# CICE-Consortium/CICE

Measured on AMD Instinct MI355X. Metric: EVP subcycle cell-updates/sec (gx1 fp64), higher is better.
Workload: dtype f64

## Files before the change

### __graft_entry__.py

```python
from __future__ import annotations

import os
import subprocess
import sys
from pathlib import Path

ROOT = Path(__file__).resolve().parent
CSRC = ROOT / "cice_amd" / "csrc"
LIB = ROOT / "cice_amd" / "libcice_evp_hip.so"
HIPCC = os.environ.get("HIPCC", "/opt/rocm/bin/hipcc")


def _stale(target: Path, sources) -> bool:
    if not target.exists():
        return True
    t = target.stat().st_mtime
    return any(Path(s).stat().st_mtime > t for s in sources)


HIP_SRCS = ["evp_kernels.hip", "evp_resident2.hip", "evp_halo_direct.hip", "evp_prep.hip",
            "evp_copy.hip", "evp_cgrid.hip", "evp_cgrid_res.hip", "evp_cgrid_prep.hip", "evp_march.hip", "evp_api.cpp", "evp_host_common.cpp", "evp_host_loop.cpp",
            "evp_host_resident.cpp", "evp_host_mailbox.cpp", "evp_host_prep.cpp", "evp_host_cgrid.cpp", "evp_host_march.cpp", "march_plan.cpp", "halo_plan.cpp", "cgrid_plan.cpp", "rim_plan.cpp"]
HIP_HDRS = ["evp_cell.inc", "evp_device.h", "evp_forcing.h", "evp_math.h", "halo_plan.h", "cgrid_plan.h", "evp_host.h", "evp_halo_direct.h", "march_plan.h", "rim_plan.h"]


LIB_TESTING = ROOT / "cice_amd" / "libcice_evp_hip_testing.so"
TESTING_KERNELS = {"evp_resident2.hip", "evp_cgrid_res.hip"}


def build_hip(force: bool = False) -> Path:
    from concurrent.futures import ThreadPoolExecutor
    srcs = [CSRC / n for n in HIP_SRCS if (CSRC / n).exists()]
    hdrs = [CSRC / n for n in HIP_HDRS if (CSRC / n).exists()] + [ROOT / "include" / "cice_evp_hip.h",
                                                                  ROOT / "include" / "cice_evp_hip_testing.h"]
    objdir = CSRC / "build"
    objdir.mkdir(exist_ok=True)
    flags = ["--offload-arch=gfx950", "-O3", "-std=c++17", "-fPIC"]
    jobs = [(src, objdir / (src.name + ".o"), []) for src in srcs]
    jobs += [(src, objdir / (src.name + ".testing.o"), ["-DCICE_EVP_HIP_TESTING"]) for src in srcs
             if src.suffix == ".cpp" or src.name in TESTING_KERNELS]

    def compile_one(job):
        src, obj, extra = job
        if force or _stale(obj, [src] + hdrs):
            subprocess.run([HIPCC, *flags, *extra, "-c", str(src), "-o", str(obj)], check=True)
        return obj

    with ThreadPoolExecutor(max_workers=min(8, os.cpu_count() or 1)) as ex:
        objs = list(ex.map(compile_one, jobs))
    kernels = [o for (src, o, extra) in jobs if src.suffix != ".cpp" and src.name not in TESTING_KERNELS]
    host = {False: [o for (src, o, extra) in jobs if (src.suffix == ".cpp" or src.name in TESTING_KERNELS) and not extra],
            True: [o for (src, o, extra) in jobs if extra]}
    for testing, lib in ((False, LIB), (True, LIB_TESTING)):
        mine = kernels + host[testing]
        if force or _stale(lib, mine + [CSRC / "exports.map"]):
            subprocess.run([HIPCC, "--offload-arch=gfx950", "-shared", "-fPIC", "-Wl,-Bsymbolic", f"-Wl,--version-script={CSRC / 'exports.map'}", *map(str, mine), "-o", str(lib),
                            "-L/opt/rocm/lib", "-lrccl"], check=True)
    return LIB


def build() -> None:
    build_hip()
    sys.path.insert(0, str(ROOT))
    sys.path.insert(0, str(ROOT / "oracle"))
    import oracle
    oracle.build()
    shim = ROOT / "cice_amd" / "fortran" / "build_shim.sh"
    if shim.exists():
        subprocess.run(["bash", str(shim)], check=True)
    ref = ROOT / "oracle" / "ref" / "build_ref.sh"
    try:
        have_reference = Path("/root/reference/cicecore").is_dir()
    except OSError:
        have_reference = False
    if have_reference:
        refdir = ROOT / "oracle" / "ref"
        srcs = [q for q in refdir.iterdir() if q.suffix in (".F90", ".c", ".sh")]
        shims = list((ROOT / "cice_amd" / "fortran").glob("*.F90"))
        out = ROOT / "oracle" / "_ref"
        for variant, binaries, extra in (("strict", ["evp_ref_harness_strict", "evp_hip_dropin_harness"], shims),
                                         ("fast", ["evp_ref_harness_fast", "evp_ref_harness_fast1d"], []),
                                         ("mpi", ["evp_ref_harness_mpistrict", "evp_ref_harness_mpifast", "evp_hip_dropin_harness_mpi"], shims)):
            if variant == "mpi" and not (Path("/opt/conda/include/mpif.h").exists() and Path("/opt/conda/lib/libmpifort.so.12").exists()):
                continue
            if any(_stale(out / b, srcs + extra) for b in binaries):
                subprocess.run(["bash", str(ref), variant], check=True)
    import cice_amd
    from cice_amd import evp
    evp.load_library()


def smoke() -> None:
    sys.path.insert(0, str(ROOT))
    sys.path.insert(0, str(ROOT / "oracle"))
    sys.path.insert(0, str(ROOT / "tests"))
    import numpy as np
    build_hip()
    from test_gpu_parity import run_hip, run_oracle, synth_case
    from cice_amd import synth
    scal = synth.evp_scalars(120)
    dc, geo, fields, tm, um = synth_case("gx3", "full", seed=1, warm=True, bs=(50, 58))
    want = run_oracle(dc, geo, fields, tm, um, scal, 8)
    got = run_hip(dc, geo, fields, tm, um, scal, strict=True, ndte=8)
    for k, w in want.items():
        assert np.array_equal(got[k].view(np.uint64), w.view(np.uint64)), f"smoke: {k} differs from the oracle (strict)"
    fused = run_hip(dc, geo, fields, tm, um, scal, strict=False, ndte=8)
# ... 11 lines not shown
```

### cice_amd/csrc/evp_api.cpp

```cpp
#include "evp_host.h"
#include "rim_plan.h"

using namespace evp_host;

namespace {
int32_t *at(int32_t *out, size_t k) { return out ? out + k : nullptr; }
template <class T> size_t copy_out(int32_t *out, const std::vector<T> &v, int stride = 1)
{
    for (size_t k = 0; out && k < v.size(); ++k) out[k * stride] = (int32_t)v[k];
    return v.size();
}
template <class T> size_t copy_out(int32_t *out, const std::vector<HaloPeer> &peers, std::vector<T> HaloPeer::*member, int stride = 1)
{
    size_t n = 0;
    for (const HaloPeer &p : peers) n += copy_out(at(out, n * stride), p.*member, stride);
    return n;
}
}

#ifdef CICE_EVP_HIP_TESTING
namespace {
struct PlanDump {
    int32_t *out;
    int32_t n = 0;
// ... 933 lines not shown
    PlanDump count{nullptr};
    count.put(S.plan);
    if (!out) return count.n;
    if (n < count.n) return fail(-1, "plan_dump: room for %d values, %d needed", (int)n, (int)count.n);
    PlanDump dump{out};
    dump.put(S.plan);
    return dump.n;
}

int cice_evp_hip_halo_plan(int32_t *counts4, int32_t *local_dst, int32_t *local_src,
                           int32_t *local_sign, int32_t *peer_rank, int32_t *peer_nsend,
                           int32_t *peer_nrecv, int32_t *send_src, int32_t *recv_dst)
{
    const HaloPlan &P = S.plan;
    copy_out(local_dst, P.local_dst);
    copy_out(local_src, P.local_src);
    copy_out(local_sign, P.local_sign);
    const size_t ns = copy_out(send_src, P.peers, &HaloPeer::send_src), nr = copy_out(recv_dst, P.peers, &HaloPeer::recv_dst);
    for (size_t q = 0; q < P.peers.size(); ++q) {
        if (peer_rank) peer_rank[q] = P.peers[q].rank;
        if (peer_nsend) peer_nsend[q] = (int32_t)P.peers[q].send_src.size();
        if (peer_nrecv) peer_nrecv[q] = (int32_t)P.peers[q].recv_dst.size();
    }
    if (counts4) {
        counts4[0] = (int32_t)P.local_dst.size();
        counts4[1] = (int32_t)P.peers.size();
        counts4[2] = (int32_t)ns;
        counts4[3] = (int32_t)nr;
    }
    return 0;
}

int cice_evp_hip_peer_plan(int32_t *send_dst, int32_t *recv_gid)
{
    copy_out(send_dst, S.plan.peers, &HaloPeer::send_dst);
    copy_out(recv_gid, S.plan.peers, &HaloPeer::recv_gid);
    return 0;
}

int cice_evp_hip_fold_images_plan(int32_t *counts4, int32_t *send_sign, int32_t *out3, int32_t *in3)
{
    const std::vector<HaloPeer> &peers = S.plan.peers;
    for (size_t q = 0; counts4 && q < peers.size(); ++q) {
        const HaloPeer &p = peers[q];
        counts4[4 * q] = p.n_ghost_send; counts4[4 * q + 1] = p.n_ghost_recv;
        counts4[4 * q + 2] = (int32_t)p.fimg_src.size(); counts4[4 * q + 3] = (int32_t)p.fimg_recv_dst.size();
    }
    copy_out(send_sign, peers, &HaloPeer::send_sign);
    copy_out(out3, peers, &HaloPeer::fimg_src, 3);
    copy_out(at(out3, 1), peers, &HaloPeer::fimg_dst, 3);
    copy_out(at(out3, 2), peers, &HaloPeer::fimg_sign, 3);
    copy_out(in3, peers, &HaloPeer::fimg_recv_dst, 3);
    copy_out(at(in3, 1), peers, &HaloPeer::fimg_recv_col, 3);
    copy_out(at(in3, 2), peers, &HaloPeer::fimg_recv_sign, 3);
    return 0;
}

int cice_evp_hip_peer_signs(int32_t *recv_sign)
{
    copy_out(recv_sign, S.plan.peers, &HaloPeer::recv_sign);
    return 0;
}

int cice_evp_hip_center_plan(int32_t *count, int32_t *dst, int32_t *src, int32_t *vsign)
{
    const HaloPlan &P = S.plan;
    const size_t n = copy_out(dst, P.center_dst);
    copy_out(src, P.center_src);
    copy_out(vsign, P.center_vsign);
    if (count) *count = (int32_t)n;
    return P.center_remote ? 1 : 0;
}

int cice_evp_hip_fold_split_plan(int32_t which, int32_t *count, int32_t *cells)
{
    const HaloPlan &P = S.plan;
    const std::vector<int32_t> *lists[9] = {&P.fold_shift_cells, &P.center_foldr_dst, &P.stress_foldr_dst, &P.center_seam_dst, &P.center_seam_slot,
                                            &P.stress_own_dst, &P.stress_own_src, &P.stress_corner_dst, &P.stress_corner_src};
    const size_t n = copy_out(cells, *lists[which >= 0 && which < 8 ? which : 8]);
    if (count) *count = (int32_t)n;
    return P.fold_split ? 1 : 0;
}

int cice_evp_hip_stress_plan(int32_t *count, int32_t *dst, int32_t *src)
{
    const size_t n = copy_out(dst, S.plan.stress_dst);
    copy_out(src, S.plan.stress_src);
    if (count) *count = (int32_t)n;
    return 0;
}
#endif

int cice_evp_hip_seam_fin_plan(int32_t *counts2, int32_t *dst, int32_t *a, int32_t *b, int32_t *coef)
{
    const HaloPlan &P = S.plan;
    if (counts2) { counts2[0] = (int32_t)P.fin_dst.size(); counts2[1] = (int32_t)P.tail; }
    copy_out(dst, P.fin_dst);
    copy_out(a, P.fin_a);
    copy_out(b, P.fin_b);
    copy_out(coef, P.fin_coef);
    return P.stress_remote ? 1 : 0;
}

int cice_evp_hip_march_info(int32_t *out, int32_t n)
{
    const State::March &M = S.march;
    const int32_t v[12] = {M.mode, (int32_t)std::min<long>(M.passes, 0x7fffffffL), M.declined, M.nstrips, M.nseg, M.seglen,
                           M.last_call ? 1 : 0, M.direct, M.kpass, (int32_t)std::min<long>(M.subcycles, 0x7fffffffL),
                           M.mode == 1 ? M.fold_h : 0, M.last_call ? M.call_band_subcycles : 0};
    for (int k = 0; out && k < n && k < 12; ++k) out[k] = v[k];
    return 0;
}

int cice_evp_hip_describe_path(char *buf, int32_t n)
{
    if (!buf || n < 2) return fail(-1, "describe_path: no buffer");
    const State::March &M = S.march;
    const char *kernel = S.res_mode == 1 ? (S.res_remote ? "on-chip resident (tagged records, neighbours on other ranks)"
                                                       : S.res2_rimu ? "on-chip resident (tagged records; edge U-cells in the rim wave)"
                                                                     : "on-chip resident (tagged records)")
                         : (M.last_call ? (M.kpass == 4 ? "four subcycles per pass (marching)" : M.kpass == 3 ? "three subcycles per pass (marching)" : "two subcycles per pass (marching)")
                                      : "one subcycle per launch (streaming)");
    const char *transport = S.plan.peers.empty() ? "none (one rank)" : (S.direct.on ? "mailbox over HIP IPC" : (S.have_comm ? "RCCL send/recv" : "not set up"));
    const char *ring = (M.mode == 1 && !S.plan.peers.empty())
                           ? (M.direct == 1 ? " (ring between ranks: stores into HIP-IPC-mapped inboxes)"
                                            : (M.direct == 2 ? " (ring between ranks: RCCL send/recv, direct stores on trial)" : " (ring between ranks: RCCL send/recv)"))
                           : "";
    char band[96] = "";
    if (M.mode == 1 && M.fold_h > 0)
        std::snprintf(band, sizeof band, " (tripole: rows 1 .. %d marched, fold band of %d rows one subcycle per launch)", M.fold_zone, M.fold_h);
    std::snprintf(buf, (size_t)n, "rank %d of %d: kernel = %s; halo transport = %s%s%s; marching path: %s%s%s%s%s; blocks %d, cells per exchange %d",
                  (int)S.d.rank, (int)std::max(1, (int)S.d.nranks), kernel, transport,
                  (!S.plan.peers.empty() && !S.direct.on && !S.direct.why.empty()) ? " (mailbox off: " : "",
                  (!S.plan.peers.empty() && !S.direct.on && !S.direct.why.empty()) ? (S.direct.why + ")").c_str() : "",
                  M.mode == 1 ? "on" : (M.mode == 0 ? "off" : "undecided"), (M.mode == 0 && !M.why.empty()) ? " -- " : "",
                  (M.mode == 0 && !M.why.empty()) ? M.why.c_str() : "", ring, band, (int)S.d.nblocks, (int)(S.msk.on ? S.msk.n_send : S.n_send));
    const std::string cg = cgrid_schedule();
    if (!cg.empty()) {
        const size_t used = std::strlen(buf);
        std::snprintf(buf + used, (size_t)n - used, "; %s", cg.c_str());
    }
    return 0;
}

#ifdef CICE_EVP_HIP_TESTING
int cice_evp_hip_plan_flags(int32_t *flags, int32_t n)
{
    const HaloPlan &P = S.plan;
    const int32_t v[5] = {P.any_fold_exchange, P.fold_rows, P.stress_remote, P.center_remote, P.center_fold_remote};
    int32_t k = 0;
    for (; flags && k < n && k < 5; ++k) flags[k] = v[k];
    return k;
}

int cice_evp_hip_cgrid_fold_xplan(int32_t loc, int32_t *info4, int32_t *count, int32_t *dst, int32_t *a, int32_t *b, int32_t *flip)
{
    if (loc < 0 || loc > 3) return fail(-1, "bad location %d", (int)loc);
    const HaloPlan &P = S.plan;
    if (info4) {
        info4[0] = P.cg_split ? 1 : 0;
        info4[1] = P.cg_tail;
        info4[2] = (int32_t)P.cg_peers.size();
        info4[3] = 0;
        for (const HaloPeer &p : P.cg_peers) info4[3] += (int32_t)p.send_src.size();
    }
    const FoldList &L = P.cg_fold[loc];
// ... 44 lines not shown
```

### cice_amd/csrc/evp_cell.inc

```

struct StressIn {
    double u_ij, u_im, u_jm, u_mm;
    double v_ij, v_im, v_jm, v_mm;
    double dxT, dyT, dxhy, dyhx, cxp, cyp, cxm, cym, DminTarea, strength;
};

__device__ __forceinline__ void metrics_cell(double hte, double hte_im, double htn, double htn_jm,
                                             double deltaminEVP, StressIn &a)
{
    a.cyp = (c1p5 * hte - p5 * hte_im);
    a.cxp = (c1p5 * htn - p5 * htn_jm);
    a.cym = -(c1p5 * hte_im - p5 * hte);
    a.cxm = -(c1p5 * htn_jm - p5 * htn);
    a.dxhy = p5 * (hte - hte_im);
    a.dyhx = p5 * (htn - htn_jm);
    const double tarea = a.dxT * a.dyT;
    a.DminTarea = deltaminEVP * tarea;
}

template <int CAP, bool SIMPLE = false>
__device__ __forceinline__ void visc_replpress(const EvpScalars &p, double strength, double DminArea,
                                               double Delta, double &zetax2, double &etax2,
                                               double &rep_prs)
{
    double tmpcalc;
    if (CAP == 1) {
        tmpcalc = strength / fmax(Delta, DminArea);
    } else if (CAP == 0) {
        tmpcalc = strength / (Delta + DminArea);
    } else {
        tmpcalc = p.capping * (strength / fmax(Delta, DminArea)) +
                  (1.0 - p.capping) * (strength / (Delta + DminArea));
    }
    if (SIMPLE) {
        zetax2 = tmpcalc;
        rep_prs = tmpcalc * Delta;
    } else {
        zetax2 = (1.0 + p.Ktens) * tmpcalc;
        rep_prs = (1.0 - p.Ktens) * tmpcalc * Delta;
    }
    etax2 = p.epp2i * zetax2;
}

template <int CAP, bool SIMPLE = false>
__device__ __forceinline__ void stress_cell(const EvpScalars &p, const StressIn &a, double (&s)[12],
                                            double (&str)[8])
{
    const double divune = a.cyp * a.u_ij - a.dyT * a.u_im + a.cxp * a.v_ij - a.dxT * a.v_jm;
    const double divunw = a.cym * a.u_im + a.dyT * a.u_ij + a.cxp * a.v_im - a.dxT * a.v_mm;
    const double divusw = a.cym * a.u_mm + a.dyT * a.u_jm + a.cxm * a.v_mm + a.dxT * a.v_im;
    const double divuse = a.cyp * a.u_jm - a.dyT * a.u_mm + a.cxm * a.v_jm + a.dxT * a.v_ij;
    const double tensionne = -a.cym * a.u_ij - a.dyT * a.u_im + a.cxm * a.v_ij + a.dxT * a.v_jm;
    const double tensionnw = -a.cyp * a.u_im + a.dyT * a.u_ij + a.cxm * a.v_im + a.dxT * a.v_mm;
    const double tensionsw = -a.cyp * a.u_mm + a.dyT * a.u_jm + a.cxp * a.v_mm - a.dxT * a.v_im;
    const double tensionse = -a.cym * a.u_jm - a.dyT * a.u_mm + a.cxp * a.v_jm - a.dxT * a.v_ij;
    const double shearne = -a.cym * a.v_ij - a.dyT * a.v_im - a.cxm * a.u_ij - a.dxT * a.u_jm;
    const double shearnw = -a.cyp * a.v_im + a.dyT * a.v_ij - a.cxm * a.u_im - a.dxT * a.u_mm;
    const double shearsw = -a.cyp * a.v_mm + a.dyT * a.v_jm - a.cxp * a.u_mm + a.dxT * a.u_im;
    const double shearse = -a.cym * a.v_jm - a.dyT * a.v_mm - a.cxp * a.u_jm + a.dxT * a.u_ij;
    const double Deltane = sqrt(divune * divune + p.e_factor * (tensionne * tensionne + shearne * shearne));
    const double Deltanw = sqrt(divunw * divunw + p.e_factor * (tensionnw * tensionnw + shearnw * shearnw));
    const double Deltasw = sqrt(divusw * divusw + p.e_factor * (tensionsw * tensionsw + shearsw * shearsw));
    const double Deltase = sqrt(divuse * divuse + p.e_factor * (tensionse * tensionse + shearse * shearse));

    double zetax2ne, etax2ne, rep_prsne, zetax2nw, etax2nw, rep_prsnw;
    double zetax2sw, etax2sw, rep_prssw, zetax2se, etax2se, rep_prsse;
    visc_replpress<CAP, SIMPLE>(p, a.strength, a.DminTarea, Deltane, zetax2ne, etax2ne, rep_prsne);
    visc_replpress<CAP, SIMPLE>(p, a.strength, a.DminTarea, Deltanw, zetax2nw, etax2nw, rep_prsnw);
    visc_replpress<CAP, SIMPLE>(p, a.strength, a.DminTarea, Deltasw, zetax2sw, etax2sw, rep_prssw);
    visc_replpress<CAP, SIMPLE>(p, a.strength, a.DminTarea, Deltase, zetax2se, etax2se, rep_prsse);

    const double arlx1i = p.arlx1i, revp = p.revp, denom1 = p.denom1;
    if (SIMPLE) {
        s[0] = (s[0] + arlx1i * (zetax2ne * divune - rep_prsne)) * denom1;
        s[1] = (s[1] + arlx1i * (zetax2nw * divunw - rep_prsnw)) * denom1;
        s[2] = (s[2] + arlx1i * (zetax2sw * divusw - rep_prssw)) * denom1;
        s[3] = (s[3] + arlx1i * (zetax2se * divuse - rep_prsse)) * denom1;

        s[4] = (s[4] + arlx1i * etax2ne * tensionne) * denom1;
        s[5] = (s[5] + arlx1i * etax2nw * tensionnw) * denom1;
        s[6] = (s[6] + arlx1i * etax2sw * tensionsw) * denom1;
        s[7] = (s[7] + arlx1i * etax2se * tensionse) * denom1;

        s[8] = (s[8] + arlx1i * p5 * etax2ne * shearne) * denom1;
        s[9] = (s[9] + arlx1i * p5 * etax2nw * shearnw) * denom1;
        s[10] = (s[10] + arlx1i * p5 * etax2sw * shearsw) * denom1;
        s[11] = (s[11] + arlx1i * p5 * etax2se * shearse) * denom1;
    } else {
    s[0] = (s[0] * (1.0 - arlx1i * revp) + arlx1i * (zetax2ne * divune - rep_prsne)) * denom1;
    s[1] = (s[1] * (1.0 - arlx1i * revp) + arlx1i * (zetax2nw * divunw - rep_prsnw)) * denom1;
    s[2] = (s[2] * (1.0 - arlx1i * revp) + arlx1i * (zetax2sw * divusw - rep_prssw)) * denom1;
    s[3] = (s[3] * (1.0 - arlx1i * revp) + arlx1i * (zetax2se * divuse - rep_prsse)) * denom1;

    s[4] = (s[4] * (1.0 - arlx1i * revp) + arlx1i * etax2ne * tensionne) * denom1;
    s[5] = (s[5] * (1.0 - arlx1i * revp) + arlx1i * etax2nw * tensionnw) * denom1;
    s[6] = (s[6] * (1.0 - arlx1i * revp) + arlx1i * etax2sw * tensionsw) * denom1;
    s[7] = (s[7] * (1.0 - arlx1i * revp) + arlx1i * etax2se * tensionse) * denom1;

    s[8] = (s[8] * (1.0 - arlx1i * revp) + arlx1i * p5 * etax2ne * shearne) * denom1;
    s[9] = (s[9] * (1.0 - arlx1i * revp) + arlx1i * p5 * etax2nw * shearnw) * denom1;
    s[10] = (s[10] * (1.0 - arlx1i * revp) + arlx1i * p5 * etax2sw * shearsw) * denom1;
    s[11] = (s[11] * (1.0 - arlx1i * revp) + arlx1i * p5 * etax2se * shearse) * denom1;
    }

    const double ssigpn = s[0] + s[1];
    const double ssigps = s[2] + s[3];
    const double ssigpe = s[0] + s[3];
    const double ssigpw = s[1] + s[2];
    const double ssigp1 = (s[0] + s[2]) * p055;
    const double ssigp2 = (s[1] + s[3]) * p055;

    const double ssigmn = s[4] + s[5];
    const double ssigms = s[6] + s[7];
    const double ssigme = s[4] + s[7];
    const double ssigmw = s[5] + s[6];
    const double ssigm1 = (s[4] + s[6]) * p055;
    const double ssigm2 = (s[5] + s[7]) * p055;

    const double ssig12n = s[8] + s[9];
    const double ssig12s = s[10] + s[11];
    const double ssig12e = s[8] + s[11];
    const double ssig12w = s[9] + s[10];
    const double ssig121 = (s[8] + s[10]) * p111;
    const double ssig122 = (s[9] + s[11]) * p111;

    const double csigpne = p111 * s[0] + ssigp2 + p027 * s[2];
    const double csigpnw = p111 * s[1] + ssigp1 + p027 * s[3];
    const double csigpsw = p111 * s[2] + ssigp2 + p027 * s[0];
    const double csigpse = p111 * s[3] + ssigp1 + p027 * s[1];

    const double csigmne = p111 * s[4] + ssigm2 + p027 * s[6];
    const double csigmnw = p111 * s[5] + ssigm1 + p027 * s[7];
    const double csigmsw = p111 * s[6] + ssigm2 + p027 * s[4];
    const double csigmse = p111 * s[7] + ssigm1 + p027 * s[5];

    const double csig12ne = p222 * s[8] + ssig122 + p055 * s[10];
    const double csig12nw = p222 * s[9] + ssig121 + p055 * s[11];
    const double csig12sw = p222 * s[10] + ssig122 + p055 * s[8];
    const double csig12se = p222 * s[11] + ssig121 + p055 * s[9];

    const double str12ew = p5 * a.dxT * (p333 * ssig12e + p166 * ssig12w);
    const double str12we = p5 * a.dxT * (p333 * ssig12w + p166 * ssig12e);
    const double str12ns = p5 * a.dyT * (p333 * ssig12n + p166 * ssig12s);
    const double str12sn = p5 * a.dyT * (p333 * ssig12s + p166 * ssig12n);

    double strp_tmp = p25 * a.dyT * (p333 * ssigpn + p166 * ssigps);
    double strm_tmp = p25 * a.dyT * (p333 * ssigmn + p166 * ssigms);
    str[0] = -strp_tmp - strm_tmp - str12ew + a.dxhy * (-csigpne + csigmne) + a.dyhx * csig12ne;
    str[1] = strp_tmp + strm_tmp - str12we + a.dxhy * (-csigpnw + csigmnw) + a.dyhx * csig12nw;
    strp_tmp = p25 * a.dyT * (p333 * ssigps + p166 * ssigpn);
    strm_tmp = p25 * a.dyT * (p333 * ssigms + p166 * ssigmn);
    str[2] = -strp_tmp - strm_tmp + str12ew + a.dxhy * (-csigpse + csigmse) + a.dyhx * csig12se;
    str[3] = strp_tmp + strm_tmp + str12we + a.dxhy * (-csigpsw + csigmsw) + a.dyhx * csig12sw;

    strp_tmp = p25 * a.dxT * (p333 * ssigpe + p166 * ssigpw);
    strm_tmp = p25 * a.dxT * (p333 * ssigme + p166 * ssigmw);
    str[4] = -strp_tmp + strm_tmp - str12ns - a.dyhx * (csigpne + csigmne) + a.dxhy * csig12ne;
    str[5] = strp_tmp - strm_tmp - str12sn - a.dyhx * (csigpse + csigmse) + a.dxhy * csig12se;
    strp_tmp = p25 * a.dxT * (p333 * ssigpw + p166 * ssigpe);
    strm_tmp = p25 * a.dxT * (p333 * ssigmw + p166 * ssigme);
    str[6] = -strp_tmp + strm_tmp + str12ns - a.dyhx * (csigpnw + csigmnw) + a.dxhy * csig12nw;
    str[7] = strp_tmp - strm_tmp + str12sn - a.dyhx * (csigpsw + csigmsw) + a.dxhy * csig12sw;
}

struct CornerIn {
    double ua, va, ub, vb, ud, vd;
    double cyA, cyB, cxA, cxB, DY, DX;
    double strength, DminTarea;
};
template <int CAP, bool SIMPLE = false>
__device__ __forceinline__ void stress_corner(const EvpScalars &p, const CornerIn &c, double &sp, double &sm, double &s12)
{
    const double divu = c.cyA * c.ua + c.DY * c.ub + c.cxA * c.va + c.DX * c.vd;
    const double tension = -c.cyB * c.ua + c.DY * c.ub + c.cxB * c.va - c.DX * c.vd;
    const double shear = -c.cyB * c.va + c.DY * c.vb - c.cxB * c.ua + c.DX * c.ud;
    const double Delta = sqrt(divu * divu + p.e_factor * (tension * tension + shear * shear));
    double zetax2, etax2, rep_prs;
    visc_replpress<CAP, SIMPLE>(p, c.strength, c.DminTarea, Delta, zetax2, etax2, rep_prs);
    const double arlx1i = p.arlx1i, revp = p.revp, denom1 = p.denom1;
    if (SIMPLE) {
        sp = (sp + arlx1i * (zetax2 * divu - rep_prs)) * denom1;
        sm = (sm + arlx1i * etax2 * tension) * denom1;
        s12 = (s12 + arlx1i * p5 * etax2 * shear) * denom1;
    } else {
        sp = (sp * (1.0 - arlx1i * revp) + arlx1i * (zetax2 * divu - rep_prs)) * denom1;
        sm = (sm * (1.0 - arlx1i * revp) + arlx1i * etax2 * tension) * denom1;
        s12 = (s12 * (1.0 - arlx1i * revp) + arlx1i * p5 * etax2 * shear) * denom1;
    }
}
__device__ __forceinline__ void corner_operands(int q, double dxT, double dyT, double cxp, double cyp, double cxm, double cym,
                                                CornerIn &c, double &KX, double &K12X, double &KYP, double &K12Y)
{
    const bool east = q == 0 || q == 3, north = q < 2;
    c.cyA = east ? cyp : cym; c.cyB = east ? cym : cyp;
    c.cxA = north ? cxp : cxm; c.cxB = north ? cxm : cxp;
    c.DY = east ? -dyT : dyT;
    c.DX = north ? -dxT : dxT;
    KX = (east ? -p25 : p25) * dyT;
    K12X = (north ? -p5 : p5) * dxT;
    KYP = (north ? -p25 : p25) * dxT;
    K12Y = (east ? -p5 : p5) * dyT;
}
__device__ __forceinline__ void stress_corner_partials(double P0, double P1, double P2, double P3, double M0, double M1, double M2,
                                                       double M3, double T0, double T1, double T2, double T3, double KX, double K12X,
                                                       double KYP, double K12Y, double dxhy, double dyhx, double &X, double &Y)
{
    const double csigp = p111 * P0 + (P1 + P3) * p055 + p027 * P2;
    const double csigm = p111 * M0 + (M1 + M3) * p055 + p027 * M2;
    const double csig12 = p222 * T0 + (T1 + T3) * p111 + p055 * T2;
    const double str12x = K12X * (p333 * (T0 + T3) + p166 * (T1 + T2));
    const double str12y = K12Y * (p333 * (T0 + T1) + p166 * (T2 + T3));
    const double strp_x = KX * (p333 * (P0 + P1) + p166 * (P2 + P3));
    const double strm_x = KX * (p333 * (M0 + M1) + p166 * (M2 + M3));
    X = strp_x + strm_x + str12x + dxhy * (-csigp + csigm) + dyhx * csig12;
    const double strp_y = KYP * (p333 * (P0 + P3) + p166 * (P1 + P2));
    const double strm_y = -KYP * (p333 * (M0 + M3) + p166 * (M1 + M2));
    Y = strp_y + strm_y + str12y - dyhx * (csigp + csigm) + dxhy * csig12;
}

struct StepuIn {
    double uold, vold;
    double vrelfac;
    double uocn, vocn, waterx, watery, forcex, forcey, Umassdti, fm, uarear, TbU;
    double uvel_init, vvel_init;
    double sx0, sx1, sx2, sx3;
    double sy0, sy1, sy2, sy3;
};

struct StepuOut {
    double u, v, strintx, strinty, taubx, tauby;
};

struct StepuPre {
    double taux, tauy, Cb, cca, ccb, ab2;
    double bu, bv;
};

template <bool SIMPLE = false, bool TBU = true, bool WITH_B = true>
__device__ __forceinline__ void stepu_pre_cell(const EvpScalars &p, const StepuIn &a, StepuPre &w)
{
    const double uold = a.uold, vold = a.vold;
    const double du = a.uocn - uold, dv = a.vocn - vold;
    const double vrel = a.vrelfac * sqrt(du * du + dv * dv);
    w.taux = vrel * a.waterx;
    w.tauy = vrel * a.watery;
    double Cb = 0.0;
    if (TBU) Cb = a.TbU / (sqrt(uold * uold + vold * vold) + p.u0);
    w.Cb = Cb;
    double cca, ccb;
    if (SIMPLE) {
        cca = p.brlx * a.Umassdti + vrel + Cb;
        ccb = a.fm;
    } else {
        cca = (p.brlx + p.revp) * a.Umassdti + vrel * p.cosw + Cb;
        ccb = a.fm + copysign(1.0, a.fm) * vrel * p.sinw;
    }
    w.cca = cca; w.ccb = ccb;
    w.ab2 = cca * cca + ccb * ccb;
    if (!WITH_B) return;
    if (SIMPLE) {
        w.bu = p.brlx * uold + 0.0;
        w.bv = p.brlx * vold + 0.0;
    } else {
        w.bu = p.brlx * uold + p.revp * a.uvel_init;
        w.bv = p.brlx * vold + p.revp * a.vvel_init;
    }
}

template <bool SIMPLE = false, bool WITH_B = true>
__device__ __forceinline__ void stepu_post_cell(const EvpScalars &p, const StepuIn &a, const StepuPre &w, StepuOut &o)
{
    o.strintx = a.uarear * (a.sx0 + a.sx1 + a.sx2 + a.sx3);
    o.strinty = a.uarear * (a.sy0 + a.sy1 + a.sy2 + a.sy3);
    double cc1, cc2;
    if (WITH_B) {
        cc1 = o.strintx + a.forcex + w.taux + a.Umassdti * w.bu;
        cc2 = o.strinty + a.forcey + w.tauy + a.Umassdti * w.bv;
    } else if (SIMPLE) {
        cc1 = o.strintx + a.forcex + w.taux + a.Umassdti * (p.brlx * a.uold + 0.0);
        cc2 = o.strinty + a.forcey + w.tauy + a.Umassdti * (p.brlx * a.vold + 0.0);
    } else {
        cc1 = o.strintx + a.forcex + w.taux + a.Umassdti * (p.brlx * a.uold + p.revp * a.uvel_init);
        cc2 = o.strinty + a.forcey + w.tauy + a.Umassdti * (p.brlx * a.vold + p.revp * a.vvel_init);
    }
    o.u = (w.cca * cc1 + w.ccb * cc2) / w.ab2;
    o.v = (w.cca * cc2 - w.ccb * cc1) / w.ab2;
    o.taubx = -o.u * w.Cb;
    o.tauby = -o.v * w.Cb;
}

template <bool SIMPLE = false, bool TBU = true>
__device__ __forceinline__ void stepu_cell(const EvpScalars &p, const StepuIn &a, StepuOut &o)
{
    StepuPre w;
    stepu_pre_cell<SIMPLE, TBU, false>(p, a, w);
    stepu_post_cell<SIMPLE, false>(p, a, w, o);
}

struct DeformOut {
    double divu, shear, vort, rdg_conv, rdg_shear;
};

__device__ __forceinline__ void deform_cell(const EvpScalars &p, const StressIn &a, double tarear,
                                            double dyU_ij, double dyU_im, double dyU_jm, double dyU_mm,
                                            double dxU_ij, double dxU_im, double dxU_jm, double dxU_mm,
                                            DeformOut &o)
{
    const double divune = a.cyp * a.u_ij - a.dyT * a.u_im + a.cxp * a.v_ij - a.dxT * a.v_jm;
    const double divunw = a.cym * a.u_im + a.dyT * a.u_ij + a.cxp * a.v_im - a.dxT * a.v_mm;
    const double divusw = a.cym * a.u_mm + a.dyT * a.u_jm + a.cxm * a.v_mm + a.dxT * a.v_im;
    const double divuse = a.cyp * a.u_jm - a.dyT * a.u_mm + a.cxm * a.v_jm + a.dxT * a.v_ij;
    const double tensionne = -a.cym * a.u_ij - a.dyT * a.u_im + a.cxm * a.v_ij + a.dxT * a.v_jm;
    const double tensionnw = -a.cyp * a.u_im + a.dyT * a.u_ij + a.cxm * a.v_im + a.dxT * a.v_mm;
    const double tensionsw = -a.cyp * a.u_mm + a.dyT * a.u_jm + a.cxp * a.v_mm - a.dxT * a.v_im;
    const double tensionse = -a.cym * a.u_jm - a.dyT * a.u_mm + a.cxp * a.v_jm - a.dxT * a.v_ij;
    const double shearne = -a.cym * a.v_ij - a.dyT * a.v_im - a.cxm * a.u_ij - a.dxT * a.u_jm;
    const double shearnw = -a.cyp * a.v_im + a.dyT * a.v_ij - a.cxm * a.u_im - a.dxT * a.u_mm;
    const double shearsw = -a.cyp * a.v_mm + a.dyT * a.v_jm - a.cxp * a.u_mm + a.dxT * a.u_im;
    const double shearse = -a.cym * a.v_jm - a.dyT * a.v_mm - a.cxp * a.u_jm + a.dxT * a.u_ij;
    const double Deltane = sqrt(divune * divune + p.e_factor * (tensionne * tensionne + shearne * shearne));
    const double Deltanw = sqrt(divunw * divunw + p.e_factor * (tensionnw * tensionnw + shearnw * shearnw));
    const double Deltasw = sqrt(divusw * divusw + p.e_factor * (tensionsw * tensionsw + shearsw * shearsw));
    const double Deltase = sqrt(divuse * divuse + p.e_factor * (tensionse * tensionse + shearse * shearse));

    o.divu = p25 * (divune + divunw + divuse + divusw) * tarear;
    const double tmp = p25 * (Deltane + Deltanw + Deltase + Deltasw) * tarear;
    o.rdg_conv = -fmin(o.divu, 0.0);
    o.rdg_shear = p5 * (tmp - fabs(o.divu));
    const double tsum = tensionne + tensionnw + tensionse + tensionsw;
    const double ssum = shearne + shearnw + shearse + shearsw;
    o.shear = p25 * tarear * sqrt(tsum * tsum + ssum * ssum);
    const double dvdxn = dyU_ij * a.v_ij - dyU_im * a.v_im;
    const double dvdxs = dyU_jm * a.v_jm - dyU_mm * a.v_mm;
    const double dudye = dxU_ij * a.u_ij - dxU_jm * a.u_jm;
    const double dudyw = dxU_im * a.u_im - dxU_mm * a.u_mm;
    o.vort = p5 * tarear * (dvdxn + dvdxs - dudye - dudyw);
}

__device__ __forceinline__ void finish_cell(const EvpScalars &p, double Cw, double aiX, double uocn,
                                            double vocn, double u, double v, double fm,
                                            double &strocnx, double &strocny)
{
    const double du = uocn - u, dv = vocn - v;
    double vrel = p.rhow * Cw * sqrt(du * du + dv * dv);
    vrel = vrel * aiX;
    strocnx = vrel * ((uocn - u) * p.cosw - (vocn - v) * p.sinw * copysign(1.0, fm));
    strocny = vrel * ((vocn - v) * p.cosw + (uocn - u) * p.sinw * copysign(1.0, fm));
}
```

### cice_amd/csrc/evp_device.h

```cpp
#pragma once
const char *evp_env_test(const char *key);
#include <hip/hip_runtime.h>
#include <stdint.h>
#include <algorithm>

struct EvpScalars {
    double arlx1i, denom1, brlx, revp;
    double e_factor, epp2i;
    double capping, Ktens;
    double u0, cosw, sinw;
    double rhow;
};

struct EvpArgs {
    EvpScalars p;
    int nx, ny;
    size_t plane;
    int gx, gy, ntiles;
    int xcdmap;
    const int *tile_list;
    int tile_count;
    int last;
    const int4 *blk;
    const uint8_t *mask;
    const double *u_in, *v_in;
    double *u_out, *v_out;
    const double *sig_in[12];
    double *sig_out[12];
    const double *dxT, *dyT, *dxhy, *dyhx, *cxp, *cyp, *cxm, *cym, *DminTarea, *uarear;
    const double *HTE, *HTN;
    double deltaminEVP;
    const double *strength, *Cw, *aiX, *uocn, *vocn, *waterx, *watery, *forcex, *forcey;
    const double *umassdti, *fm, *TbU, *uvel_init, *vvel_init;
    const double *vrelfac;
    unsigned flags;
    const int *push;
    int push_ni, push_nj;
    double *strintx, *strinty, *taubx, *tauby;
    const struct EvpDirect *dx;
    unsigned *dx_count;
    unsigned *dx_fseq;
    int dx_nb;
};

void evp_resident_geometry(int max_ni, int max_nj, int logw, int *gx, int *gy);
#define EVP_RES2_RING 256
struct EvpResident2 {
    int ndte;
    int cur0;
    int dry;
    unsigned tag_base;
    unsigned spin_limit;
    int *err;
    const uint8_t *pubmap;
    const int4 *ring;
    const int *ring_cnt;
    void *rec[2];
    double *u[2], *v[2];
    double *const *tab;
    int nblocks;
    const int *order;
    int nlaunch;
    const uint8_t *live;
    const int *celltile;
    const uint8_t *perm;
    const uint8_t *uperm;
    const uint8_t *late_waves;
    const uint8_t *nact;
    const uint8_t *nlate;
    int *cuload;
    unsigned long long *prof;
    int dbg;
    int par0;
    const int2 *rimg;
    void *const *peer_rec;
    const size_t *peer_rstride;
    unsigned long long timeout_ticks;
    const int *seam;
    int tfold;
    const int *img3;
    void *rec_raw[2];
    const int2 *rraw;
    void *const *peer_raw;
    const size_t *peer_raw_stride;
};
int evp_resident2_max_blocks_per_cu(bool strict, int cap, unsigned flags, int logw, bool remote, bool coop = false);
bool evp_resident2_coop_built(bool strict, int cap, int logw, bool remote);
bool evp_resident2_lean_built(bool strict, int cap, int logw, bool remote);
void evp_launch_resident2(const EvpArgs &A, const EvpResident2 &R, int max_ni, int max_nj, int logw,
                          bool strict, int cap, int lean, hipStream_t st);

#ifndef EVP_MARCH_PAD
#define EVP_MARCH_PAD 4
#endif
#define EVP_MARCH_KMAX EVP_MARCH_PAD
#define EVP_MARCH_OWN (64 - 2 * EVP_MARCH_PAD)
#define EVP_MARCH_S_NF 14
#define EVP_MARCH_C_NF 13
#define EVP_MARCH_O_NF 5
#define EVP_MARCH_D_NF 4
#define EVP_MARCH_NODUP 0xffffffffu
struct EvpMarch {
    EvpScalars p;
    double deltaminEVP;
    int nxr, nyr;
    int ldx;
    int own;
    int nstrips, nseg, seglen, nitems;
    int wrapx;
    int last;
    int kpass;
    int order;
    unsigned flags;
    const uint8_t *mask;
    const double *st_in;
    double *st_out;
    const double *cst;
    const double *opt;
    double *diag;
    const unsigned *dup;
    const int4 *items;
};
struct EvpMarchGeo {
    int nxr, nyr, ldx, rows;
    int own, nstrips;
    int nxb, nyb, plane;
    int nblocks;
    int bsx, bsy, nbx, nby;
    int ilo;
    int wrapx;
    int gx0, gy0, nxg, nyg, ew_cyclic;
    int ext_w, ext_s, nxo, nyo;
    int nyblk;
    const int *blkid;
    const int2 *blk_org;
    const int4 *blk;
};
#define EVP_MARCH_TAB 40
struct EvpMarchTab {
    double *blk[EVP_MARCH_TAB];
    double *pk[EVP_MARCH_TAB];
    double *pk2[EVP_MARCH_TAB];
    int nf[EVP_MARCH_TAB];
    int slot[EVP_MARCH_TAB];
    int n;
};
void evp_launch_march(const EvpMarch &A, bool strict, int mode, hipStream_t st);
struct EvpMarchRows { int y0, y1, j0, nj; };
constexpr EvpMarchRows EvpMarchAllRows{-(1 << 28), 1 << 28, 1, 1 << 28};
void evp_launch_march_gather(const EvpMarchGeo &G, const EvpMarchTab &T, const uint8_t *mask_blk, uint8_t *mask_rect,
                             EvpMarchRows W, hipStream_t st);
void evp_launch_march_check(const EvpMarchGeo &G, const EvpMarchTab &T, const uint8_t *mask_blk, const uint8_t *mask_rect,
                            int nuv, int nfringe, unsigned *bad, EvpMarchRows W, hipStream_t st);
void evp_launch_march_scatter(const EvpMarchGeo &G, const EvpMarchTab &T, const uint8_t *mask_blk, int nuv, int nsig,
                              EvpMarchRows W, hipStream_t st);
#define EVP_MARCH_DIRECT_MAXPEER 16
struct EvpRingCuts {
    int n;
    int start[EVP_MARCH_DIRECT_MAXPEER + 1];
};
void evp_launch_march_pack(const double *buf, int nf, const int *pos, int n, const EvpRingCuts &C, double *out, hipStream_t st);
struct EvpMarchDirect {
    int npeers;
    double *dst[EVP_MARCH_DIRECT_MAXPEER];
    size_t dst_pstride[EVP_MARCH_DIRECT_MAXPEER];
    unsigned *peer_flag[EVP_MARCH_DIRECT_MAXPEER];
    unsigned *flags_in;
    unsigned *count;
// ... 285 lines not shown
```

### cice_amd/csrc/evp_host_resident.cpp

```cpp
#include "evp_host.h"
#include "rim_plan.h"

namespace evp_host {

bool tripole_seam() { return (S.n_seam + S.n_pole + S.n_late) > 0 || S.plan.tail > 0 || !S.plan.fin_dst.empty(); }

static bool tfold_image(size_t k)
{
    if (!S.plan.tfold) return false;
    const int dst = S.plan.local_dst[k];
    const int b = dst / (int)S.plane, r = dst % (int)S.plane, j = r / S.d.nx_block + 1, i = r % S.d.nx_block + 1;
    return i >= S.ilo[b] && i <= S.ihi[b] && j >= S.jlo[b] && j <= S.jhi[b];
}

bool resident_possible(bool with_peers)
{
    if (!with_peers && !S.plan.peers.empty()) return false;
    if (S.plan.tfold) {
        for (const HaloPeer &p : S.plan.peers)
            for (int k = 0; k < p.n_ghost_recv; ++k) {
                const int dst = p.recv_dst[k];
                const int b = dst / (int)S.plane, r = dst % (int)S.plane, j = r / S.d.nx_block + 1, i = r % S.d.nx_block + 1;
                if (i >= S.ilo[b] && i <= S.ihi[b] && j >= S.jlo[b] && j <= S.jhi[b]) return false;
            }
// ... 297 lines not shown
    }
    S.res2_rimu_ok = rimu_ok;
    S.res2_coop_ok = coop_ok;
    const bool off = env_test("CICE_EVP_HIP_RES_ORDER") && !std::atoi(env_test("CICE_EVP_HIP_RES_ORDER"));
    std::vector<int> order((size_t)ntiles, 0);
    for (int w = 0; w < nrun; ++w) order[w] = run[w];
    if (!off) {
        hipDeviceProp_t prop;
        int ncu = 256;
        if (hipGetDeviceProperties(&prop, S.device) == hipSuccess && prop.multiProcessorCount > 0) ncu = prop.multiProcessorCount;
        std::vector<int> by_cost = run;
        std::stable_sort(by_cost.begin(), by_cost.end(), [&](int a, int c) { return cost[a] > cost[c]; });
        std::vector<int> slots((size_t)ncu), load((size_t)ncu, 0);
        std::vector<std::vector<int>> mine((size_t)ncu);
        for (int c = 0; c < ncu; ++c) slots[c] = nrun / ncu + (c < nrun % ncu ? 1 : 0);
        for (int tile : by_cost) {
            int best = -1;
            for (int c = 0; c < ncu; ++c) {
                if ((int)mine[c].size() >= slots[c]) continue;
                if (best < 0 || load[c] < load[best] || (load[c] == load[best] && slots[c] < slots[best])) best = c;
            }
            mine[best].push_back(tile);
            load[best] += cost[tile] >> 10;
        }
        for (int c = 0; c < ncu; ++c)
            for (size_t k = 0; k < mine[c].size(); ++k) order[c + (int)k * ncu] = mine[c][k];
    }
    if (S.res2_order_for != S.res2_logw) S.mem.free_one(S.res2_order);
    if (!S.res2_order && S.mem.alloc(S.res2_order, order.size())) return -1;
    HIPC(hipMemcpyAsync(S.res2_order, order.data(), order.size() * sizeof(int), hipMemcpyHostToDevice, S.stream));
    HIPC(hipMemcpyAsync(S.res2_live, live.data(), live.size(), hipMemcpyHostToDevice, S.stream));
    HIPC(hipStreamSynchronize(S.stream));
    S.res2_nlive = nrun;
    S.res2_order_for = S.res2_logw;
    S.res2_order_stale = false;
    return 0;
}

int launch_resident2(int ndte, int cur0, bool dry)
{
    if (ndte >= 4096) return fail(-6, "resident2: ndte must be < 4096");
    if (int rc = resident_tables()) return rc;
    if (int rc = resident2_order()) return rc;
    EvpArgs A;
    fill_args(A, cur0, 1);
    EvpResident2 R;
    R.ndte = ndte;
    R.cur0 = dry ? 0 : cur0;
    R.dry = dry ? 1 : 0;
    S.res2_epoch = (S.res2_epoch + 1u) & 0xFFFFFu;
    if (S.res2_epoch == 0) S.res2_epoch = 1;
    R.tag_base = S.res2_epoch << 12;
    R.par0 = S.res2_par;
    S.res2_par = (S.res2_par + ndte + 1) & 1;
    R.nblocks = S.d.nblocks;
    R.order = S.res2_order;
    R.nlaunch = S.res2_nlive;
    R.live = S.plan.peers.empty() ? S.res2_live : nullptr;
    R.celltile = S.res2_celltile;
    R.perm = S.res2_perm;
    R.late_waves = S.res2_late;
    R.nact = S.res2_nact;
    {
        const int want = env_test("CICE_EVP_HIP_RES_COOP") ? std::atoi(env_test("CICE_EVP_HIP_RES_COOP")) : EVP_RES2_COOP_DEFAULT;
        bool can = want != 0 && S.res2_coop_ok && S.res2_logw == 4 && !S.res_remote &&
                   evp_resident2_coop_built(S.prm.strict != 0, cap_mode(), S.res2_logw, false);
        if (can) {
            hipDeviceProp_t prop;
            const int per_cu = std::min(evp_resident2_max_blocks_per_cu(S.prm.strict != 0, cap_mode(), A.flags, 4, false, true), 8);
            can = hipGetDeviceProperties(&prop, S.device) == hipSuccess &&
                  (long)std::max(S.res2_nlive, 1) * 10 <= (long)per_cu * prop.multiProcessorCount * 9;
        }
        S.res2_coop = can ? 1 : 0;
        R.nlate = can ? S.res2_nlate : nullptr;
    }
    R.cuload = S.res2_cuload;
    R.prof = nullptr;
    if (S.res2_logw == 4 && env_test("CICE_EVP_HIP_RES_PROF") && std::atoi(env_test("CICE_EVP_HIP_RES_PROF"))) {
        if (!S.res2_prof && S.mem.alloc(S.res2_prof, (size_t)S.res2_ntiles * 32)) return -1;
        HIPC(hipMemsetAsync(S.res2_prof, 0, (size_t)S.res2_ntiles * 32 * sizeof(unsigned long long), S.stream));
        R.prof = S.res2_prof;
    }
    const int dbg2 = env_test("CICE_EVP_HIP_RES_DEBUG") ? std::atoi(env_test("CICE_EVP_HIP_RES_DEBUG")) : 0;
    R.dbg = dbg2;
    R.seam = S.res2_seam;
    R.tfold = S.plan.tfold ? 1 : 0;
    R.img3 = S.res2_img3;
    R.rec_raw[0] = S.res2_rec_raw[0];
    R.rec_raw[1] = S.res2_rec_raw[1];
    R.rimg = S.res_remote ? S.res2_rimg : nullptr;
    R.peer_rec = S.res2_peer_rec;
    R.peer_rstride = S.res2_peer_rstride;
    R.rraw = S.res_remote ? S.res2_rraw : nullptr;
    R.peer_raw = S.res2_peer_raw;
    R.peer_raw_stride = S.res2_peer_raw_stride;
    const double tmo_ms = env("CICE_EVP_HIP_HALO_TIMEOUT_MS") ? std::atof(env("CICE_EVP_HIP_HALO_TIMEOUT_MS")) : 30000.0;
    R.timeout_ticks = (unsigned long long)((S.res_timeout_ms > 0 ? S.res_timeout_ms : tmo_ms) * 1.0e5);
    R.spin_limit = 4000000u;
    R.err = S.res_err;
    R.pubmap = S.res2_pub;
    R.ring = S.res2_ring;
    R.ring_cnt = S.res2_cnt;
    R.rec[0] = S.res2_rec[0];
    R.rec[1] = S.res2_rec[1];
    if (dry) {
        R.u[0] = S.u[cur0]; R.v[0] = S.v[cur0]; R.u[1] = S.u[cur0]; R.v[1] = S.v[cur0];
    } else {
        R.u[0] = S.u[0]; R.v[0] = S.v[0]; R.u[1] = S.u[1]; R.v[1] = S.v[1];
    }
    R.tab = S.res_tab + (dry ? 28 * (1 + cur0) : 0);
    const bool lean = evp_resident2_lean_built(S.prm.strict != 0, cap_mode(), S.res2_logw, R.rimg != nullptr) &&
                      R.nblocks == 1 && !R.seam && !R.tfold && !R.img3 && !R.rimg && !R.rraw && !R.nlate &&
                      A.p.revp == 0.0 && (A.flags & EVP_F_WATER_IS_OCN) && (A.flags & EVP_F_TBU_ZERO) &&
                      !(env_test("CICE_EVP_HIP_RES_LEAN") && !std::atoi(env_test("CICE_EVP_HIP_RES_LEAN")));
    const int want_rimu = env_test("CICE_EVP_HIP_RES_RIMU") ? std::atoi(env_test("CICE_EVP_HIP_RES_RIMU")) : EVP_RES2_RIMU_DEFAULT;
    const bool rimu = lean && want_rimu != 0 && S.res2_rimu_ok && !(dbg2 & (32 | 256 | 512));
    R.uperm = nullptr;
    if (rimu) { R.perm = S.res2_perm_rim; R.uperm = S.res2_uperm; R.nact = S.res2_nact_rim; }
    S.res2_rimu = rimu ? 1 : 0;
    evp_launch_resident2(A, R, S.max_ni, S.max_nj, S.res2_logw, S.prm.strict != 0, cap_mode(), rimu ? 2 : lean ? 1 : 0, S.stream);
    HIPC(hipGetLastError());
    return 0;
}

int resident_tables()
{
    if (!S.res_tab) {
        double *tab[3][28];
        for (int v = 0; v < 3; ++v) {
            for (int k = 0; k < 12; ++k) {
                tab[v][k] = S.sig[v == 0 ? 0 : v - 1][k];
                tab[v][12 + k] = S.sig[v == 0 ? 1 : v - 1][k];
            }
            tab[v][24] = S.in[F_STRINTX]; tab[v][25] = S.in[F_STRINTY];
            tab[v][26] = S.in[F_TAUBX]; tab[v][27] = S.in[F_TAUBY];
        }
        if (S.mem.alloc(S.res_tab, sizeof tab / sizeof(double *))) return -1;
        HIPC(hipMemcpy(S.res_tab, tab, sizeof tab, hipMemcpyHostToDevice));
    }
    return 0;
}

int resident_check_error()
{
    if (!S.res_launched) return 0;
    S.res_launched = false;
    int ev[8] = {0};
    HIPC(hipMemcpy(ev, S.res_err, sizeof ev, hipMemcpyDeviceToHost));
    const int e = ev[0];
    if (e) {
        HIPC(hipMemset(S.res_err, 0, sizeof ev));
        S.res_mode = 0;
        return fail(-7, "resident EVP kernel: a wait gave up (%s; tile %d, subcycle %d, cell %d, tag seen %#x, wanted %#x)%s",
                    e == 1 ? "record of this GPU" : e == 2 ? "record of another rank" : e == 3 ? "fold-row partner"
                           : e == 5 ? "interior waves of the tile" : "?",
                    ev[1], ev[2], ev[3], (unsigned)ev[4], (unsigned)ev[5],
                    e == 2 ? " -- CICE_EVP_HIP_HALO_TIMEOUT_MS bounds the wait for other ranks"
                           : " -- workgroups not co-resident?");
    }
    return 0;
}


int tune_after_upload()
{
    float ms = 0;
    if (!S.tyb_forced && !S.tuned) {
// ... 74 lines not shown
```

### cice_amd/csrc/evp_math.h

```cpp
#pragma once
#include <hip/hip_runtime.h>
#include "evp_device.h"

namespace {

__device__ constexpr double p027 = 1.0 / 36.0;
__device__ constexpr double p055 = 1.0 / 18.0;
__device__ constexpr double p111 = 1.0 / 9.0;
__device__ constexpr double p166 = 1.0 / 6.0;
__device__ constexpr double p222 = 2.0 / 9.0;
__device__ constexpr double p25 = 0.25;
__device__ constexpr double p333 = 1.0 / 3.0;
__device__ constexpr double p5 = 0.5;
__device__ constexpr double c1p5 = 1.5;

}

#pragma clang fp contract(off)
namespace evp_strict {
#include "evp_cell.inc"
}
#pragma clang fp contract(on)
namespace evp_fused {
#include "evp_cell.inc"
}

namespace {

template <bool STRICT> struct Math;
template <> struct Math<true> {
    using SI = evp_strict::StressIn;
    using UI = evp_strict::StepuIn;
    using UO = evp_strict::StepuOut;
    template <int MODE>
    static __device__ __forceinline__ void stress(const EvpScalars &p, const SI &a, double (&s)[12], double (&str)[8])
    {
        evp_strict::stress_cell<(MODE == 3 ? 1 : MODE), MODE == 3>(p, a, s, str);
    }
    template <int MODE = -1, bool TBU = true>
    static __device__ __forceinline__ void stepu(const EvpScalars &p, const UI &a, UO &o) { evp_strict::stepu_cell<MODE == 3, TBU>(p, a, o); }
    using UP = evp_strict::StepuPre;
    template <int MODE = -1, bool TBU = true>
    static __device__ __forceinline__ void stepu_pre(const EvpScalars &p, const UI &a, UP &w) { evp_strict::stepu_pre_cell<MODE == 3, TBU>(p, a, w); }
    template <int MODE = -1>
    static __device__ __forceinline__ void stepu_post(const EvpScalars &p, const UI &a, const UP &w, UO &o) { evp_strict::stepu_post_cell<MODE == 3, true>(p, a, w, o); }
    static __device__ __forceinline__ void metrics(double hte, double hte_im, double htn, double htn_jm, double dmin, SI &a)
    {
        evp_strict::metrics_cell(hte, hte_im, htn, htn_jm, dmin, a);
    }
    using CI = evp_strict::CornerIn;
    template <int MODE>
    static __device__ __forceinline__ void corner(const EvpScalars &p, const CI &c, double &sp, double &sm, double &s12)
    {
        evp_strict::stress_corner<(MODE == 3 ? 1 : MODE), MODE == 3>(p, c, sp, sm, s12);
    }
    static __device__ __forceinline__ void corner_operands(int q, double dxT, double dyT, double cxp, double cyp, double cxm, double cym,
                                                           CI &c, double &KX, double &K12X, double &KYP, double &K12Y)
    {
        evp_strict::corner_operands(q, dxT, dyT, cxp, cyp, cxm, cym, c, KX, K12X, KYP, K12Y);
    }
    static __device__ __forceinline__ void partials(double P0, double P1, double P2, double P3, double M0, double M1, double M2, double M3,
                                                    double T0, double T1, double T2, double T3, double KX, double K12X, double KYP,
                                                    double K12Y, double dxhy, double dyhx, double &X, double &Y)
    {
        evp_strict::stress_corner_partials(P0, P1, P2, P3, M0, M1, M2, M3, T0, T1, T2, T3, KX, K12X, KYP, K12Y, dxhy, dyhx, X, Y);
    }
};
template <> struct Math<false> {
    using SI = evp_fused::StressIn;
    using UI = evp_fused::StepuIn;
    using UO = evp_fused::StepuOut;
    template <int MODE>
    static __device__ __forceinline__ void stress(const EvpScalars &p, const SI &a, double (&s)[12], double (&str)[8])
    {
        evp_fused::stress_cell<(MODE == 3 ? 1 : MODE), MODE == 3>(p, a, s, str);
    }
    template <int MODE = -1, bool TBU = true>
    static __device__ __forceinline__ void stepu(const EvpScalars &p, const UI &a, UO &o) { evp_fused::stepu_cell<MODE == 3, TBU>(p, a, o); }
    using UP = evp_fused::StepuPre;
    template <int MODE = -1, bool TBU = true>
    static __device__ __forceinline__ void stepu_pre(const EvpScalars &p, const UI &a, UP &w) { evp_fused::stepu_pre_cell<MODE == 3, TBU>(p, a, w); }
    template <int MODE = -1>
    static __device__ __forceinline__ void stepu_post(const EvpScalars &p, const UI &a, const UP &w, UO &o) { evp_fused::stepu_post_cell<MODE == 3, true>(p, a, w, o); }
    static __device__ __forceinline__ void metrics(double hte, double hte_im, double htn, double htn_jm, double dmin, SI &a)
    {
        evp_fused::metrics_cell(hte, hte_im, htn, htn_jm, dmin, a);
    }
    using CI = evp_fused::CornerIn;
    template <int MODE>
    static __device__ __forceinline__ void corner(const EvpScalars &p, const CI &c, double &sp, double &sm, double &s12)
    {
        evp_fused::stress_corner<(MODE == 3 ? 1 : MODE), MODE == 3>(p, c, sp, sm, s12);
    }
    static __device__ __forceinline__ void corner_operands(int q, double dxT, double dyT, double cxp, double cyp, double cxm, double cym,
                                                           CI &c, double &KX, double &K12X, double &KYP, double &K12Y)
    {
        evp_fused::corner_operands(q, dxT, dyT, cxp, cyp, cxm, cym, c, KX, K12X, KYP, K12Y);
    }
    static __device__ __forceinline__ void partials(double P0, double P1, double P2, double P3, double M0, double M1, double M2, double M3,
                                                    double T0, double T1, double T2, double T3, double KX, double K12X, double KYP,
                                                    double K12Y, double dxhy, double dyhx, double &X, double &Y)
    {
        evp_fused::stress_corner_partials(P0, P1, P2, P3, M0, M1, M2, M3, T0, T1, T2, T3, KX, K12X, KYP, K12Y, dxhy, dyhx, X, Y);
    }
};

}
```

### cice_amd/csrc/evp_resident2.hip

```cpp
#include <hip/hip_runtime.h>
#include <stdint.h>
#include <algorithm>

#ifdef CICE_EVP_HIP_TESTING
#define RES_DBG(R) ((R).dbg)
#define RES_PROF(R) ((R).prof != nullptr)
#else
#define RES_DBG(R) 0
#define RES_PROF(R) false
#endif

#include "evp_math.h"

namespace {

constexpr int RTY = 4;

typedef unsigned v4u __attribute__((ext_vector_type(4)));

__device__ __forceinline__ void st_rec2(void *p, v4u a, v4u b)
{
    asm volatile("global_store_dwordx4 %0, %1, off sc1\n\tglobal_store_dwordx4 %0, %2, off offset:16 sc1"
                 :
                 : "v"(p), "v"(a), "v"(b)
                 : "memory");
}
__device__ __forceinline__ void ld_rec2(const void *p, v4u &a, v4u &b)
{
    asm volatile("global_load_dwordx4 %0, %2, off sc1\n\tglobal_load_dwordx4 %1, %2, off offset:16 sc1\n\ts_waitcnt vmcnt(0)"
                 : "=&v"(a), "=&v"(b)
                 : "v"(p)
                 : "memory");
}
__device__ __forceinline__ void st_rec2_s(const void *base, unsigned off, v4u a, v4u b)
{
    asm volatile("global_store_dwordx4 %0, %1, %3 sc1\n\tglobal_store_dwordx4 %0, %2, %3 offset:16 sc1"
                 :
                 : "v"(off), "v"(a), "v"(b), "s"(base)
                 : "memory");
}
__device__ __forceinline__ void ld_rec2_s(const void *base, unsigned off, v4u &a, v4u &b)
{
    asm volatile("global_load_dwordx4 %0, %2, %3 sc1\n\tglobal_load_dwordx4 %1, %2, %3 offset:16 sc1\n\ts_waitcnt vmcnt(0)"
                 : "=&v"(a), "=&v"(b)
                 : "v"(off), "s"(base)
                 : "memory");
}
__device__ __forceinline__ void st_rec2_sys(void *p, v4u a, v4u b)
{
    asm volatile("global_store_dwordx4 %0, %1, off sc0 sc1\n\tglobal_store_dwordx4 %0, %2, off offset:16 sc0 sc1"
                 :
                 : "v"(p), "v"(a), "v"(b)
                 : "memory");
}
__device__ __forceinline__ void ld_rec2_sys(const void *p, v4u &a, v4u &b)
{
    asm volatile("global_load_dwordx4 %0, %2, off sc0 sc1\n\tglobal_load_dwordx4 %1, %2, off offset:16 sc0 sc1\n\ts_waitcnt vmcnt(0)"
                 : "=&v"(a), "=&v"(b)
                 : "v"(p)
                 : "memory");
}
__device__ __forceinline__ v4u pack_rec(double x, unsigned tag)
{
    const unsigned long long bits = (unsigned long long)__double_as_longlong(x);
    v4u r;
    r.x = tag; r.y = (unsigned)bits; r.z = (unsigned)(bits >> 32); r.w = tag;
    return r;
}
__device__ __forceinline__ double unpack_rec(v4u r)
{
    return __longlong_as_double((long long)(((unsigned long long)r.z << 32) | r.y));
}

template <int CTRL>
__device__ __forceinline__ double quad_perm(double v)
{
    const long long b = __double_as_longlong(v);
    const int lo = __builtin_amdgcn_update_dpp(0, (int)(b & 0xffffffffll), CTRL, 0xf, 0xf, false);
    const int hi = __builtin_amdgcn_update_dpp(0, (int)(b >> 32), CTRL, 0xf, 0xf, false);
    return __longlong_as_double(((long long)hi << 32) | (unsigned)lo);
}
constexpr int QP_X1 = 0xB1, QP_X2 = 0x4E, QP_X3 = 0x1B;

template <bool STRICT, int CAP, int LOGW, bool REMOTE, bool COOP = false, bool LEAN = false, bool RIMU = false>
__global__ __launch_bounds__(64 * RTY, REMOTE ? 2 : 3) void evp_resident2_tile(EvpArgs A, EvpResident2 R)
{
    static_assert(!COOP || (STRICT && CAP == 3 && LOGW == 4), "COOP: 16 x 16 tiles, strict build, default scalars");
    static_assert(!LEAN || (!REMOTE && !COOP && LOGW == 4), "LEAN: one rank, 16 x 16 tiles, one thread per rim cell");
    static_assert(!RIMU || LEAN, "RIMU: a schedule of the lean loop");
    using MM = Math<STRICT>;
    constexpr int W = 1 << LOGW;
    constexpr int H = 256 / W;
    constexpr int LW = W + 1;
    constexpr int NUV = ((H + 1) * LW + 7) & ~7;
    constexpr bool PERM = (LOGW == 4);
    constexpr int NSTR = RIMU ? 8 : PERM ? 6 : 4;
    constexpr int SW = PERM ? W + 1 : W;
    constexpr int SP = SW * H;
    extern __shared__ __attribute__((aligned(16))) double smem[];
    double *s_str = smem;
    double *s_tc = smem + NSTR * SP;
    double *s_u = s_tc + 4 * 256;
    double *s_v = s_u + NUV;
    double *s_uc = s_v + NUV;
    double *s_rc = nullptr, *s_r04 = nullptr;
    __shared__ int s_bad;

    __shared__ int s_chunk[4], s_simd[4], s_cu;
    __shared__ int s_slot[4];

    const int tx = threadIdx.x, ty = threadIdx.y;
    const int t = ty * 64 + tx;
    const int tile = R.order ? R.order[blockIdx.x] : (int)blockIdx.x;
    bool no_ucell;
    {
        const int pb = A.gx * A.gy;
        const int4 rb = A.blk[tile / pb];
        no_ucell = rb.x + ((tile % pb) % A.gx) * (W - 1) > rb.y || rb.z + ((tile % pb) / A.gx) * (H - 1) > rb.w;
        if (no_ucell && !(RES_DBG(R) & 512)) return;
    }
    int tq = t;
    int cu_rank = 0;
    if (PERM && R.cuload && !(RES_DBG(R) & 64)) {
        const int wave = t >> 6;
        if ((t & 63) == 0) {
            unsigned hw, xcc;
            asm volatile("s_getreg_b32 %0, hwreg(HW_REG_HW_ID)" : "=s"(hw));
            asm volatile("s_getreg_b32 %0, hwreg(HW_REG_XCC_ID)" : "=s"(xcc));
            s_simd[wave] = (int)((hw >> 4) & 3u);
            if (wave == 0) s_cu = (int)(((xcc & 7u) << 8) | ((hw >> 8) & 0xffu));
        }
        __syncthreads();
        if (t == 0) {
            int *L = R.cuload + 8 * s_cu;
            const int nact = R.nact[tile];
            int chunk_of[4] = {0, 1, 2, 3};
            unsigned spins = 0;
            bool locked = false;
            while (spins++ < 200000u) {
                if (atomicCAS(&L[0], 0, 1) == 0) { locked = true; break; }
                __builtin_amdgcn_s_sleep(2);
            }
            if (locked) {
                int ld[4];
                const int stamp = __hip_atomic_load(&L[1], __ATOMIC_RELAXED, __HIP_MEMORY_SCOPE_AGENT);
                const bool fresh = stamp != (int)R.tag_base;
#pragma unroll
                for (int q = 0; q < 4; ++q)
                    ld[q] = fresh ? 0 : __hip_atomic_load(&L[2 + q], __ATOMIC_RELAXED, __HIP_MEMORY_SCOPE_AGENT);
                const int rank = fresh ? 0 : __hip_atomic_load(&L[6], __ATOMIC_RELAXED, __HIP_MEMORY_SCOPE_AGENT);
                s_simd[0] |= rank << 8;
                bool used[4] = {false, false, false, false};
                for (int ck = 0; ck < 4; ++ck) {
                    int best = -1;
                    for (int w = 0; w < 4; ++w) {
                        if (used[w]) continue;
                        if (best < 0 || ld[s_simd[w] & 3] < ld[s_simd[best] & 3]) best = w;
                    }
                    used[best] = true;
                    chunk_of[best] = ck;
                    if (ck < nact) ld[s_simd[best] & 3] += 1;
                }
#pragma unroll
                for (int q = 0; q < 4; ++q) __hip_atomic_store(&L[2 + q], ld[q], __ATOMIC_RELAXED, __HIP_MEMORY_SCOPE_AGENT);
                __hip_atomic_store(&L[6], rank + 1, __ATOMIC_RELAXED, __HIP_MEMORY_SCOPE_AGENT);
                __hip_atomic_store(&L[1], (int)R.tag_base, __ATOMIC_RELAXED, __HIP_MEMORY_SCOPE_AGENT);
                asm volatile("s_waitcnt vmcnt(0)" ::: "memory");
                __hip_atomic_store(&L[0], 0, __ATOMIC_RELAXED, __HIP_MEMORY_SCOPE_AGENT);
            }
#pragma unroll
            for (int w = 0; w < 4; ++w) s_chunk[w] = chunk_of[w];
        }
        __syncthreads();
// ... 13 lines not shown
    const int by = (tile % per_blk) / A.gx;
    const int4 r = A.blk[bz];
    const int i0 = r.x + bx * (W - 1), j0 = r.z + by * (H - 1);
    const int i = i0 + tcol;
    const int j = j0 + trow;
    const int nx = A.nx, ny = A.ny;
    const int cb = bz * (int)A.plane;
    const int c = cb + (j - 1) * nx + (i - 1);
    const int li = (trow + 1) * LW + (tcol + 1);
    const int upos = RIMU ? (int)R.uperm[tile * 256 + tq] : pos;
    const int ucol = upos & (W - 1), urow = upos >> LOGW;
    const int ui = RIMU ? i0 + ucol : i, uj = RIMU ? j0 + urow : j;
    const int cu = RIMU ? cb + (uj - 1) * nx + (ui - 1) : c;
    const int uli = RIMU ? (urow + 1) * LW + (ucol + 1) : li;
    const int usp = RIMU ? urow * SW + ucol : sp;
    const unsigned flags = A.flags;
    const bool water = !LEAN && !(flags & EVP_F_WATER_IS_OCN);
    const bool tbu = !LEAN && !(flags & EVP_F_TBU_ZERO);
    if (COOP) {
        s_rc = s_uc + (8 + (water ? 2 : 0) + (tbu ? 1 : 0)) * 256;
        s_r04 = s_rc + 10 * 64;
    }

    const bool inT = (i <= r.y + 1) && (j <= r.w + 1);
    unsigned m = 0;
    if (inT) m = A.mask[c];
    const bool actT = inT && (m & 1u);
    const bool ownU = (ucol < W - 1) && (urow < H - 1) && (ui <= r.y) && (uj <= r.w);
    unsigned mU = m;
    if (RIMU) mU = ownU ? A.mask[cu] : 0u;
    const bool isU = ownU && (mU & 2u);
    const bool own = (tcol < W - 1 || i == r.y + 1) && (trow < H - 1 || j == r.w + 1);
    const bool pub = ownU && (R.pubmap[cu] != 0);
    const int par0 = R.par0;
    const int nlate = COOP ? (int)R.nlate[tile] : 0;
    const bool rim_owner = COOP && tq < nlate;
    const bool actN = actT && !rim_owner;
    const int g = t >> 2, qc = t & 3;
    const bool quad = COOP && g < nlate;
    int gc = 0;
    unsigned g_vel = 0, g_out = 0;
    bool gown = false;
    double sr0 = 0.0, sr1 = 0.0, sr2 = 0.0;
    if (quad) {
        const int gpos = (int)R.perm[tile * 256 + g];
        const int gcol = gpos & (W - 1), grow = gpos >> LOGW;
        const int gi = i0 + gcol, gj = j0 + grow;
        gc = cb + (gj - 1) * nx + (gi - 1);
        gown = (gcol < W - 1 || gi == r.y + 1) && (grow < H - 1 || gj == r.w + 1);
        const int gli = (grow + 1) * LW + (gcol + 1);
        const int ij = gli, im = gli - 1, jm = gli - LW, mm = gli - LW - 1;
        const int g_oa = qc == 0 ? ij : qc == 1 ? im : qc == 2 ? mm : jm;
        const int g_ob = qc == 0 ? im : qc == 1 ? ij : qc == 2 ? jm : mm;
        const int g_od = qc == 0 ? jm : qc == 1 ? mm : qc == 2 ? im : ij;
        g_vel = (unsigned)g_oa | ((unsigned)g_ob << 10) | ((unsigned)g_od << 20);
        const int gsp = grow * SW + gcol;
        const int off04 = (int)(s_r04 - s_str);
        const int g_ox = qc == 0 ? off04 + g : (qc == 1 ? 4 : qc == 2 ? 2 : 0) * SP + gsp;
        const int g_oy = qc == 0 ? off04 + 64 + g : (qc == 1 ? 5 : qc == 2 ? 3 : 1) * SP + gsp;
        g_out = (unsigned)g_ox | ((unsigned)g_oy << 16);
        sr0 = R.tab[R.cur0 * 12 + qc][gc];
        sr1 = R.tab[R.cur0 * 12 + 4 + qc][gc];
        sr2 = R.tab[R.cur0 * 12 + 8 + qc][gc];
        if (qc == 0) {
            typename MM::SI b;
            b.dxT = A.dxT[gc]; b.dyT = A.dyT[gc];
            b.strength = A.strength[gc];
            if ((flags & EVP_F_METRICS) && !(flags & EVP_F_DXHY_ARRAY)) {
                MM::metrics(A.HTE[gc], A.HTE[gc - 1], A.HTN[gc], A.HTN[gc - nx], A.deltaminEVP, b);
            } else {
                b.dxhy = A.dxhy[gc]; b.dyhx = A.dyhx[gc];
                b.cxp = A.cxp[gc]; b.cyp = A.cyp[gc]; b.cxm = A.cxm[gc]; b.cym = A.cym[gc];
                b.DminTarea = A.DminTarea[gc];
            }
            s_rc[0 * 64 + g] = b.strength; s_rc[1 * 64 + g] = b.DminTarea;
            s_rc[2 * 64 + g] = b.dxT; s_rc[3 * 64 + g] = b.dyT;
            s_rc[4 * 64 + g] = b.cxp; s_rc[5 * 64 + g] = b.cyp; s_rc[6 * 64 + g] = b.cxm; s_rc[7 * 64 + g] = b.cym;
            s_rc[8 * 64 + g] = b.dxhy; s_rc[9 * 64 + g] = b.dyhx;
        }
    }

    typename MM::SI a;
    double s[12];
    if (actN) {
#pragma unroll
        for (int k = 0; k < 12; ++k) s[k] = R.tab[R.cur0 * 12 + k][c];
        a.dxT = A.dxT[c]; a.dyT = A.dyT[c];
        a.strength = A.strength[c];
        if ((flags & EVP_F_METRICS) && !(flags & EVP_F_DXHY_ARRAY)) {
            MM::metrics(A.HTE[c], A.HTE[c - 1], A.HTN[c], A.HTN[c - nx], A.deltaminEVP, a);
        } else {
            a.dxhy = A.dxhy[c]; a.dyhx = A.dyhx[c];
            a.cxp = A.cxp[c]; a.cyp = A.cyp[c]; a.cxm = A.cxm[c]; a.cym = A.cym[c];
            a.DminTarea = A.DminTarea[c];
        }
        s_tc[0 * 256 + t] = a.strength;
        s_tc[1 * 256 + t] = a.DminTarea;
        s_tc[2 * 256 + t] = a.dxhy;
        s_tc[3 * 256 + t] = a.dyhx;
    }
    if (isU) {
        s_uc[0 * 256 + t] = A.vrelfac[cu];
        s_uc[1 * 256 + t] = A.uocn[cu];
        s_uc[2 * 256 + t] = A.vocn[cu];
        s_uc[3 * 256 + t] = A.forcex[cu];
        s_uc[4 * 256 + t] = A.forcey[cu];
        s_uc[5 * 256 + t] = A.umassdti[cu];
        s_uc[6 * 256 + t] = A.fm[cu];
        s_uc[7 * 256 + t] = A.uarear[cu];
        int row = 8;
        if (water) { s_uc[row * 256 + t] = A.waterx[cu]; s_uc[(row + 1) * 256 + t] = A.watery[cu]; row += 2; }
        if (tbu) s_uc[row * 256 + t] = A.TbU[cu];
    }
    {
        const double *u0 = R.u[R.cur0], *v0 = R.v[R.cur0];
        for (int q = t; q < (H + 1) * LW; q += 256) {
            const int pr = q / LW - 1, pc = q % LW - 1;
            const int gi = i0 + pc, gj = j0 + pr;
            double uu = 0.0, vv = 0.0;
            if (gi >= 1 && gi <= nx && gj >= 1 && gj <= ny) {
                const int cp = cb + (gj - 1) * nx + (gi - 1);
                uu = u0[cp]; vv = v0[cp];
            }
            s_u[q] = uu; s_v[q] = vv;
        }
    }
    int img0 = -1, img1 = -1, img2 = -1;
    int seam_role = 0, seam_partner = -1;
    if (!LEAN && R.seam && ownU && j == r.w) {
        const int sv = R.seam[bz * nx + i - 1];
        seam_role = sv & 3;
        seam_partner = sv >> 2;
    }
    const bool isSeam = seam_role != 0;
    if (!LEAN && R.img3) {
        if (ownU) { img0 = R.img3[3 * c]; img1 = R.img3[3 * c + 1]; img2 = R.img3[3 * c + 2]; }
    } else
    if (ownU && (flags & EVP_F_PUSH) && (ui == r.x || ui == r.y || uj == r.z || uj == r.w)) {
        const int slots[4] = {(ui == r.x) ? (uj - r.z) : -1, (ui == r.y) ? A.push_nj + (uj - r.z) : -1,
                              (uj == r.z) ? 2 * A.push_nj + (ui - r.x) : -1,
                              (uj == r.w) ? 2 * A.push_nj + A.push_ni + (ui - r.x) : -1};
#pragma unroll
        for (int e = 0; e < 4; ++e) {
            if (slots[e] < 0) continue;
#pragma unroll
            for (int w = 0; w < 2; ++w) {
                const int v = A.push[slots[e] * 2 + w];
                if (v < 0) continue;
                if (img0 < 0) img0 = v;
                else if (img1 < 0) img1 = v;
                else img2 = v;
            }
        }
    }
    char *rp0 = nullptr, *rp1 = nullptr, *rp2 = nullptr;
    size_t rs0 = 0, rs1 = 0, rs2 = 0;
    double rg0 = 1.0, rg1 = 1.0, rg2 = 1.0;
    char *rq0 = nullptr, *rq1 = nullptr, *rq2 = nullptr;
    size_t rqs0 = 0, rqs1 = 0, rqs2 = 0;
    if (REMOTE) {
        if (ownU) {
#pragma unroll
            for (int e = 0; e < 3; ++e) {
                const int2 v = R.rimg[3 * (size_t)c + e];
                if (v.x < 0) continue;
                const int pe = v.x & 255;
                char *ptr = (char *)R.peer_rec[pe] + 32 * (size_t)v.y;
                const size_t st = R.peer_rstride[pe];
                const double sg = (v.x & 256) ? -1.0 : 1.0;
                if (!rp0) { rp0 = ptr; rs0 = st; rg0 = sg; }
                else if (!rp1) { rp1 = ptr; rs1 = st; rg1 = sg; }
                else { rp2 = ptr; rs2 = st; rg2 = sg; }
            }
            if (R.rraw && isSeam) {
#pragma unroll
                for (int e = 0; e < 3; ++e) {
                    const int2 v = R.rraw[3 * (size_t)c + e];
                    if (v.x < 0) continue;
                    char *ptr = (char *)R.peer_raw[v.x] + 32 * (size_t)v.y;
                    const size_t st = R.peer_raw_stride[v.x];
                    if (!rq0) { rq0 = ptr; rqs0 = st; }
                    else if (!rq1) { rq1 = ptr; rqs1 = st; }
                    else { rq2 = ptr; rqs2 = st; }
// ... 49 lines not shown
            return wall_clock64() - t0 > R.timeout_ticks ||
                   __hip_atomic_load(R.err, __ATOMIC_RELAXED, __HIP_MEMORY_SCOPE_AGENT) != 0;
        }
        return spins > R.spin_limit ||
               ((spins & 255u) == 0 && __hip_atomic_load(R.err, __ATOMIC_RELAXED, __HIP_MEMORY_SCOPE_AGENT) != 0);
    };
    double u_own = 0.0, v_own = 0.0;
    if (ownU) { u_own = s_u[uli]; v_own = s_v[uli]; }
    {
        const unsigned tag = R.tag_base;
        v4u *r0 = (v4u *)R.rec[par0 & 1];
        if (rpub) publish_remote(par0 & 1, u_own, v_own, tag);
        if (pub) st_rec2(r0 + 2 * (size_t)cu, pack_rec(u_own, tag), pack_rec(v_own, tag));
        if (ownU) {
            if (img0 >= 0) { const double sg = (img0 & 1) ? -1.0 : 1.0; st_rec2(r0 + 2 * (size_t)(img0 >> 1), pack_rec(sg * u_own, tag), pack_rec(sg * v_own, tag)); }
            if (img1 >= 0) { const double sg = (img1 & 1) ? -1.0 : 1.0; st_rec2(r0 + 2 * (size_t)(img1 >> 1), pack_rec(sg * u_own, tag), pack_rec(sg * v_own, tag)); }
            if (img2 >= 0) { const double sg = (img2 & 1) ? -1.0 : 1.0; st_rec2(r0 + 2 * (size_t)(img2 >> 1), pack_rec(sg * u_own, tag), pack_rec(sg * v_own, tag)); }
        }
    }

    const bool prof = RES_PROF(R);
    unsigned long long pc0 = 0, pacc0 = 0, pacc1 = 0, pacc2 = 0, pacc3 = 0, pacc4 = 0;
    if (prof) pc0 = __builtin_readcyclecounter();
#define EVP_STAMP(acc)                                                  \
    if (prof) {                                                         \
        const unsigned long long now_ = __builtin_readcyclecounter();   \
        acc += now_ - pc0;                                              \
        pc0 = now_;                                                     \
    }
    const unsigned ring_off = 32u * (unsigned)(ring_cp >= 0 ? ring_cp : 0);
    const unsigned own_off = 32u * (unsigned)cu;
    const unsigned img_off0 = 32u * (unsigned)(img0 >> 1), img_off1 = 32u * (unsigned)(img1 >> 1), img_off2 = 32u * (unsigned)(img2 >> 1);
    const double img_sg0 = (img0 & 1) ? -1.0 : 1.0, img_sg1 = (img1 & 1) ? -1.0 : 1.0, img_sg2 = (img2 & 1) ? -1.0 : 1.0;
    auto subcycle = [&](const int k, const v4u *rd, v4u *wr) -> bool {
        const unsigned want = R.tag_base + (unsigned)k;

        if (((RES_DBG(R) & 8) && (tile & 3) == 1) || ((RES_DBG(R) & 256) && no_ucell)) {
            const unsigned long long t0 = wall_clock64();
            while (wall_clock64() - t0 < 1000ull) __builtin_amdgcn_s_sleep(8);
        }
        if (REMOTE && ring_remote) {
            v4u ra, rb;
            if (!poll_remote(rd + 2 * (size_t)ring_cp, want, ra, rb)) s_bad = 1;
            s_u[ring_li] = unpack_rec(ra);
            s_v[ring_li] = unpack_rec(rb);
        } else if (ring_cp >= 0 && !(RES_DBG(R) & 2)) {
            v4u ra, rb;
            unsigned spins = 0;
            if (REMOTE) t_wait0 = wall_clock64();
            for (;;) {
                if (LEAN) ld_rec2_s(rd, ring_off, ra, rb);
                else ld_rec2(rd + 2 * (size_t)ring_cp, ra, rb);
                if ((ra.x == want && ra.w == want && rb.x == want && rb.w == want) || (RES_DBG(R) & 1)) break;
                if (gave_up(++spins, t_wait0)) {
                    give_up_note(1, k, ring_cp, ra.x, want);
                    s_bad = 1;
                    break;
                }
                if (RES_DBG(R) & 4) __builtin_amdgcn_s_sleep(8); else __builtin_amdgcn_s_sleep(1);
            }
            s_u[ring_li] = unpack_rec(ra);
            s_v[ring_li] = unpack_rec(rb);
        }
        if (!split) {
            __syncthreads();
            if (s_bad) return false;
        } else {
            __builtin_amdgcn_fence(__ATOMIC_RELEASE, "wavefront");
            __builtin_amdgcn_wave_barrier();
            __builtin_amdgcn_fence(__ATOMIC_ACQUIRE, "wavefront");
        }
        EVP_STAMP(pacc0)

        double str[8];
#pragma unroll
        for (int e = 0; e < 8; ++e) str[e] = 0.0;
        if (actN) {
            a.u_ij = s_u[li]; a.v_ij = s_v[li];
            a.u_im = s_u[li - 1]; a.v_im = s_v[li - 1];
            a.u_jm = s_u[li - LW]; a.v_jm = s_v[li - LW];
            a.u_mm = s_u[li - LW - 1]; a.v_mm = s_v[li - LW - 1];
            a.strength = s_tc[0 * 256 + t]; a.DminTarea = s_tc[1 * 256 + t];
            a.dxhy = s_tc[2 * 256 + t]; a.dyhx = s_tc[3 * 256 + t];
            MM::template stress<CAP>(A.p, a, s, str);
        }
        EVP_STAMP(pacc1)
        double sx1, sy2;
        if (PERM) {
            if (!rim_owner) {
                s_str[0 * SP + sp] = str[2];
                s_str[1 * SP + sp] = str[5];
                s_str[2 * SP + sp] = str[3];
                s_str[3 * SP + sp] = str[7];
                s_str[4 * SP + sp] = str[1];
                s_str[5 * SP + sp] = str[6];
            }
            __syncthreads();
            if (split && s_bad) return false;
            if (COOP) {
                EVP_STAMP(pacc2)
                if (quad) {
                    typename MM::CI cn;
                    double KX, K12X, KYP, K12Y;
                    MM::corner_operands(qc, s_rc[2 * 64 + g], s_rc[3 * 64 + g], s_rc[4 * 64 + g], s_rc[5 * 64 + g], s_rc[6 * 64 + g],
                                        s_rc[7 * 64 + g], cn, KX, K12X, KYP, K12Y);
                    unsigned pv = g_vel, po = g_out;
                    asm volatile("" : "+v"(pv), "+v"(po));
                    const int g_oa = (int)(pv & 1023u), g_ob = (int)((pv >> 10) & 1023u), g_od = (int)(pv >> 20);
                    cn.ua = s_u[g_oa]; cn.va = s_v[g_oa];
                    cn.ub = s_u[g_ob]; cn.vb = s_v[g_ob];
                    cn.ud = s_u[g_od]; cn.vd = s_v[g_od];
                    cn.strength = s_rc[0 * 64 + g]; cn.DminTarea = s_rc[1 * 64 + g];
                    MM::template corner<CAP>(A.p, cn, sr0, sr1, sr2);
                    double X, Y;
                    MM::partials(sr0, quad_perm<QP_X1>(sr0), quad_perm<QP_X2>(sr0), quad_perm<QP_X3>(sr0),
                                 sr1, quad_perm<QP_X1>(sr1), quad_perm<QP_X2>(sr1), quad_perm<QP_X3>(sr1),
                                 sr2, quad_perm<QP_X1>(sr2), quad_perm<QP_X2>(sr2), quad_perm<QP_X3>(sr2),
                                 KX, K12X, KYP, K12Y, s_rc[8 * 64 + g], s_rc[9 * 64 + g], X, Y);
                    s_str[po & 0xffffu] = X;
                    s_str[po >> 16] = Y;
                }
                EVP_STAMP(pacc1)
                __syncthreads();
                if (rim_owner) { str[0] = s_r04[tq]; str[4] = s_r04[64 + tq]; }
            }
            sx1 = s_str[4 * SP + sp + 1];
            sy2 = s_str[5 * SP + sp + 1];
        } else {
            s_str[0 * SP + sp] = str[2];
            s_str[1 * SP + sp] = str[5];
            s_str[2 * SP + sp] = str[3];
            s_str[3 * SP + sp] = str[7];
            sx1 = __shfl_down(str[1], 1);
            sy2 = __shfl_down(str[6], 1);
            __syncthreads();
        }
        EVP_STAMP(pacc2)

        if (isU) {
            typename MM::UI q;
            typename MM::UO o;
            q.uold = u_own; q.vold = v_own;
            q.vrelfac = s_uc[0 * 256 + t]; q.uocn = s_uc[1 * 256 + t]; q.vocn = s_uc[2 * 256 + t];
            q.forcex = s_uc[3 * 256 + t]; q.forcey = s_uc[4 * 256 + t]; q.Umassdti = s_uc[5 * 256 + t];
            q.fm = s_uc[6 * 256 + t]; q.uarear = s_uc[7 * 256 + t];
            int row = 8;
            if (water) { q.waterx = s_uc[row * 256 + t]; q.watery = s_uc[(row + 1) * 256 + t]; row += 2; }
            else { q.waterx = q.uocn; q.watery = q.vocn; }
            q.TbU = tbu ? s_uc[row * 256 + t] : 0.0;
            q.uvel_init = !LEAN && A.p.revp != 0.0 ? A.uvel_init[c] : 0.0;
            q.vvel_init = !LEAN && A.p.revp != 0.0 ? A.vvel_init[c] : 0.0;
            q.sx0 = str[0]; q.sx1 = sx1;
            q.sx2 = s_str[0 * SP + sp + SW]; q.sx3 = s_str[2 * SP + sp + SW + 1];
            q.sy0 = str[4]; q.sy1 = s_str[1 * SP + sp + SW];
            q.sy2 = sy2; q.sy3 = s_str[3 * SP + sp + SW + 1];
            if (tbu) MM::template stepu<CAP, true>(A.p, q, o);
            else MM::template stepu<CAP, false>(A.p, q, o);
            u_own = o.u; v_own = o.v;
            if (k == R.ndte - 1 && !R.dry) {
                R.tab[24][c] = o.strintx; R.tab[25][c] = o.strinty;
                R.tab[26][c] = o.taubx; R.tab[27][c] = o.tauby;
            }
        }
        bool published = false;
        if (!LEAN && R.tfold && !isSeam) {
            if (ownU) {
                const unsigned tag = want + 1u;
                if (pub) st_rec2(wr + 2 * (size_t)c, pack_rec(u_own, tag), pack_rec(v_own, tag));
                if (img0 >= 0) { const double sg = (img0 & 1) ? -1.0 : 1.0; st_rec2(wr + 2 * (size_t)(img0 >> 1), pack_rec(sg * u_own, tag), pack_rec(sg * v_own, tag)); }
                if (img1 >= 0) { const double sg = (img1 & 1) ? -1.0 : 1.0; st_rec2(wr + 2 * (size_t)(img1 >> 1), pack_rec(sg * u_own, tag), pack_rec(sg * v_own, tag)); }
                if (img2 >= 0) { const double sg = (img2 & 1) ? -1.0 : 1.0; st_rec2(wr + 2 * (size_t)(img2 >> 1), pack_rec(sg * u_own, tag), pack_rec(sg * v_own, tag)); }
            }
            if (rpub) publish_remote(((k + par0) & 1) ^ 1, u_own, v_own, want + 1u);
            published = true;
        }
        if (isSeam) {
            const double isign = -1.0;
            const unsigned tag = want + 1u;
            if (R.tfold) {
                v4u ra, rb;
                unsigned spins = 0;
                if (REMOTE) t_wait0 = wall_clock64();
                for (;;) {
                    ld_rec2(wr + 2 * (size_t)seam_partner, ra, rb);
                    if (ra.x == tag && ra.w == tag && rb.x == tag && rb.w == tag) {
                        u_own = isign * unpack_rec(ra); v_own = isign * unpack_rec(rb);
                        break;
                    }
                    if (gave_up(++spins, t_wait0)) {
                        give_up_note(3, k, seam_partner, ra.x, tag);
                        s_bad = 1;
                        break;
                    }
                    __builtin_amdgcn_s_sleep(1);
                }
            } else if (seam_role == 3) {
                u_own = isign * u_own; v_own = isign * v_own;
            } else {
                v4u *rw = (v4u *)R.rec_raw[((k + par0) & 1) ^ 1];
                st_rec2(rw + 2 * (size_t)c, pack_rec(u_own, tag), pack_rec(v_own, tag));
                if (REMOTE && rq0) {
                    const int parw = ((k + par0) & 1) ^ 1;
                    const v4u a = pack_rec(u_own, tag), b = pack_rec(v_own, tag);
                    st_rec2_sys(rq0 + (size_t)parw * rqs0, a, b);
                    if (rq1) st_rec2_sys(rq1 + (size_t)parw * rqs1, a, b);
                    if (rq2) st_rec2_sys(rq2 + (size_t)parw * rqs2, a, b);
                }
                v4u ra, rb;
                unsigned spins = 0;
                bool ok = true;
                if (REMOTE) t_wait0 = wall_clock64();
                if (seam_remote) {
                    ok = poll_remote(rw + 2 * (size_t)seam_partner, tag, ra, rb, 3, seam_partner);
                    if (!ok) s_bad = 1;
                } else
                for (;;) {
                    ld_rec2(rw + 2 * (size_t)seam_partner, ra, rb);
                    if (ra.x == tag && ra.w == tag && rb.x == tag && rb.w == tag) break;
                    if (gave_up(++spins, t_wait0)) {
                        give_up_note(3, k, seam_partner, ra.x, tag);
                        ok = false;
                        break;
                    }
                    __builtin_amdgcn_s_sleep(1);
                }
                if (ok) {
                    const double pu = unpack_rec(ra), pv = unpack_rec(rb);
                    if (seam_role == 1) {
                        u_own = 0.5 * (u_own + isign * pu);
                        v_own = 0.5 * (v_own + isign * pv);
                    } else {
                        u_own = isign * (0.5 * (pu + isign * u_own));
                        v_own = isign * (0.5 * (pv + isign * v_own));
                    }
                }
            }
        }
        if (isU || isSeam) { s_u[li] = u_own; s_v[li] = v_own; }
        if (LEAN && ownU) {
            const unsigned tag = want + 1u;
            if (pub) st_rec2_s(wr, own_off, pack_rec(u_own, tag), pack_rec(v_own, tag));
            if (img0 >= 0) st_rec2_s(wr, img_off0, pack_rec(img_sg0 * u_own, tag), pack_rec(img_sg0 * v_own, tag));
            if (img1 >= 0) st_rec2_s(wr, img_off1, pack_rec(img_sg1 * u_own, tag), pack_rec(img_sg1 * v_own, tag));
            if (img2 >= 0) st_rec2_s(wr, img_off2, pack_rec(img_sg2 * u_own, tag), pack_rec(img_sg2 * v_own, tag));
        } else if (ownU && !published) {
            const unsigned tag = want + 1u;
            if (pub) st_rec2(wr + 2 * (size_t)c, pack_rec(u_own, tag), pack_rec(v_own, tag));
            if (img0 >= 0) { const double sg = (img0 & 1) ? -1.0 : 1.0; st_rec2(wr + 2 * (size_t)(img0 >> 1), pack_rec(sg * u_own, tag), pack_rec(sg * v_own, tag)); }
            if (img1 >= 0) { const double sg = (img1 & 1) ? -1.0 : 1.0; st_rec2(wr + 2 * (size_t)(img1 >> 1), pack_rec(sg * u_own, tag), pack_rec(sg * v_own, tag)); }
            if (img2 >= 0) { const double sg = (img2 & 1) ? -1.0 : 1.0; st_rec2(wr + 2 * (size_t)(img2 >> 1), pack_rec(sg * u_own, tag), pack_rec(sg * v_own, tag)); }
        }
        if (rpub && !published) publish_remote(((k + par0) & 1) ^ 1, u_own, v_own, want + 1u);
        EVP_STAMP(pacc3)
        if (split) __syncthreads();
        EVP_STAMP(pacc4)
        return true;
    };
    const bool rimw = RIMU && __builtin_amdgcn_readfirstlane(tq >> 6) == 0;
    typename MM::UP upre;
    auto ucell_operands = [&](typename MM::UI &q) {
        q.uold = u_own; q.vold = v_own;
        q.vrelfac = s_uc[0 * 256 + t]; q.uocn = s_uc[1 * 256 + t]; q.vocn = s_uc[2 * 256 + t];
        q.forcex = s_uc[3 * 256 + t]; q.forcey = s_uc[4 * 256 + t]; q.Umassdti = s_uc[5 * 256 + t];
        q.fm = s_uc[6 * 256 + t]; q.uarear = s_uc[7 * 256 + t];
        q.waterx = q.uocn; q.watery = q.vocn;
        q.TbU = 0.0; q.uvel_init = 0.0; q.vvel_init = 0.0;
    };
    if constexpr (RIMU) if (rimw && isU) {
        typename MM::UI q;
        ucell_operands(q);
        MM::template stepu_pre<CAP, false>(A.p, q, upre);
    }
    auto subcycle_rim = [&](const int k, const v4u *rd, v4u *wr) -> bool {
        const unsigned want = R.tag_base + (unsigned)k;
        const int done = k + 1;
        if ((RES_DBG(R) & 8) && (tile & 3) == 1) {
            const unsigned long long t0 = wall_clock64();
            while (wall_clock64() - t0 < 1000ull) __builtin_amdgcn_s_sleep(8);
        }
        int bad = 0;
        if (rimw) {
            bool gave = false;
            if (ring_cp >= 0 && !(RES_DBG(R) & 2)) {
                v4u ra, rb;
                unsigned spins = 0;
                for (;;) {
                    ld_rec2_s(rd, ring_off, ra, rb);
                    if ((ra.x == want && ra.w == want && rb.x == want && rb.w == want) || (RES_DBG(R) & 1)) break;
                    if (gave_up(++spins, t_wait0)) {
                        give_up_note(1, k, ring_cp, ra.x, want);
                        __hip_atomic_store(&s_bad, 1, __ATOMIC_RELAXED, __HIP_MEMORY_SCOPE_WORKGROUP);
                        gave = true;
                        break;
                    }
                    if (RES_DBG(R) & 4) __builtin_amdgcn_s_sleep(8); else __builtin_amdgcn_s_sleep(1);
                }
                s_u[ring_li] = unpack_rec(ra);
                s_v[ring_li] = unpack_rec(rb);
            }
            __builtin_amdgcn_fence(__ATOMIC_RELEASE, "wavefront");
            __builtin_amdgcn_wave_barrier();
            __builtin_amdgcn_fence(__ATOMIC_ACQUIRE, "wavefront");
            bad = __builtin_amdgcn_ballot_w64(gave) != 0;
        }
        int slots_seen = 0;
        if (rimw && !bad) {
            const int a0 = __hip_atomic_load(&s_slot[0], __ATOMIC_RELAXED, __HIP_MEMORY_SCOPE_WORKGROUP);
            const int a1 = __hip_atomic_load(&s_slot[1], __ATOMIC_RELAXED, __HIP_MEMORY_SCOPE_WORKGROUP);
            const int a2 = __hip_atomic_load(&s_slot[2], __ATOMIC_RELAXED, __HIP_MEMORY_SCOPE_WORKGROUP);
            slots_seen = __builtin_amdgcn_readfirstlane(min(a0, min(a1, a2))) >= done;
            __builtin_amdgcn_fence(__ATOMIC_ACQUIRE, "workgroup");
        }
        EVP_STAMP(pacc0)
        if (!bad) {
            if (actT) {
                double str[8];
                a.u_ij = s_u[li]; a.v_ij = s_v[li];
                a.u_im = s_u[li - 1]; a.v_im = s_v[li - 1];
                a.u_jm = s_u[li - LW]; a.v_jm = s_v[li - LW];
                a.u_mm = s_u[li - LW - 1]; a.v_mm = s_v[li - LW - 1];
                a.strength = s_tc[0 * 256 + t]; a.DminTarea = s_tc[1 * 256 + t];
                a.dxhy = s_tc[2 * 256 + t]; a.dyhx = s_tc[3 * 256 + t];
                MM::template stress<CAP>(A.p, a, s, str);
                s_str[0 * SP + sp] = str[2];
                s_str[1 * SP + sp] = str[5];
                s_str[2 * SP + sp] = str[3];
                s_str[3 * SP + sp] = str[7];
                s_str[4 * SP + sp] = str[1];
                s_str[5 * SP + sp] = str[6];
                s_str[6 * SP + sp] = str[0];
                s_str[7 * SP + sp] = str[4];
            }
            EVP_STAMP(pacc1)
            __builtin_amdgcn_fence(__ATOMIC_RELEASE, "workgroup");
            if (!rimw && (t & 63) == 0) __hip_atomic_store(&s_slot[(tq >> 6) - 1], done, __ATOMIC_RELAXED, __HIP_MEMORY_SCOPE_WORKGROUP);
            if (!slots_seen) {
                unsigned spins = 0;
                for (;;) {
                    const int a0 = __hip_atomic_load(&s_slot[0], __ATOMIC_RELAXED, __HIP_MEMORY_SCOPE_WORKGROUP);
                    const int a1 = __hip_atomic_load(&s_slot[1], __ATOMIC_RELAXED, __HIP_MEMORY_SCOPE_WORKGROUP);
                    const int a2 = __hip_atomic_load(&s_slot[2], __ATOMIC_RELAXED, __HIP_MEMORY_SCOPE_WORKGROUP);
                    const int lo = __builtin_amdgcn_readfirstlane(min(a0, min(a1, a2)));
                    if (lo >= done) break;
                    if (++spins > R.spin_limit) {
                        give_up_note(5, k, -1, (unsigned)lo, (unsigned)done);
                        __hip_atomic_store(&s_bad, 1, __ATOMIC_RELAXED, __HIP_MEMORY_SCOPE_WORKGROUP);
                    }
                    if ((spins & 255u) == 0 || spins > R.spin_limit)
                        bad = __builtin_amdgcn_readfirstlane(__hip_atomic_load(&s_bad, __ATOMIC_RELAXED, __HIP_MEMORY_SCOPE_WORKGROUP));
                    if (bad) break;
                    __builtin_amdgcn_s_sleep(1);
                }
            }
            __builtin_amdgcn_fence(__ATOMIC_ACQUIRE, "workgroup");
            EVP_STAMP(pacc2)
        }
        if (!bad) {
            double fin0 = 0.0, fin1 = 0.0, fin2 = 0.0, fin3 = 0.0;
            if (isU) {
                typename MM::UI q;
                typename MM::UO o;
                ucell_operands(q);
                q.sx0 = s_str[6 * SP + usp]; q.sx1 = s_str[4 * SP + usp + 1];
                q.sx2 = s_str[0 * SP + usp + SW]; q.sx3 = s_str[2 * SP + usp + SW + 1];
                q.sy0 = s_str[7 * SP + usp]; q.sy1 = s_str[1 * SP + usp + SW];
                q.sy2 = s_str[5 * SP + usp + 1]; q.sy3 = s_str[3 * SP + usp + SW + 1];
                if (!rimw) MM::template stepu_pre<CAP, false>(A.p, q, upre);
                MM::template stepu_post<CAP>(A.p, q, upre, o);
                u_own = o.u; v_own = o.v;
                fin0 = o.strintx; fin1 = o.strinty; fin2 = o.taubx; fin3 = o.tauby;
            }
            if (ownU) {
                const unsigned tag = want + 1u;
                if (pub) st_rec2_s(wr, own_off, pack_rec(u_own, tag), pack_rec(v_own, tag));
                if (img0 >= 0) st_rec2_s(wr, img_off0, pack_rec(img_sg0 * u_own, tag), pack_rec(img_sg0 * v_own, tag));
                if (img1 >= 0) st_rec2_s(wr, img_off1, pack_rec(img_sg1 * u_own, tag), pack_rec(img_sg1 * v_own, tag));
                if (img2 >= 0) st_rec2_s(wr, img_off2, pack_rec(img_sg2 * u_own, tag), pack_rec(img_sg2 * v_own, tag));
            }
            if (isU) {
                s_u[uli] = u_own; s_v[uli] = v_own;
                if (k == R.ndte - 1 && !R.dry) {
                    R.tab[24][cu] = fin0; R.tab[25][cu] = fin1;
                    R.tab[26][cu] = fin2; R.tab[27][cu] = fin3;
                }
            }
            EVP_STAMP(pacc3)
        }
        __syncthreads();
        EVP_STAMP(pacc4)
        if (s_bad) return false;
        if (rimw && isU) {
            typename MM::UI q;
            ucell_operands(q);
            MM::template stepu_pre<CAP, false>(A.p, q, upre);
        }
        return true;
    };
    if constexpr (RIMU) {
        const v4u *const rec_a = (const v4u *)R.rec[par0 & 1];
        v4u *const rec_b = (v4u *)R.rec[(par0 & 1) ^ 1];
        for (int k = 0; k < R.ndte; k += 2) {
            if (!subcycle_rim(k, rec_a, rec_b)) return;
            if (k + 1 == R.ndte) break;
            if (!subcycle_rim(k + 1, rec_b, (v4u *)rec_a)) return;
        }
    } else
    if (LEAN) {
        const v4u *const rec_a = (const v4u *)R.rec[par0 & 1];
        v4u *const rec_b = (v4u *)R.rec[(par0 & 1) ^ 1];
        for (int k = 0; k < R.ndte; k += 2) {
            if (!subcycle(k, rec_a, rec_b)) return;
            if (k + 1 == R.ndte) break;
            if (!subcycle(k + 1, rec_b, (v4u *)rec_a)) return;
        }
    } else {
        for (int k = 0; k < R.ndte; ++k)
            if (!subcycle(k, (const v4u *)R.rec[(k + par0) & 1], (v4u *)R.rec[((k + par0) & 1) ^ 1])) return;
    }
#undef EVP_STAMP
    if (prof && (t & 63) == 0) {
        unsigned long long *o = R.prof + ((size_t)tile * 4 + (tq >> 6)) * 8;
        o[0] = pacc0; o[1] = pacc1; o[2] = pacc2; o[3] = pacc3; o[4] = pacc4;
        o[5] = (unsigned long long)cu_rank | ((unsigned long long)(PERM && R.cuload ? s_cu : 0) << 8) | ((unsigned long long)(s_simd[t >> 6] & 3) << 24);
        o[6] = (unsigned long long)(t >> 6); o[7] = (unsigned long long)R.nact[tile];
    }
    if (REMOTE && ring_remote) {
        v4u ra, rb;
        const v4u *rd = (const v4u *)R.rec[(R.ndte + par0) & 1];
        const bool ok = poll_remote(rd + 2 * (size_t)ring_cp, R.tag_base + (unsigned)R.ndte, ra, rb);
        if (ok && !R.dry) {
#pragma unroll
            for (int b = 0; b < 2; ++b) { R.u[b][ring_cp] = unpack_rec(ra); R.v[b][ring_cp] = unpack_rec(rb); }
        }
    }

    if (!R.dry) {
        if (actN && own) {
#pragma unroll
            for (int k = 0; k < 12; ++k) {
                R.tab[k][c] = s[k];
                R.tab[12 + k][c] = s[k];
            }
        }
        if (quad && gown) {
            R.tab[qc][gc] = sr0; R.tab[12 + qc][gc] = sr0;
            R.tab[4 + qc][gc] = sr1; R.tab[16 + qc][gc] = sr1;
            R.tab[8 + qc][gc] = sr2; R.tab[20 + qc][gc] = sr2;
        }
        if (isU || isSeam) {
#pragma unroll
            for (int b = 0; b < 2; ++b) {
                double *uu = R.u[b], *vv = R.v[b];
                uu[cu] = u_own; vv[cu] = v_own;
                if (img0 >= 0) { const double sg = (img0 & 1) ? -1.0 : 1.0; uu[img0 >> 1] = sg * u_own; vv[img0 >> 1] = sg * v_own; }
                if (img1 >= 0) { const double sg = (img1 & 1) ? -1.0 : 1.0; uu[img1 >> 1] = sg * u_own; vv[img1 >> 1] = sg * v_own; }
                if (img2 >= 0) { const double sg = (img2 & 1) ? -1.0 : 1.0; uu[img2 >> 1] = sg * u_own; vv[img2 >> 1] = sg * v_own; }
            }
        }
    }
}

size_t lds_bytes(unsigned flags, int logw, bool coop = false, bool rimu = false)
{
    const int W = 1 << logw, H = 256 / W;
    const int nuv = ((H + 1) * (W + 1) + 7) & ~7;
    const int nu = 8 + ((flags & EVP_F_WATER_IS_OCN) ? 0 : 2) + ((flags & EVP_F_TBU_ZERO) ? 0 : 1);
    const size_t nstr = logw == 4 ? (rimu ? 8 : 6) * (size_t)(W + 1) * H : 4 * (size_t)256;
    return sizeof(double) * (nstr + (size_t)256 * (4 + nu) + 2 * (size_t)nuv + (coop ? 12 * (size_t)64 : 0));
}

template <int LOGW, bool REMOTE>
int occ(bool strict, int cap, size_t lds)
{
    int nb = 0;
#define EVP_OCC(S, C) hipOccupancyMaxActiveBlocksPerMultiprocessor(&nb, evp_resident2_tile<S, C, LOGW, REMOTE>, 64 * RTY, lds)
    hipError_t e;
    if (strict) e = cap == 3 ? EVP_OCC(true, 3) : cap == 1 ? EVP_OCC(true, 1) : cap == 0 ? EVP_OCC(true, 0) : EVP_OCC(true, -1);
    else e = cap == 3 ? EVP_OCC(false, 3) : cap == 1 ? EVP_OCC(false, 1) : cap == 0 ? EVP_OCC(false, 0) : EVP_OCC(false, -1);
#undef EVP_OCC
    return e == hipSuccess ? nb : 0;
}

template <int LOGW, bool REMOTE>
void launch(const EvpArgs &A, const EvpResident2 &R, bool strict, int cap, hipStream_t st)
{
    dim3 grid(R.nlaunch > 0 ? R.nlaunch : A.ntiles), block(64, RTY);
    const size_t lds = lds_bytes(A.flags, LOGW);
#define EVP_LAUNCH(S, C) hipLaunchKernelGGL((evp_resident2_tile<S, C, LOGW, REMOTE>), grid, block, lds, st, A, R)
    if (strict) {
        if (cap == 3) EVP_LAUNCH(true, 3);
        else if (cap == 1) EVP_LAUNCH(true, 1);
        else if (cap == 0) EVP_LAUNCH(true, 0);
        else EVP_LAUNCH(true, -1);
    } else {
        if (cap == 3) EVP_LAUNCH(false, 3);
        else if (cap == 1) EVP_LAUNCH(false, 1);
        else if (cap == 0) EVP_LAUNCH(false, 0);
        else EVP_LAUNCH(false, -1);
    }
#undef EVP_LAUNCH
}

}

void evp_resident_geometry(int max_ni, int max_nj, int logw, int *gx, int *gy)
{
    const int W = 1 << logw, H = 256 / W;
    *gx = (max_ni + W - 2) / (W - 1);
    *gy = (max_nj + H - 2) / (H - 1);
}

bool evp_resident2_lean_built(bool, int cap, int logw, bool remote) { return cap == 3 && logw == 4 && !remote; }

#ifdef CICE_EVP_HIP_TESTING
bool evp_resident2_coop_built(bool strict, int cap, int logw, bool remote) { return strict && cap == 3 && logw == 4 && !remote; }
#else
bool evp_resident2_coop_built(bool, int, int, bool) { return false; }
#endif

int evp_resident2_max_blocks_per_cu(bool strict, int cap, unsigned flags, int logw, bool remote, bool coop)
{
    if (coop) {
#ifdef CICE_EVP_HIP_TESTING
        if (!evp_resident2_coop_built(strict, cap, logw, remote)) return 0;
        int nb = 0;
        return hipOccupancyMaxActiveBlocksPerMultiprocessor(&nb, evp_resident2_tile<true, 3, 4, false, true>, 64 * RTY, lds_bytes(flags, 4, true)) == hipSuccess ? nb : 0;
#else
        return 0;
#endif
    }
    const size_t lds = lds_bytes(flags, logw);
    if (evp_resident2_lean_built(strict, cap, logw, remote)) {
        int nb = 0;
        const hipError_t e = strict ? hipOccupancyMaxActiveBlocksPerMultiprocessor(&nb, evp_resident2_tile<true, 3, 4, false, false, true>, 64 * RTY, lds)
                                    : hipOccupancyMaxActiveBlocksPerMultiprocessor(&nb, evp_resident2_tile<false, 3, 4, false, false, true>, 64 * RTY, lds);
        int nr = 0;
        const size_t lds_r = lds_bytes(flags | EVP_F_WATER_IS_OCN | EVP_F_TBU_ZERO, 4, false, true);
        const hipError_t er = strict ? hipOccupancyMaxActiveBlocksPerMultiprocessor(&nr, evp_resident2_tile<true, 3, 4, false, false, true, true>, 64 * RTY, lds_r)
                                     : hipOccupancyMaxActiveBlocksPerMultiprocessor(&nr, evp_resident2_tile<false, 3, 4, false, false, true, true>, 64 * RTY, lds_r);
        return e == hipSuccess && er == hipSuccess ? std::min(std::min(nb, nr), occ<4, false>(strict, cap, lds)) : 0;
    }
    if (remote) return logw == 4 ? occ<4, true>(strict, cap, lds) : logw == 5 ? occ<5, true>(strict, cap, lds) : occ<6, true>(strict, cap, lds);
    return logw == 4 ? occ<4, false>(strict, cap, lds) : logw == 5 ? occ<5, false>(strict, cap, lds) : occ<6, false>(strict, cap, lds);
}

void evp_launch_resident2(const EvpArgs &A0, const EvpResident2 &R, int max_ni, int max_nj, int logw,
                          bool strict, int cap, int lean, hipStream_t st)
{
    EvpArgs A = A0;
    evp_resident_geometry(max_ni, max_nj, logw, &A.gx, &A.gy);
    A.ntiles = A.gx * A.gy * (R.nblocks > 0 ? R.nblocks : 1);
    const bool remote = R.rimg != nullptr;
#ifdef CICE_EVP_HIP_TESTING
    if (R.nlate && evp_resident2_coop_built(strict, cap, logw, remote)) {
        dim3 grid(R.nlaunch > 0 ? R.nlaunch : A.ntiles), block(64, RTY);
        hipLaunchKernelGGL((evp_resident2_tile<true, 3, 4, false, true>), grid, block, lds_bytes(A.flags, 4, true), st, A, R);
        return;
    }
#endif
    if (lean == 2 && evp_resident2_lean_built(strict, cap, logw, remote)) {
        dim3 grid(R.nlaunch > 0 ? R.nlaunch : A.ntiles), block(64, RTY);
        const size_t lds = lds_bytes(A.flags, 4, false, true);
        if (strict) hipLaunchKernelGGL((evp_resident2_tile<true, 3, 4, false, false, true, true>), grid, block, lds, st, A, R);
        else hipLaunchKernelGGL((evp_resident2_tile<false, 3, 4, false, false, true, true>), grid, block, lds, st, A, R);
        return;
    }
    if (lean && evp_resident2_lean_built(strict, cap, logw, remote)) {
        dim3 grid(R.nlaunch > 0 ? R.nlaunch : A.ntiles), block(64, RTY);
        if (strict) hipLaunchKernelGGL((evp_resident2_tile<true, 3, 4, false, false, true>), grid, block, lds_bytes(A.flags, 4), st, A, R);
        else hipLaunchKernelGGL((evp_resident2_tile<false, 3, 4, false, false, true>), grid, block, lds_bytes(A.flags, 4), st, A, R);
        return;
    }
    if (remote) {
        if (logw == 4) launch<4, true>(A, R, strict, cap, st);
        else if (logw == 5) launch<5, true>(A, R, strict, cap, st);
        else launch<6, true>(A, R, strict, cap, st);
    } else {
        if (logw == 4) launch<4, false>(A, R, strict, cap, st);
        else if (logw == 5) launch<5, false>(A, R, strict, cap, st);
        else launch<6, false>(A, R, strict, cap, st);
    }
}
```

### cice_amd/evp.py

```python
from __future__ import annotations

import ctypes as C
import os
from pathlib import Path

import numpy as np

HERE = Path(__file__).resolve().parent
LIB_PATH = Path(os.environ["CICE_EVP_HIP_LIBRARY"]) if os.environ.get("CICE_EVP_HIP_LIBRARY") else HERE / "libcice_evp_hip.so"
LIB_TESTING_PATH = HERE / "libcice_evp_hip_testing.so"

BND = {"closed": 0, "open": 1, "cyclic": 2, "tripole": 3, "tripoleT": 4}

FIELDS = [
    "stressp_1", "stressp_2", "stressp_3", "stressp_4",
    "stressm_1", "stressm_2", "stressm_3", "stressm_4",
    "stress12_1", "stress12_2", "stress12_3", "stress12_4",
    "strength", "cdn_ocnU", "aiU", "uocnU", "vocnU", "waterxU", "wateryU",
    "forcexU", "forceyU", "umassdti", "fmU", "strintxU", "strintyU", "TbU",
    "taubxU", "taubyU", "uvel", "vvel", "uvel_init", "vvel_init",
]
OUTPUTS = FIELDS[:12] + ["strintxU", "strintyU", "taubxU", "taubyU", "uvel", "vvel"]
EXPORTS = [
    "cice_evp_hip_abi_version", "cice_evp_hip_last_error", "cice_evp_hip_init",
    "cice_evp_hip_set_metrics", "cice_evp_hip_run", "cice_evp_hip_finalize",
    "cice_evp_hip_upload", "cice_evp_hip_subcycle", "cice_evp_hip_download", "cice_evp_hip_sync",
    "cice_evp_hip_comm_unique_id", "cice_evp_hip_comm_init", "cice_evp_hip_comm_info", "cice_evp_hip_get_timings",
    "cice_evp_hip_time_kernels", "cice_evp_hip_mark", "cice_evp_hip_seam_fin_plan",
    "cice_evp_hip_cgrid_set_prep_geometry", "cice_evp_hip_cgrid_prep", "cice_evp_hip_cgrid_seabed_lkd", "cice_evp_hip_cgrid_seabed_prob",
    "cice_evp_hip_cgrid_prep_finish", "cice_evp_hip_cgrid_fetch", "cice_evp_hip_cgrid_set_tb", "cice_evp_hip_describe_path",
    "cice_evp_hip_pin_host", "cice_evp_hip_set_post_geometry", "cice_evp_hip_deformations", "cice_evp_hip_dyn_finish",
    "cice_evp_hip_halo_export", "cice_evp_hip_halo_import", "cice_evp_hip_stress_halo", "cice_evp_hip_stress_halo_available", 
    "cice_evp_hip_set_prep_geometry", "cice_evp_hip_prep", "cice_evp_hip_set_strength", "cice_evp_hip_set_tbu", "cice_evp_hip_seabed_lkd", "cice_evp_hip_seabed_prob", "cice_evp_hip_halo_mask", "cice_evp_hip_march_info", "cice_evp_hip_prep_fetch",
    "cice_evp_hip_set_forcing_layout",
    "cice_evp_hip_addr", "cice_evp_hip_set_option", "cice_evp_hip_fetch_stresses", "cice_evp_hip_invalidate_stresses",
    "cice_evp_hip_cgrid_set_geometry", "cice_evp_hip_cgrid_run", "cice_evp_hip_cgrid_upload", "cice_evp_hip_cgrid_subcycle",
    "cice_evp_hip_cgrid_download", "cice_evp_hip_cgrid_sync", "cice_evp_hip_cgrid_deformations", "cice_evp_hip_cgrid_dyn_finish", "cice_evp_hip_cgrid_timings", "cice_evp_hip_stream_probe", 
]
TEST_EXPORTS = [
    "cice_evp_hip_cgrid_fold_plan", "cice_evp_hip_cgrid_window_plan", "cice_evp_hip_cgrid_window_plan_ext", "cice_evp_hip_cgrid_window_deps", "cice_evp_hip_cgrid_strip_plan", "cice_evp_hip_cgrid_strip_zones", "cice_evp_hip_cgrid_frame_plan", "cice_evp_hip_cgrid_march_fold_plan", "cice_evp_hip_set_test_transport", "cice_evp_hip_march_plan", "cice_evp_hip_march_fold_plan",
    "cice_evp_hip_debug_device_allocs", "cice_evp_hip_debug_cuload", "cice_evp_hip_debug_prof", "cice_evp_hip_debug_cgrid_prof", "cice_evp_hip_debug_cgres_prof", "cice_evp_hip_plan_build", "cice_evp_hip_halo_plan", "cice_evp_hip_seam_plan",
    "cice_evp_hip_peer_plan", "cice_evp_hip_peer_signs", "cice_evp_hip_center_plan", "cice_evp_hip_stress_plan",
    "cice_evp_hip_fold_split_plan", "cice_evp_hip_plan_flags", "cice_evp_hip_fold_images_plan", "cice_evp_hip_cgrid_fold_xplan",
    "cice_evp_hip_cgrid_fold_xpeers", "cice_evp_hip_plan_dump", "cice_evp_hip_rim_plan",
]
TEST_ENV = [
    "CICE_EVP_HIP_RES_REMOTE", "CICE_EVP_HIP_RES_REMOTE_BREAK", "CICE_EVP_HIP_RES_ORDER", "CICE_EVP_HIP_RES_PROF", "CICE_EVP_HIP_RES_DEBUG",
    "CICE_EVP_HIP_MARCH_OWN", "CICE_EVP_HIP_MARCH_SELFX", "CICE_EVP_HIP_MARCH_SEG", "CICE_EVP_HIP_MARCH_ORDER",
    "CICE_EVP_HIP_MARCH_LEAN", "CICE_EVP_HIP_MARCH_K", "CICE_EVP_HIP_CGRID_SPLIT", "CICE_EVP_HIP_CGRID_XCD", "CICE_EVP_HIP_CGRID_ONE_XCD", "CICE_EVP_HIP_CGRID_ONE_SHAPE",
    "CICE_EVP_HIP_CGRID_ONE_STRIP", "CICE_EVP_HIP_CGRID_FAST", "CICE_EVP_HIP_HALO_DEBUG", "CICE_EVP_HIP_SEAM_FIN", "CICE_EVP_HIP_OVERLAP",
    "CICE_EVP_HIP_HALO_RIDE", "CICE_EVP_HIP_GATHER", "CICE_EVP_HIP_SIMPLE", "CICE_EVP_HIP_SELF_EXCHANGE", "CICE_EVP_HIP_FLAGS", "CICE_EVP_HIP_LEAN",
    "CICE_EVP_HIP_PREFETCH", "CICE_EVP_HIP_FAULT_REPLAY", "CICE_EVP_HIP_MARCH_BANDSEG", "CICE_EVP_HIP_CGRID_PROF",
    "CICE_EVP_HIP_NO_OVERLAP", "CICE_EVP_HIP_TYB", "CICE_EVP_HIP_NOGRAPH", "CICE_EVP_HIP_GRAPH_RCCL", "CICE_EVP_HIP_RES_LOGW", "CICE_EVP_HIP_RES_COOP", "CICE_EVP_HIP_RES_LEAN", "CICE_EVP_HIP_RES_RIMU",
    "CICE_EVP_HIP_MARCH_EXT", "CICE_EVP_HIP_MARCH_DIRECT", "CICE_EVP_HIP_CGRID_FUSED", "CICE_EVP_HIP_CGRID_GEO",
    "CICE_EVP_HIP_CGRID_RES_SLEEP", "CICE_EVP_HIP_CGRID_RES_CULL", "CICE_EVP_HIP_CGRID_RES_DEBUG",
    "CICE_EVP_HIP_CGRID_STRIP", "CICE_EVP_HIP_CGRID_STRIP_SEG", "CICE_EVP_HIP_CGRID_STRIP_EDGE", "CICE_EVP_HIP_CGRID_STRIP_RIDE", "CICE_EVP_HIP_CGRID_STRIP_LEN", "CICE_EVP_HIP_CGRID_STRIP_ITEMS", "CICE_EVP_HIP_CGRID_STRIP_LAST",
    "CICE_EVP_HIP_CGRID_MARCH_RESERVE", "CICE_EVP_HIP_CGRID_MARCH_RANKS", "CICE_EVP_HIP_CGRID_MARCH_FOLD", "CICE_EVP_HIP_CGRID_MARCH_FOLD_SERIAL",
]
CGRID_FIELDS = ["uvelE", "vvelE", "uvelN", "vvelN", "uvel", "vvel", "stresspT", "stressmT", "stress12T", "stress12U",
                "strintxE", "strintyN", "taubxE", "taubyN", "zetax2T", "etax2T", "etax2U", "shearU", "deltaU"]
CGRID_INPUTS = ["strength", "cdn_ocnE", "aiE", "uocnE", "vocnE", "waterxE", "forcexE", "emassdti", "fmE", "uvelE_init",
                "TbE", "rheofactE", "cdn_ocnN", "aiN", "uocnN", "vocnN", "wateryN", "forceyN", "nmassdti", "fmN",
                "vvelN_init", "TbN", "rheofactN"]
CGRID_STATIC = ["dxT", "dyT", "dxU", "dyU", "dxE", "dyE", "dxN", "dyN", "uarea", "tarea", "earea", "narea", "earear",
                "narear", "epm", "npm", "uvm", "hm", "DminTarea", "ratiodxN", "ratiodxNr", "ratiodyE", "ratiodyEr"]
CGRID_MASKS = ["iceTmask", "iceUmask", "iceEmask", "iceNmask"]
VISC_METHOD = {"avg_zeta": 0, "avg_strength": 1}
HALO_BLOB = 1024
OPT_STRESS_RESIDENT = 1
PREP_T = ["aice", "vice", "vsno", "aice_init", "cdn_ocn", "uocn", "vocn", "ss_tltx", "ss_tlty",
          "strairxT", "strairyT"]
PREP_FETCH = ["aiU", "cdn_ocnU", "uocnU", "vocnU", "umassdti", "fmU", "waterxU", "wateryU", "forcexU",
              "forceyU", "uvel_init", "vvel_init", "strtltxU", "strtltyU", "strairxU", "strairyU",
              "tmass", "umass", "uvel", "vvel"]
PREP_FETCH_MORE = {"TbU": 20}
PREP_FETCH_TESTING = {"ss_tltxU": 21, "ss_tltyU": 22}
CGRID_FORCING_PRODUCTS = ["strairxE", "strairyN", "ss_tltxE", "ss_tltyN"]
LOC = {"T": 0, "U": 1, "E": 2, "N": 3, "NE": 4}
GRID_LOC = {"A": ("T", "T"), "B": ("U", "U"), "C": ("E", "N"), "CD": ("NE", "NE")}


class PrepParams(C.Structure):
    _fields_ = [("dt", C.c_double), ("rhoi", C.c_double), ("rhos", C.c_double), ("gravit", C.c_double),
                ("dyn_area_min", C.c_double), ("dyn_mass_min", C.c_double), ("ssh_stress_coupled", C.c_int32)]

_i32p = C.POINTER(C.c_int32)
_f64p = C.POINTER(C.c_double)


class EvpHipError(RuntimeError):
    """Raised where the Fortran wrapper would call abort_ice(...)."""


class Dims(C.Structure):
    _fields_ = [("nx_block", C.c_int32), ("ny_block", C.c_int32), ("nblocks", C.c_int32),
                ("max_blocks", C.c_int32), ("nghost", C.c_int32), ("nx_global", C.c_int32),
                ("ny_global", C.c_int32), ("ew_boundary_type", C.c_int32),
                ("ns_boundary_type", C.c_int32), ("rank", C.c_int32), ("nranks", C.c_int32),
                ("ilo", _i32p), ("ihi", _i32p), ("jlo", _i32p), ("jhi", _i32p),
                ("iglob0", _i32p), ("jglob0", _i32p), ("nblocks_tot", C.c_int32),
                ("gi0", _i32p), ("gj0", _i32p), ("gnx", _i32p), ("gny", _i32p),
                ("gowner", _i32p), ("glocal", _i32p)]


class Params(C.Structure):
    _fields_ = [("ndte", C.c_int32), ("strict", C.c_int32)] + [(n, C.c_double) for n in (
        "arlx1i", "denom1", "brlx", "revp", "e_factor", "epp2i", "capping", "Ktens",
        "deltaminEVP", "u0", "cosw", "sinw", "rhow")]


_lib = None
_lib_testing = None


def testing_wanted() -> bool:
    return any(k in os.environ for k in TEST_ENV)


def load_library(path: os.PathLike | None = None, testing: bool = False) -> C.CDLL:
    global _lib, _lib_testing
    if path is None:
        if testing and _lib_testing is not None:
            return _lib_testing
        if not testing and _lib is not None:
            return _lib
    p = Path(path) if path else (LIB_TESTING_PATH if testing else LIB_PATH)
    if not p.exists():
        raise EvpHipError(f"{p} not found: build it with `python -c 'import __graft_entry__ as g; g.build()'` "
                          "(hipcc --offload-arch=gfx950); there is no CPU fallback")
    lib = C.CDLL(str(p), mode=C.RTLD_LOCAL)
    for name in EXPORTS + (TEST_EXPORTS if testing else []):
        getattr(lib, name).restype = C.c_int
    lib.cice_evp_hip_addr.restype = C.c_void_p
    if path is None:
        if testing:
            _lib_testing = lib
# ... 639 lines not shown
                to_block=(int(v[5]), int(v[6])), to_rect=(int(v[7]), int(v[8])), rect_rows=int(v[9]), tile_rows=tr[:int(dims.nblocks)])


def halo_plan(dims: Dims) -> dict:
    lib = load_library(testing=True)
    _check(lib, lib.cice_evp_hip_plan_build(C.byref(dims)), "(plan_build)")
    cnt = np.zeros(4, dtype=np.int32)
    lib.cice_evp_hip_halo_plan(_ip(cnt), None, None, None, None, None, None, None, None)
    nl, npeer, ns, nr = [int(v) for v in cnt]
    ld, ls, lg = [np.zeros(max(nl, 1), dtype=np.int32) for _ in range(3)]
    pr, pns, pnr = [np.zeros(max(npeer, 1), dtype=np.int32) for _ in range(3)]
    ss = np.zeros(max(ns, 1), dtype=np.int32)
    rd = np.zeros(max(nr, 1), dtype=np.int32)
    lib.cice_evp_hip_halo_plan(_ip(cnt), _ip(ld), _ip(ls), _ip(lg), _ip(pr), _ip(pns), _ip(pnr), _ip(ss), _ip(rd))
    c3 = np.zeros(3, dtype=np.int32)
    lib.cice_evp_hip_seam_plan(_ip(c3), None, None, None, None, None, None)
    npair, npole, nlate = [int(v) for v in c3]
    sa, sb = [np.zeros(max(npair, 1), dtype=np.int32) for _ in range(2)]
    sp = np.zeros(max(npole, 1), dtype=np.int32)
    td, ts, tg = [np.zeros(max(nlate, 1), dtype=np.int32) for _ in range(3)]
    lib.cice_evp_hip_seam_plan(_ip(c3), _ip(sa), _ip(sb), _ip(sp), _ip(td), _ip(ts), _ip(tg))
    c1 = np.zeros(1, dtype=np.int32)
    lib.cice_evp_hip_stress_plan(_ip(c1), None, None)
    nst = int(c1[0])
    std, sts = [np.zeros(max(nst, 1), dtype=np.int32) for _ in range(2)]
    lib.cice_evp_hip_stress_plan(_ip(c1), _ip(std), _ip(sts))
    lib.cice_evp_hip_center_plan(_ip(c1), None, None, None)
    ncen = int(c1[0])
    cd, cs, cv = [np.zeros(max(ncen, 1), dtype=np.int32) for _ in range(3)]
    center_remote = lib.cice_evp_hip_center_plan(_ip(c1), _ip(cd), _ip(cs), _ip(cv)) == 1
    sd = np.zeros(max(ns, 1), dtype=np.int32)
    rg = np.zeros(max(nr, 1), dtype=np.int32)
    lib.cice_evp_hip_peer_plan(_ip(sd), _ip(rg))
    rsg = np.zeros(max(nr, 1), dtype=np.int32)
    lib.cice_evp_hip_peer_signs(_ip(rsg))
    c2 = np.zeros(2, dtype=np.int32)
    stress_remote = lib.cice_evp_hip_seam_fin_plan(_ip(c2), None, None, None, None) == 1
    nfin, tail = int(c2[0]), int(c2[1])
    fd, fa, fb, fc = [np.zeros(max(nfin, 1), dtype=np.int32) for _ in range(4)]
    lib.cice_evp_hip_seam_fin_plan(_ip(c2), _ip(fd), _ip(fa), _ip(fb), _ip(fc))
    c4 = np.zeros((max(npeer, 1), 4), dtype=np.int32)
    lib.cice_evp_hip_fold_images_plan(_ip(c4), None, None, None)
    ssg = np.zeros(max(ns, 1), dtype=np.int32)
    fo = np.zeros((max(int(c4[:, 2].sum()), 1), 3), dtype=np.int32)
    fi = np.zeros((max(int(c4[:, 3].sum()), 1), 3), dtype=np.int32)
    lib.cice_evp_hip_fold_images_plan(_ip(c4), _ip(ssg), _ip(fo), _ip(fi))
    fl = np.zeros(5, dtype=np.int32)
    lib.cice_evp_hip_plan_flags(_ip(fl), 5)
    return dict(peer_counts4=c4[:npeer], send_sign=ssg[:ns], fimg_out=fo[:int(c4[:npeer, 2].sum())], fimg_in=fi[:int(c4[:npeer, 3].sum())],
                any_fold_exchange=bool(fl[0]), fold_rows=int(fl[1]), fin_dst=fd[:nfin], fin_a=fa[:nfin], fin_b=fb[:nfin], fin_coef=fc[:nfin], tail=tail, stress_remote=stress_remote, recv_sign=rsg[:nr],
                stress_dst=std[:nst], stress_src=sts[:nst], send_dst=sd[:ns], recv_gid=rg[:nr],
                center_dst=cd[:ncen], center_src=cs[:ncen], center_vsign=cv[:ncen], center_remote=center_remote,
                local_dst=ld[:nl], local_src=ls[:nl], local_sign=lg[:nl], peer_rank=pr[:npeer],
                peer_nsend=pns[:npeer], peer_nrecv=pnr[:npeer], send_src=ss[:ns], recv_dst=rd[:nr],
                seam_a=sa[:npair], seam_b=sb[:npair], seam_pole=sp[:npole],
                late_dst=td[:nlate], late_src=ts[:nlate], late_sign=tg[:nlate])


def halo_plan_dump(dims: Dims) -> np.ndarray:
    lib = load_library(testing=True)
    _check(lib, lib.cice_evp_hip_plan_build(C.byref(dims)), "(plan_build)")
    out = np.zeros(lib.cice_evp_hip_plan_dump(None, 0), dtype=np.int32)
    n = lib.cice_evp_hip_plan_dump(_ip(out), len(out))
    if n != len(out):
        _check(lib, n if n < 0 else -1, "(plan_dump)")
    return out


def rim_plan(ni: int, nj: int, mask: np.ndarray, cyclic_ew: bool = False, cyclic_ns: bool = False) -> dict:
    lib = load_library(testing=True)
    mask = np.ascontiguousarray(mask, dtype=np.uint8)
    assert mask.shape == (nj + 2, ni + 2), mask.shape
    u8 = lambda a: a.ctypes.data_as(C.POINTER(C.c_uint8))
    nt = lib.cice_evp_hip_rim_plan(ni, nj, int(cyclic_ew), int(cyclic_ns), u8(mask), 0, None, None, None, None)
    if nt < 0:
        _check(lib, nt, "(rim_plan)")
    perm, uperm, cls = (np.zeros((nt, 256), dtype=np.uint8) for _ in range(3))
    info = np.zeros((nt, 8), dtype=np.int32)
    rc = lib.cice_evp_hip_rim_plan(ni, nj, int(cyclic_ew), int(cyclic_ns), u8(mask), nt, u8(perm), u8(uperm), _ip(info), u8(cls))
    if rc != nt:
        _check(lib, rc if rc < 0 else -1, "(rim_plan)")
    return dict(perm=perm, uperm=uperm, cls=cls, n_lt=info[:, 0], n_lu=info[:, 1], nact=info[:, 2], nact_packed=info[:, 3],
                ok=info[:, 4].astype(bool), gx=int(info[0, 5]), gy=int(info[0, 6]))
```

### include/cice_evp_hip_testing.h

```cpp
#ifndef CICE_EVP_HIP_TESTING_H
#define CICE_EVP_HIP_TESTING_H

#include "cice_evp_hip.h"

#ifdef __cplusplus
extern "C" {
#endif

int cice_evp_hip_cgrid_fold_plan(const cice_evp_hip_dims *dims, int32_t loc, int32_t *count, int32_t *dst, int32_t *a,
                                 int32_t *b, int32_t *flip);
int cice_evp_hip_cgrid_window_plan(const cice_evp_hip_dims *dims, int32_t ox, int32_t oy, int32_t *ntiles, int32_t *tiles4, int32_t *tab);
int cice_evp_hip_cgrid_window_plan_ext(const cice_evp_hip_dims *dims, int32_t ox, int32_t oy, int32_t extra, int32_t *ntiles,
                                       int32_t *tiles4, int32_t *tab);
int cice_evp_hip_cgrid_window_deps(const cice_evp_hip_dims *dims, int32_t *n_windows, int32_t *n_edges, int32_t *n_oneway, int32_t *n_unsafe);
int cice_evp_hip_cgrid_strip_plan(const cice_evp_hip_dims *dims, int32_t ex, int32_t ey, int32_t lo0, int32_t slots, int32_t seg_min, int32_t seg,
                                  int32_t *n_items, int32_t *items6, int32_t items_cap, int32_t *n_windows, int32_t *tiles4, uint8_t *in_zone, int32_t windows_cap,
                                  int32_t *seg_rows);
int cice_evp_hip_cgrid_strip_zones(const cice_evp_hip_dims *dims, int32_t ex, int32_t ey, int32_t *n_zones, int32_t *zones10, int32_t zones_cap);
int cice_evp_hip_cgrid_frame_plan(const cice_evp_hip_dims *dims, int32_t ex, int32_t ey, int32_t lo0, int32_t slots, int32_t seg_min, int32_t seg,
                                  int64_t *info6, uint8_t *cells, int32_t *wg, int32_t wg_cap, int32_t *items6, int32_t items_cap);
int cice_evp_hip_cgrid_march_fold_plan(const cice_evp_hip_dims *dims, int32_t ex, int32_t ey, int32_t slots, int32_t seg_min, int32_t seg, int32_t len,
                                       int64_t *info11, uint8_t *cells, int32_t *wg, int32_t wg_cap, int32_t *items6, int32_t items_cap);
typedef int (*cice_evp_hip_test_xchg_fn)(void *user, int32_t npeers, const int32_t *peer_rank, const int64_t *send_count,
                                         const int64_t *recv_count, const double *send, double *recv);
typedef int (*cice_evp_hip_test_reduce_fn)(void *user, int32_t op, void *value);
int cice_evp_hip_set_test_transport(cice_evp_hip_test_xchg_fn xchg, cice_evp_hip_test_reduce_fn reduce, void *user);
int cice_evp_hip_march_plan(const cice_evp_hip_dims *dims, int32_t own_max, int32_t wrap_inside, int32_t ext, int32_t *geo14,
                            int32_t *peer_rank, int32_t *peer_nsend, int32_t *peer_nrecv, int32_t *send_pos,
                            int32_t *recv_pos1, int32_t *recv_pos2);
int cice_evp_hip_march_fold_plan(const cice_evp_hip_dims *dims, int32_t ext, int32_t tyb, int32_t *out10, int32_t *tile_rows);
int cice_evp_hip_debug_cuload(int32_t *out, int32_t n);
int cice_evp_hip_debug_prof(uint64_t *out, int32_t ntiles_max);
int cice_evp_hip_debug_cgrid_prof(uint64_t *out, int32_t ntiles_max);
int cice_evp_hip_debug_cgres_prof(uint64_t *out, int32_t ntiles_max);
int cice_evp_hip_debug_device_allocs(int64_t *count);
int cice_evp_hip_plan_build(const cice_evp_hip_dims *dims);
int cice_evp_hip_plan_dump(int32_t *out, int32_t n);
int cice_evp_hip_rim_plan(int32_t ni, int32_t nj, int32_t cyclic_ew, int32_t cyclic_ns, const uint8_t *mask, int32_t ntiles_max,
                          uint8_t *perm, uint8_t *uperm, int32_t *info8, uint8_t *cls);
int cice_evp_hip_halo_plan(int32_t *counts4, int32_t *local_dst, int32_t *local_src,
                           int32_t *local_sign, int32_t *peer_rank, int32_t *peer_nsend,
                           int32_t *peer_nrecv, int32_t *send_src, int32_t *recv_dst);

int cice_evp_hip_seam_plan(int32_t *counts3, int32_t *seam_a, int32_t *seam_b, int32_t *seam_pole,
                           int32_t *late_dst, int32_t *late_src, int32_t *late_sign);
int cice_evp_hip_peer_plan(int32_t *send_dst, int32_t *recv_gid);
int cice_evp_hip_fold_images_plan(int32_t *counts4, int32_t *send_sign, int32_t *out3, int32_t *in3);
int cice_evp_hip_peer_signs(int32_t *recv_sign);
int cice_evp_hip_center_plan(int32_t *count, int32_t *dst, int32_t *src, int32_t *vsign);
int cice_evp_hip_stress_plan(int32_t *count, int32_t *dst, int32_t *src);
int cice_evp_hip_fold_split_plan(int32_t which, int32_t *count, int32_t *cells);
int cice_evp_hip_plan_flags(int32_t *flags, int32_t n);
int cice_evp_hip_cgrid_fold_xplan(int32_t loc, int32_t *info4, int32_t *count, int32_t *dst, int32_t *a, int32_t *b, int32_t *flip);
int cice_evp_hip_cgrid_fold_xpeers(int32_t *peer5, int32_t *send_src, int32_t *send_dst, int32_t *recv_dst, int32_t *recv_gid);


#ifdef __cplusplus
}
#endif
#endif
```

Baseline: 32.39 billion.

## Use range-checked core sqrt and division paths in EVP stress and stepu

Adds a range-math policy that checks whether Delta² and the division operands fall inside a safe exponent range for the whole wavefront. When they do, it uses cheaper core sqrt and division sequences that skip the library's special-case handling, and otherwise it falls back to the library calls. The aim is to cut the expensive fp64 sqrt/div instruction sequences in the stress and momentum updates. The cost is a wave-uniform vote, duplicated code paths that raise register pressure, and reliance on the range proof for bitwise parity. It appears to be gated by a new CICE_EVP_HIP_RES_RANGE environment variable.

```diff
diff --git a/__graft_entry__.py b/__graft_entry__.py
--- a/__graft_entry__.py
+++ b/__graft_entry__.py
@@ -21,7 +21,7 @@
 HIP_SRCS = ["evp_kernels.hip", "evp_resident2.hip", "evp_halo_direct.hip", "evp_prep.hip",
             "evp_copy.hip", "evp_cgrid.hip", "evp_cgrid_res.hip", "evp_cgrid_prep.hip", "evp_march.hip", "evp_api.cpp", "evp_host_common.cpp", "evp_host_loop.cpp",
             "evp_host_resident.cpp", "evp_host_mailbox.cpp", "evp_host_prep.cpp", "evp_host_cgrid.cpp", "evp_host_march.cpp", "march_plan.cpp", "halo_plan.cpp", "cgrid_plan.cpp", "rim_plan.cpp"]
-HIP_HDRS = ["evp_cell.inc", "evp_device.h", "evp_forcing.h", "evp_math.h", "halo_plan.h", "cgrid_plan.h", "evp_host.h", "evp_halo_direct.h", "march_plan.h", "rim_plan.h"]
+HIP_HDRS = ["evp_cell.inc", "evp_device.h", "evp_forcing.h", "evp_math.h", "evp_range_math.h", "halo_plan.h", "cgrid_plan.h", "evp_host.h", "evp_halo_direct.h", "march_plan.h", "rim_plan.h"]
 
 
 LIB_TESTING = ROOT / "cice_amd" / "libcice_evp_hip_testing.so"
diff --git a/cice_amd/csrc/evp_api.cpp b/cice_amd/csrc/evp_api.cpp
--- a/cice_amd/csrc/evp_api.cpp
+++ b/cice_amd/csrc/evp_api.cpp
@@ -1039,6 +1039,30 @@
     return P.fold_split ? 1 : 0;
 }
 
+int cice_evp_hip_debug_range_math(int64_t n, const double *x, const double *num, const double *den, double *sqrt_lib, double *sqrt_core,
+                                  double *div_lib, double *div_core, uint8_t *verdict)
+{
+    if (n < 1 || n > ((int64_t)1 << 26) || !x || !num || !den || !sqrt_lib || !sqrt_core || !div_lib || !div_core || !verdict)
+        return fail(-1, "debug_range_math: bad argument");
+    const size_t nb = (size_t)n * sizeof(double);
+    double *d = nullptr;
+    unsigned char *dv = nullptr;
+    HIPC(hipMalloc((void **)&d, 7 * nb));
+    hipError_t e = hipMalloc((void **)&dv, (size_t)n);
+    if (e == hipSuccess) e = hipMemcpy(d, x, nb, hipMemcpyHostToDevice);
+    if (e == hipSuccess) e = hipMemcpy(d + n, num, nb, hipMemcpyHostToDevice);
+    if (e == hipSuccess) e = hipMemcpy(d + 2 * n, den, nb, hipMemcpyHostToDevice);
+    if (e == hipSuccess) e = evp_range_math_probe((long long)n, d, d + n, d + 2 * n, d + 3 * n, d + 4 * n, d + 5 * n, d + 6 * n, dv, nullptr);
+    if (e == hipSuccess) e = hipDeviceSynchronize();
+    double *outs[4] = {sqrt_lib, sqrt_core, div_lib, div_core};
+    for (int k = 0; k < 4 && e == hipSuccess; ++k) e = hipMemcpy(outs[k], d + (3 + k) * n, nb, hipMemcpyDeviceToHost);
+    if (e == hipSuccess) e = hipMemcpy(verdict, dv, (size_t)n, hipMemcpyDeviceToHost);
+    (void)hipFree(d);
+    if (dv) (void)hipFree(dv);
+    if (e != hipSuccess) return fail(-2, "debug_range_math: %s", hipGetErrorString(e));
+    return 0;
+}
+
 int cice_evp_hip_stress_plan(int32_t *count, int32_t *dst, int32_t *src)
 {
     const size_t n = copy_out(dst, S.plan.stress_dst);
diff --git a/cice_amd/csrc/evp_cell.inc b/cice_amd/csrc/evp_cell.inc
--- a/cice_amd/csrc/evp_cell.inc
+++ b/cice_amd/csrc/evp_cell.inc
@@ -18,13 +18,16 @@
     a.DminTarea = deltaminEVP * tarea;
 }
 
-template <int CAP, bool SIMPLE = false>
+template <int CAP, bool SIMPLE = false, bool CORE = false>
 __device__ __forceinline__ void visc_replpress(const EvpScalars &p, double strength, double DminArea,
                                                double Delta, double &zetax2, double &etax2,
                                                double &rep_prs)
 {
+    static_assert(!CORE || CAP == 1, "the range-proved division is instantiated for capping == 1 only");
     double tmpcalc;
-    if (CAP == 1) {
+    if (CORE) {
+        tmpcalc = evp_range::div_core(strength, fmax(Delta, DminArea));
+    } else if (CAP == 1) {
         tmpcalc = strength / fmax(Delta, DminArea);
     } else if (CAP == 0) {
         tmpcalc = strength / (Delta + DminArea);
@@ -42,9 +45,302 @@
     etax2 = p.epp2i * zetax2;
 }
 
+template <int CAP, bool SIMPLE = false, class POL = evp_range::LibMath>
+__device__ __forceinline__ void stress_cell(const EvpScalars &p, const StressIn &a, double (&s)[12],
+                                            double (&str)[8], const POL &pol = POL())
+{
+    const double divune = a.cyp * a.u_ij - a.dyT * a.u_im + a.cxp * a.v_ij - a.dxT * a.v_jm;
+    const double divunw = a.cym * a.u_im + a.dyT * a.u_ij + a.cxp * a.v_im - a.dxT * a.v_mm;
+    const double divusw = a.cym * a.u_mm + a.dyT * a.u_jm + a.cxm * a.v_mm + a.dxT * a.v_im;
+    const double divuse = a.cyp * a.u_jm - a.dyT * a.u_mm + a.cxm * a.v_jm + a.dxT * a.v_ij;
+    const double tensionne = -a.cym * a.u_ij - a.dyT * a.u_im + a.cxm * a.v_ij + a.dxT * a.v_jm;
+    const double tensionnw = -a.cyp * a.u_im + a.dyT * a.u_ij + a.cxm * a.v_im + a.dxT * a.v_mm;
+    const double tensionsw = -a.cyp * a.u_mm + a.dyT * a.u_jm + a.cxp * a.v_mm - a.dxT * a.v_im;
+    const double tensionse = -a.cym * a.u_jm - a.dyT * a.u_mm + a.cxp * a.v_jm - a.dxT * a.v_ij;
+    const double shearne = -a.cym * a.v_ij - a.dyT * a.v_im - a.cxm * a.u_ij - a.dxT * a.u_jm;
+    const double shearnw = -a.cyp * a.v_im + a.dyT * a.v_ij - a.cxm * a.u_im - a.dxT * a.u_mm;
+    const double shearsw = -a.cyp * a.v_mm + a.dyT * a.v_jm - a.cxp * a.u_mm + a.dxT * a.u_im;
+    const double shearse = -a.cym * a.v_jm - a.dyT * a.v_mm - a.cxp * a.u_jm + a.dxT * a.u_ij;
+    double zetax2ne, etax2ne, rep_prsne, zetax2nw, etax2nw, rep_prsnw;
+    double zetax2sw, etax2sw, rep_prssw, zetax2se, etax2se, rep_prsse;
+    if constexpr (POL::ranged) {
+        using namespace evp_range;
+        const double Delta2ne = divune * divune + p.e_factor * (tensionne * tensionne + shearne * shearne);
+        const double Delta2nw = divunw * divunw + p.e_factor * (tensionnw * tensionnw + shearnw * shearnw);
+        const double Delta2sw = divusw * divusw + p.e_factor * (tensionsw * tensionsw + shearsw * shearsw);
+        const double Delta2se = divuse * divuse + p.e_factor * (tensionse * tensionse + shearse * shearse);
+        bool cores;
+        const unsigned far = umax(umax(off_pos(Delta2ne), off_pos(Delta2nw)), umax(off_pos(Delta2sw), off_pos(Delta2se)));
+        cores = pol.wave_inside(outside(far), true);
+        if (cores) {
+            const double Deltane = sqrt_core(Delta2ne), Deltanw = sqrt_core(Delta2nw);
+            const double Deltasw = sqrt_core(Delta2sw), Deltase = sqrt_core(Delta2se);
+            visc_replpress<CAP, SIMPLE, true>(p, a.strength, a.DminTarea, Deltane, zetax2ne, etax2ne, rep_prsne);
+            visc_replpress<CAP, SIMPLE, true>(p, a.strength, a.DminTarea, Deltanw, zetax2nw, etax2nw, rep_prsnw);
+            visc_replpress<CAP, SIMPLE, true>(p, a.strength, a.DminTarea, Deltasw, zetax2sw, etax2sw, rep_prssw);
+            visc_replpress<CAP, SIMPLE, true>(p, a.strength, a.DminTarea, Deltase, zetax2se, etax2se, rep_prsse);
+        } else {
+            const double Deltane = sqrt(Delta2ne), Deltanw = sqrt(Delta2nw);
+            const double Deltasw = sqrt(Delta2sw), Deltase = sqrt(Delta2se);
+            visc_replpress<CAP, SIMPLE>(p, a.strength, a.DminTarea, Deltane, zetax2ne, etax2ne, rep_prsne);
+            visc_replpress<CAP, SIMPLE>(p, a.strength, a.DminTarea, Deltanw, zetax2nw, etax2nw, rep_prsnw);
+            visc_replpress<CAP, SIMPLE>(p, a.strength, a.DminTarea, Deltasw, zetax2sw, etax2sw, rep_prssw);
+            visc_replpress<CAP, SIMPLE>(p, a.strength, a.DminTarea, Deltase, zetax2se, etax2se, rep_prsse);
+        }
+    } else {
+    const double Deltane = sqrt(divune * divune + p.e_factor * (tensionne * tensionne + shearne * shearne));
+    const double Deltanw = sqrt(divunw * divunw + p.e_factor * (tensionnw * tensionnw + shearnw * shearnw));
+    const double Deltasw = sqrt(divusw * divusw + p.e_factor * (tensionsw * tensionsw + shearsw * shearsw));
+    const double Deltase = sqrt(divuse * divuse + p.e_factor * (tensionse * tensionse + shearse * shearse));
+    visc_replpress<CAP, SIMPLE>(p, a.strength, a.DminTarea, Deltane, zetax2ne, etax2ne, rep_prsne);
+    visc_replpress<CAP, SIMPLE>(p, a.strength, a.DminTarea, Deltanw, zetax2nw, etax2nw, rep_prsnw);
+    visc_replpress<CAP, SIMPLE>(p, a.strength, a.DminTarea, Deltasw, zetax2sw, etax2sw, rep_prssw);
+    visc_replpress<CAP, SIMPLE>(p, a.strength, a.DminTarea, Deltase, zetax2se, etax2se, rep_prsse);
+    }
+
+    const double arlx1i = p.arlx1i, revp = p.revp, denom1 = p.denom1;
+    if (SIMPLE) {
+        s[0] = (s[0] + arlx1i * (zetax2ne * divune - rep_prsne)) * denom1;
+        s[1] = (s[1] + arlx1i * (zetax2nw * divunw - rep_prsnw)) * denom1;
+        s[2] = (s[2] + arlx1i * (zetax2sw * divusw - rep_prssw)) * denom1;
+        s[3] = (s[3] + arlx1i * (zetax2se * divuse - rep_prsse)) * denom1;
+
+        s[4] = (s[4] + arlx1i * etax2ne * tensionne) * denom1;
+        s[5] = (s[5] + arlx1i * etax2nw * tensionnw) * denom1;
+        s[6] = (s[6] + arlx1i * etax2sw * tensionsw) * denom1;
+        s[7] = (s[7] + arlx1i * etax2se * tensionse) * denom1;
+
+        s[8] = (s[8] + arlx1i * p5 * etax2ne * shearne) * denom1;
+        s[9] = (s[9] + arlx1i * p5 * etax2nw * shearnw) * denom1;
+        s[10] = (s[10] + arlx1i * p5 * etax2sw * shearsw) * denom1;
+        s[11] = (s[11] + arlx1i * p5 * etax2se * shearse) * denom1;
+    } else {
+    s[0] = (s[0] * (1.0 - arlx1i * revp) + arlx1i * (zetax2ne * divune - rep_prsne)) * denom1;
+    s[1] = (s[1] * (1.0 - arlx1i * revp) + arlx1i * (zetax2nw * divunw - rep_prsnw)) * denom1;
+    s[2] = (s[2] * (1.0 - arlx1i * revp) + arlx1i * (zetax2sw * divusw - rep_prssw)) * denom1;
+    s[3] = (s[3] * (1.0 - arlx1i * revp) + arlx1i * (zetax2se * divuse - rep_prsse)) * denom1;
+
+    s[4] = (s[4] * (1.0 - arlx1i * revp) + arlx1i * etax2ne * tensionne) * denom1;
+    s[5] = (s[5] * (1.0 - arlx1i * revp) + arlx1i * etax2nw * tensionnw) * denom1;
+    s[6] = (s[6] * (1.0 - arlx1i * revp) + arlx1i * etax2sw * tensionsw) * denom1;
+    s[7] = (s[7] * (1.0 - arlx1i * revp) + arlx1i * etax2se * tensionse) * denom1;
+
+    s[8] = (s[8] * (1.0 - arlx1i * revp) + arlx1i * p5 * etax2ne * shearne) * denom1;
+    s[9] = (s[9] * (1.0 - arlx1i * revp) + arlx1i * p5 * etax2nw * shearnw) * denom1;
+    s[10] = (s[10] * (1.0 - arlx1i * revp) + arlx1i * p5 * etax2sw * shearsw) * denom1;
+    s[11] = (s[11] * (1.0 - arlx1i * revp) + arlx1i * p5 * etax2se * shearse) * denom1;
+    }
+
+    const double ssigpn = s[0] + s[1];
+    const double ssigps = s[2] + s[3];
+    const double ssigpe = s[0] + s[3];
+    const double ssigpw = s[1] + s[2];
+    const double ssigp1 = (s[0] + s[2]) * p055;
+    const double ssigp2 = (s[1] + s[3]) * p055;
+
+    const double ssigmn = s[4] + s[5];
+    const double ssigms = s[6] + s[7];
+    const double ssigme = s[4] + s[7];
+    const double ssigmw = s[5] + s[6];
+    const double ssigm1 = (s[4] + s[6]) * p055;
+    const double ssigm2 = (s[5] + s[7]) * p055;
+
+    const double ssig12n = s[8] + s[9];
+    const double ssig12s = s[10] + s[11];
+    const double ssig12e = s[8] + s[11];
+    const double ssig12w = s[9] + s[10];
+    const double ssig121 = (s[8] + s[10]) * p111;
+    const double ssig122 = (s[9] + s[11]) * p111;
+
+    const double csigpne = p111 * s[0] + ssigp2 + p027 * s[2];
+    const double csigpnw = p111 * s[1] + ssigp1 + p027 * s[3];
+    const double csigpsw = p111 * s[2] + ssigp2 + p027 * s[0];
+    const double csigpse = p111 * s[3] + ssigp1 + p027 * s[1];
+
+    const double csigmne = p111 * s[4] + ssigm2 + p027 * s[6];
+    const double csigmnw = p111 * s[5] + ssigm1 + p027 * s[7];
+    const double csigmsw = p111 * s[6] + ssigm2 + p027 * s[4];
+    const double csigmse = p111 * s[7] + ssigm1 + p027 * s[5];
+
+    const double csig12ne = p222 * s[8] + ssig122 + p055 * s[10];
+    const double csig12nw = p222 * s[9] + ssig121 + p055 * s[11];
+    const double csig12sw = p222 * s[10] + ssig122 + p055 * s[8];
+    const double csig12se = p222 * s[11] + ssig121 + p055 * s[9];
+
+    const double str12ew = p5 * a.dxT * (p333 * ssig12e + p166 * ssig12w);
+    const double str12we = p5 * a.dxT * (p333 * ssig12w + p166 * ssig12e);
+    const double str12ns = p5 * a.dyT * (p333 * ssig12n + p166 * ssig12s);
+    const double str12sn = p5 * a.dyT * (p333 * ssig12s + p166 * ssig12n);
+
+    double strp_tmp = p25 * a.dyT * (p333 * ssigpn + p166 * ssigps);
+    double strm_tmp = p25 * a.dyT * (p333 * ssigmn + p166 * ssigms);
+    str[0] = -strp_tmp - strm_tmp - str12ew + a.dxhy * (-csigpne + csigmne) + a.dyhx * csig12ne;
+    str[1] = strp_tmp + strm_tmp - str12we + a.dxhy * (-csigpnw + csigmnw) + a.dyhx * csig12nw;
+    strp_tmp = p25 * a.dyT * (p333 * ssigps + p166 * ssigpn);
+    strm_tmp = p25 * a.dyT * (p333 * ssigms + p166 * ssigmn);
+    str[2] = -strp_tmp - strm_tmp + str12ew + a.dxhy * (-csigpse + csigmse) + a.dyhx * csig12se;
+    str[3] = strp_tmp + strm_tmp + str12we + a.dxhy * (-csigpsw + csigmsw) + a.dyhx * csig12sw;
+
+    strp_tmp = p25 * a.dxT * (p333 * ssigpe + p166 * ssigpw);
+    strm_tmp = p25 * a.dxT * (p333 * ssigme + p166 * ssigmw);
+    str[4] = -strp_tmp + strm_tmp - str12ns - a.dyhx * (csigpne + csigmne) + a.dxhy * csig12ne;
+    str[5] = strp_tmp - strm_tmp - str12sn - a.dyhx * (csigpse + csigmse) + a.dxhy * csig12se;
+    strp_tmp = p25 * a.dxT * (p333 * ssigpw + p166 * ssigpe);
+    strm_tmp = p25 * a.dxT * (p333 * ssigmw + p166 * ssigme);
+    str[6] = -strp_tmp + strm_tmp + str12ns - a.dyhx * (csigpnw + csigmnw) + a.dxhy * csig12nw;
+    str[7] = strp_tmp - strm_tmp + str12sn - a.dyhx * (csigpsw + csigmsw) + a.dxhy * csig12sw;
+}
+
+struct CornerIn {
+    double ua, va, ub, vb, ud, vd;
+    double cyA, cyB, cxA, cxB, DY, DX;
+    double strength, DminTarea;
+};
 template <int CAP, bool SIMPLE = false>
-__device__ __forceinline__ void stress_cell(const EvpScalars &p, const StressIn &a, double (&s)[12],
-                                            double (&str)[8])
+__device__ __forceinline__ void stress_corner(const EvpScalars &p, const CornerIn &c, double &sp, double &sm, double &s12)
+{
+    const double divu = c.cyA * c.ua + c.DY * c.ub + c.cxA * c.va + c.DX * c.vd;
+    const double tension = -c.cyB * c.ua + c.DY * c.ub + c.cxB * c.va - c.DX * c.vd;
+    const double shear = -c.cyB * c.va + c.DY * c.vb - c.cxB * c.ua + c.DX * c.ud;
+    const double Delta = sqrt(divu * divu + p.e_factor * (tension * tension + shear * shear));
+    double zetax2, etax2, rep_prs;
+    visc_replpress<CAP, SIMPLE>(p, c.strength, c.DminTarea, Delta, zetax2, etax2, rep_prs);
+    const double arlx1i = p.arlx1i, revp = p.revp, denom1 = p.denom1;
+    if (SIMPLE) {
+        sp = (sp + arlx1i * (zetax2 * divu - rep_prs)) * denom1;
+        sm = (sm + arlx1i * etax2 * tension) * denom1;
+        s12 = (s12 + arlx1i * p5 * etax2 * shear) * denom1;
+    } else {
+        sp = (sp * (1.0 - arlx1i * revp) + arlx1i * (zetax2 * divu - rep_prs)) * denom1;
+        sm = (sm * (1.0 - arlx1i * revp) + arlx1i * etax2 * tension) * denom1;
+        s12 = (s12 * (1.0 - arlx1i * revp) + arlx1i * p5 * etax2 * shear) * denom1;
+    }
+}
+__device__ __forceinline__ void corner_operands(int q, double dxT, double dyT, double cxp, double cyp, double cxm, double cym,
+                                                CornerIn &c, double &KX, double &K12X, double &KYP, double &K12Y)
+{
+    const bool east = q == 0 || q == 3, north = q < 2;
+    c.cyA = east ? cyp : cym; c.cyB = east ? cym : cyp;
+    c.cxA = north ? cxp : cxm; c.cxB = north ? cxm : cxp;
+    c.DY = east ? -dyT : dyT;
+    c.DX = north ? -dxT : dxT;
+    KX = (east ? -p25 : p25) * dyT;
+    K12X = (north ? -p5 : p5) * dxT;
+    KYP = (north ? -p25 : p25) * dxT;
+    K12Y = (east ? -p5 : p5) * dyT;
+}
+__device__ __forceinline__ void stress_corner_partials(double P0, double P1, double P2, double P3, double M0, double M1, double M2,
+                                                       double M3, double T0, double T1, double T2, double T3, double KX, double K12X,
+                                                       double KYP, double K12Y, double dxhy, double dyhx, double &X, double &Y)
+{
+    const double csigp = p111 * P0 + (P1 + P3) * p055 + p027 * P2;
+    const double csigm = p111 * M0 + (M1 + M3) * p055 + p027 * M2;
+    const double csig12 = p222 * T0 + (T1 + T3) * p111 + p055 * T2;
+    const double str12x = K12X * (p333 * (T0 + T3) + p166 * (T1 + T2));
+    const double str12y = K12Y * (p333 * (T0 + T1) + p166 * (T2 + T3));
+    const double strp_x = KX * (p333 * (P0 + P1) + p166 * (P2 + P3));
+    const double strm_x = KX * (p333 * (M0 + M1) + p166 * (M2 + M3));
+    X = strp_x + strm_x + str12x + dxhy * (-csigp + csigm) + dyhx * csig12;
+    const double strp_y = KYP * (p333 * (P0 + P3) + p166 * (P1 + P2));
+    const double strm_y = -KYP * (p333 * (M0 + M3) + p166 * (M1 + M2));
+    Y = strp_y + strm_y + str12y - dyhx * (csigp + csigm) + dxhy * csig12;
+}
+
+struct StepuIn {
+    double uold, vold;
+    double vrelfac;
+    double uocn, vocn, waterx, watery, forcex, forcey, Umassdti, fm, uarear, TbU;
+    double uvel_init, vvel_init;
+    double sx0, sx1, sx2, sx3;
+    double sy0, sy1, sy2, sy3;
+};
+
+struct StepuOut {
+    double u, v, strintx, strinty, taubx, tauby;
+};
+
+struct StepuPre {
+    double taux, tauy, Cb, cca, ccb, ab2;
+    double bu, bv;
+};
+
+template <bool SIMPLE = false, bool TBU = true, bool WITH_B = true, class POL = evp_range::LibMath>
+__device__ __forceinline__ void stepu_pre_cell(const EvpScalars &p, const StepuIn &a, StepuPre &w, const POL &pol = POL())
+{
+    const double uold = a.uold, vold = a.vold;
+    const double du = a.uocn - uold, dv = a.vocn - vold;
+    double vrel;
+    if constexpr (POL::ranged) {
+        const double speed2 = du * du + dv * dv;
+        if (pol.wave_inside(evp_range::outside(evp_range::off_pos(speed2)), false)) vrel = a.vrelfac * evp_range::sqrt_core(speed2);
+        else vrel = a.vrelfac * sqrt(speed2);
+    } else {
+    vrel = a.vrelfac * sqrt(du * du + dv * dv);
+    }
+    w.taux = vrel * a.waterx;
+    w.tauy = vrel * a.watery;
+    double Cb = 0.0;
+    if (TBU) Cb = a.TbU / (sqrt(uold * uold + vold * vold) + p.u0);
+    w.Cb = Cb;
+    double cca, ccb;
+    if (SIMPLE) {
+        cca = p.brlx * a.Umassdti + vrel + Cb;
+        ccb = a.fm;
+    } else {
+        cca = (p.brlx + p.revp) * a.Umassdti + vrel * p.cosw + Cb;
+        ccb = a.fm + copysign(1.0, a.fm) * vrel * p.sinw;
+    }
+    w.cca = cca; w.ccb = ccb;
+    w.ab2 = cca * cca + ccb * ccb;
+    if (!WITH_B) return;
+    if (SIMPLE) {
+        w.bu = p.brlx * uold + 0.0;
+        w.bv = p.brlx * vold + 0.0;
+    } else {
+        w.bu = p.brlx * uold + p.revp * a.uvel_init;
+        w.bv = p.brlx * vold + p.revp * a.vvel_init;
+    }
+}
+
+template <bool SIMPLE = false, bool WITH_B = true, class POL = evp_range::LibMath>
+__device__ __forceinline__ void stepu_post_cell(const EvpScalars &p, const StepuIn &a, const StepuPre &w, StepuOut &o)
+{
+    o.strintx = a.uarear * (a.sx0 + a.sx1 + a.sx2 + a.sx3);
+    o.strinty = a.uarear * (a.sy0 + a.sy1 + a.sy2 + a.sy3);
+    double cc1, cc2;
+    if (WITH_B) {
+        cc1 = o.strintx + a.forcex + w.taux + a.Umassdti * w.bu;
+        cc2 = o.strinty + a.forcey + w.tauy + a.Umassdti * w.bv;
+    } else if (SIMPLE) {
+        cc1 = o.strintx + a.forcex + w.taux + a.Umassdti * (p.brlx * a.uold + 0.0);
+        cc2 = o.strinty + a.forcey + w.tauy + a.Umassdti * (p.brlx * a.vold + 0.0);
+    } else {
+        cc1 = o.strintx + a.forcex + w.taux + a.Umassdti * (p.brlx * a.uold + p.revp * a.uvel_init);
+        cc2 = o.strinty + a.forcey + w.tauy + a.Umassdti * (p.brlx * a.vold + p.revp * a.vvel_init);
+    }
+    o.u = (w.cca * cc1 + w.ccb * cc2) / w.ab2;
+    o.v = (w.cca * cc2 - w.ccb * cc1) / w.ab2;
+    if (POL::lazy_taub) return;
+    o.taubx = -o.u * w.Cb;
+    o.tauby = -o.v * w.Cb;
+}
+
+template <bool SIMPLE = false, bool TBU = true, class POL = evp_range::LibMath>
+__device__ __forceinline__ void stepu_cell(const EvpScalars &p, const StepuIn &a, StepuOut &o, const POL &pol = POL())
+{
+    StepuPre w;
+    stepu_pre_cell<SIMPLE, TBU, false, POL>(p, a, w, pol);
+    stepu_post_cell<SIMPLE, false>(p, a, w, o);
+}
+
+struct DeformOut {
+    double divu, shear, vort, rdg_conv, rdg_shear;
+};
+
+__device__ __forceinline__ void deform_cell(const EvpScalars &p, const StressIn &a, double tarear,
+                                            double dyU_ij, double dyU_im, double dyU_jm, double dyU_mm,
+                                            double dxU_ij, double dxU_im, double dxU_jm, double dxU_mm,
+                                            DeformOut &o)
 {
     const double divune = a.cyp * a.u_ij - a.dyT * a.u_im + a.cxp * a.v_ij - a.dxT * a.v_jm;
     const double divunw = a.cym * a.u_im + a.dyT * a.u_ij + a.cxp * a.v_im - a.dxT * a.v_mm;
@@ -63,266 +359,6 @@
     const double Deltasw = sqrt(divusw * divusw + p.e_factor * (tensionsw * tensionsw + shearsw * shearsw));
     const double Deltase = sqrt(divuse * divuse + p.e_factor * (tensionse * tensionse + shearse * shearse));
 
-    double zetax2ne, etax2ne, rep_prsne, zetax2nw, etax2nw, rep_prsnw;
-    double zetax2sw, etax2sw, rep_prssw, zetax2se, etax2se, rep_prsse;
-    visc_replpress<CAP, SIMPLE>(p, a.strength, a.DminTarea, Deltane, zetax2ne, etax2ne, rep_prsne);
-    visc_replpress<CAP, SIMPLE>(p, a.strength, a.DminTarea, Deltanw, zetax2nw, etax2nw, rep_prsnw);
-    visc_replpress<CAP, SIMPLE>(p, a.strength, a.DminTarea, Deltasw, zetax2sw, etax2sw, rep_prssw);
-    visc_replpress<CAP, SIMPLE>(p, a.strength, a.DminTarea, Deltase, zetax2se, etax2se, rep_prsse);
-
-    const double arlx1i = p.arlx1i, revp = p.revp, denom1 = p.denom1;
-    if (SIMPLE) {
-        s[0] = (s[0] + arlx1i * (zetax2ne * divune - rep_prsne)) * denom1;
-        s[1] = (s[1] + arlx1i * (zetax2nw * divunw - rep_prsnw)) * denom1;
-        s[2] = (s[2] + arlx1i * (zetax2sw * divusw - rep_prssw)) * denom1;
-        s[3] = (s[3] + arlx1i * (zetax2se * divuse - rep_prsse)) * denom1;
-
-        s[4] = (s[4] + arlx1i * etax2ne * tensionne) * denom1;
-        s[5] = (s[5] + arlx1i * etax2nw * tensionnw) * denom1;
-        s[6] = (s[6] + arlx1i * etax2sw * tensionsw) * denom1;
-        s[7] = (s[7] + arlx1i * etax2se * tensionse) * denom1;
-
-        s[8] = (s[8] + arlx1i * p5 * etax2ne * shearne) * denom1;
-        s[9] = (s[9] + arlx1i * p5 * etax2nw * shearnw) * denom1;
-        s[10] = (s[10] + arlx1i * p5 * etax2sw * shearsw) * denom1;
-        s[11] = (s[11] + arlx1i * p5 * etax2se * shearse) * denom1;
-    } else {
-    s[0] = (s[0] * (1.0 - arlx1i * revp) + arlx1i * (zetax2ne * divune - rep_prsne)) * denom1;
-    s[1] = (s[1] * (1.0 - arlx1i * revp) + arlx1i * (zetax2nw * divunw - rep_prsnw)) * denom1;
-    s[2] = (s[2] * (1.0 - arlx1i * revp) + arlx1i * (zetax2sw * divusw - rep_prssw)) * denom1;
-    s[3] = (s[3] * (1.0 - arlx1i * revp) + arlx1i * (zetax2se * divuse - rep_prsse)) * denom1;
-
-    s[4] = (s[4] * (1.0 - arlx1i * revp) + arlx1i * etax2ne * tensionne) * denom1;
-    s[5] = (s[5] * (1.0 - arlx1i * revp) + arlx1i * etax2nw * tensionnw) * denom1;
-    s[6] = (s[6] * (1.0 - arlx1i * revp) + arlx1i * etax2sw * tensionsw) * denom1;
-    s[7] = (s[7] * (1.0 - arlx1i * revp) + arlx1i * etax2se * tensionse) * denom1;
-
-    s[8] = (s[8] * (1.0 - arlx1i * revp) + arlx1i * p5 * etax2ne * shearne) * denom1;
-    s[9] = (s[9] * (1.0 - arlx1i * revp) + arlx1i * p5 * etax2nw * shearnw) * denom1;
-    s[10] = (s[10] * (1.0 - arlx1i * revp) + arlx1i * p5 * etax2sw * shearsw) * denom1;
-    s[11] = (s[11] * (1.0 - arlx1i * revp) + arlx1i * p5 * etax2se * shearse) * denom1;
-    }
-
-    const double ssigpn = s[0] + s[1];
-    const double ssigps = s[2] + s[3];
-    const double ssigpe = s[0] + s[3];
-    const double ssigpw = s[1] + s[2];
-    const double ssigp1 = (s[0] + s[2]) * p055;
-    const double ssigp2 = (s[1] + s[3]) * p055;
-
-    const double ssigmn = s[4] + s[5];
-    const double ssigms = s[6] + s[7];
-    const double ssigme = s[4] + s[7];
-    const double ssigmw = s[5] + s[6];
-    const double ssigm1 = (s[4] + s[6]) * p055;
-    const double ssigm2 = (s[5] + s[7]) * p055;
-
-    const double ssig12n = s[8] + s[9];
-    const double ssig12s = s[10] + s[11];
-    const double ssig12e = s[8] + s[11];
-    const double ssig12w = s[9] + s[10];
-    const double ssig121 = (s[8] + s[10]) * p111;
-    const double ssig122 = (s[9] + s[11]) * p111;
-
-    const double csigpne = p111 * s[0] + ssigp2 + p027 * s[2];
-    const double csigpnw = p111 * s[1] + ssigp1 + p027 * s[3];
-    const double csigpsw = p111 * s[2] + ssigp2 + p027 * s[0];
-    const double csigpse = p111 * s[3] + ssigp1 + p027 * s[1];
-
-    const double csigmne = p111 * s[4] + ssigm2 + p027 * s[6];
-    const double csigmnw = p111 * s[5] + ssigm1 + p027 * s[7];
-    const double csigmsw = p111 * s[6] + ssigm2 + p027 * s[4];
-    const double csigmse = p111 * s[7] + ssigm1 + p027 * s[5];
-
-    const double csig12ne = p222 * s[8] + ssig122 + p055 * s[10];
-    const double csig12nw = p222 * s[9] + ssig121 + p055 * s[11];
-    const double csig12sw = p222 * s[10] + ssig122 + p055 * s[8];
-    const double csig12se = p222 * s[11] + ssig121 + p055 * s[9];
-
-    const double str12ew = p5 * a.dxT * (p333 * ssig12e + p166 * ssig12w);
-    const double str12we = p5 * a.dxT * (p333 * ssig12w + p166 * ssig12e);
-    const double str12ns = p5 * a.dyT * (p333 * ssig12n + p166 * ssig12s);
-    const double str12sn = p5 * a.dyT * (p333 * ssig12s + p166 * ssig12n);
-
-    double strp_tmp = p25 * a.dyT * (p333 * ssigpn + p166 * ssigps);
-    double strm_tmp = p25 * a.dyT * (p333 * ssigmn + p166 * ssigms);
-    str[0] = -strp_tmp - strm_tmp - str12ew + a.dxhy * (-csigpne + csigmne) + a.dyhx * csig12ne;
-    str[1] = strp_tmp + strm_tmp - str12we + a.dxhy * (-csigpnw + csigmnw) + a.dyhx * csig12nw;
-    strp_tmp = p25 * a.dyT * (p333 * ssigps + p166 * ssigpn);
-    strm_tmp = p25 * a.dyT * (p333 * ssigms + p166 * ssigmn);
-    str[2] = -strp_tmp - strm_tmp + str12ew + a.dxhy * (-csigpse + csigmse) + a.dyhx * csig12se;
-    str[3] = strp_tmp + strm_tmp + str12we + a.dxhy * (-csigpsw + csigmsw) + a.dyhx * csig12sw;
-
-    strp_tmp = p25 * a.dxT * (p333 * ssigpe + p166 * ssigpw);
-    strm_tmp = p25 * a.dxT * (p333 * ssigme + p166 * ssigmw);
-    str[4] = -strp_tmp + strm_tmp - str12ns - a.dyhx * (csigpne + csigmne) + a.dxhy * csig12ne;
-    str[5] = strp_tmp - strm_tmp - str12sn - a.dyhx * (csigpse + csigmse) + a.dxhy * csig12se;
-    strp_tmp = p25 * a.dxT * (p333 * ssigpw + p166 * ssigpe);
-    strm_tmp = p25 * a.dxT * (p333 * ssigmw + p166 * ssigme);
-    str[6] = -strp_tmp + strm_tmp + str12ns - a.dyhx * (csigpnw + csigmnw) + a.dxhy * csig12nw;
-    str[7] = strp_tmp - strm_tmp + str12sn - a.dyhx * (csigpsw + csigmsw) + a.dxhy * csig12sw;
-}
-
-struct CornerIn {
-    double ua, va, ub, vb, ud, vd;
-    double cyA, cyB, cxA, cxB, DY, DX;
-    double strength, DminTarea;
-};
-template <int CAP, bool SIMPLE = false>
-__device__ __forceinline__ void stress_corner(const EvpScalars &p, const CornerIn &c, double &sp, double &sm, double &s12)
-{
-    const double divu = c.cyA * c.ua + c.DY * c.ub + c.cxA * c.va + c.DX * c.vd;
-    const double tension = -c.cyB * c.ua + c.DY * c.ub + c.cxB * c.va - c.DX * c.vd;
-    const double shear = -c.cyB * c.va + c.DY * c.vb - c.cxB * c.ua + c.DX * c.ud;
-    const double Delta = sqrt(divu * divu + p.e_factor * (tension * tension + shear * shear));
-    double zetax2, etax2, rep_prs;
-    visc_replpress<CAP, SIMPLE>(p, c.strength, c.DminTarea, Delta, zetax2, etax2, rep_prs);
-    const double arlx1i = p.arlx1i, revp = p.revp, denom1 = p.denom1;
-    if (SIMPLE) {
-        sp = (sp + arlx1i * (zetax2 * divu - rep_prs)) * denom1;
-        sm = (sm + arlx1i * etax2 * tension) * denom1;
-        s12 = (s12 + arlx1i * p5 * etax2 * shear) * denom1;
-    } else {
-        sp = (sp * (1.0 - arlx1i * revp) + arlx1i * (zetax2 * divu - rep_prs)) * denom1;
-        sm = (sm * (1.0 - arlx1i * revp) + arlx1i * etax2 * tension) * denom1;
-        s12 = (s12 * (1.0 - arlx1i * revp) + arlx1i * p5 * etax2 * shear) * denom1;
-    }
-}
-__device__ __forceinline__ void corner_operands(int q, double dxT, double dyT, double cxp, double cyp, double cxm, double cym,
-                                                CornerIn &c, double &KX, double &K12X, double &KYP, double &K12Y)
-{
-    const bool east = q == 0 || q == 3, north = q < 2;
-    c.cyA = east ? cyp : cym; c.cyB = east ? cym : cyp;
-    c.cxA = north ? cxp : cxm; c.cxB = north ? cxm : cxp;
-    c.DY = east ? -dyT : dyT;
-    c.DX = north ? -dxT : dxT;
-    KX = (east ? -p25 : p25) * dyT;
-    K12X = (north ? -p5 : p5) * dxT;
-    KYP = (north ? -p25 : p25) * dxT;
-    K12Y = (east ? -p5 : p5) * dyT;
-}
-__device__ __forceinline__ void stress_corner_partials(double P0, double P1, double P2, double P3, double M0, double M1, double M2,
-                                                       double M3, double T0, double T1, double T2, double T3, double KX, double K12X,
-                                                       double KYP, double K12Y, double dxhy, double dyhx, double &X, double &Y)
-{
-    const double csigp = p111 * P0 + (P1 + P3) * p055 + p027 * P2;
-    const double csigm = p111 * M0 + (M1 + M3) * p055 + p027 * M2;
-    const double csig12 = p222 * T0 + (T1 + T3) * p111 + p055 * T2;
-    const double str12x = K12X * (p333 * (T0 + T3) + p166 * (T1 + T2));
-    const double str12y = K12Y * (p333 * (T0 + T1) + p166 * (T2 + T3));
-    const double strp_x = KX * (p333 * (P0 + P1) + p166 * (P2 + P3));
-    const double strm_x = KX * (p333 * (M0 + M1) + p166 * (M2 + M3));
-    X = strp_x + strm_x + str12x + dxhy * (-csigp + csigm) + dyhx * csig12;
-    const double strp_y = KYP * (p333 * (P0 + P3) + p166 * (P1 + P2));
-    const double strm_y = -KYP * (p333 * (M0 + M3) + p166 * (M1 + M2));
-    Y = strp_y + strm_y + str12y - dyhx * (csigp + csigm) + dxhy * csig12;
-}
-
-struct StepuIn {
-    double uold, vold;
-    double vrelfac;
-    double uocn, vocn, waterx, watery, forcex, forcey, Umassdti, fm, uarear, TbU;
-    double uvel_init, vvel_init;
-    double sx0, sx1, sx2, sx3;
-    double sy0, sy1, sy2, sy3;
-};
-
-struct StepuOut {
-    double u, v, strintx, strinty, taubx, tauby;
-};
-
-struct StepuPre {
-    double taux, tauy, Cb, cca, ccb, ab2;
-    double bu, bv;
-};
-
-template <bool SIMPLE = false, bool TBU = true, bool WITH_B = true>
-__device__ __forceinline__ void stepu_pre_cell(const EvpScalars &p, const StepuIn &a, StepuPre &w)
-{
-    const double uold = a.uold, vold = a.vold;
-    const double du = a.uocn - uold, dv = a.vocn - vold;
-    const double vrel = a.vrelfac * sqrt(du * du + dv * dv);
-    w.taux = vrel * a.waterx;
-    w.tauy = vrel * a.watery;
-    double Cb = 0.0;
-    if (TBU) Cb = a.TbU / (sqrt(uold * uold + vold * vold) + p.u0);
-    w.Cb = Cb;
-    double cca, ccb;
-    if (SIMPLE) {
-        cca = p.brlx * a.Umassdti + vrel + Cb;
-        ccb = a.fm;
-    } else {
-        cca = (p.brlx + p.revp) * a.Umassdti + vrel * p.cosw + Cb;
-        ccb = a.fm + copysign(1.0, a.fm) * vrel * p.sinw;
-    }
-    w.cca = cca; w.ccb = ccb;
-    w.ab2 = cca * cca + ccb * ccb;
-    if (!WITH_B) return;
-    if (SIMPLE) {
-        w.bu = p.brlx * uold + 0.0;
-        w.bv = p.brlx * vold + 0.0;
-    } else {
-        w.bu = p.brlx * uold + p.revp * a.uvel_init;
-        w.bv = p.brlx * vold + p.revp * a.vvel_init;
-    }
-}
-
-template <bool SIMPLE = false, bool WITH_B = true>
-__device__ __forceinline__ void stepu_post_cell(const EvpScalars &p, const StepuIn &a, const StepuPre &w, StepuOut &o)
-{
-    o.strintx = a.uarear * (a.sx0 + a.sx1 + a.sx2 + a.sx3);
-    o.strinty = a.uarear * (a.sy0 + a.sy1 + a.sy2 + a.sy3);
-    double cc1, cc2;
-    if (WITH_B) {
-        cc1 = o.strintx + a.forcex + w.taux + a.Umassdti * w.bu;
-        cc2 = o.strinty + a.forcey + w.tauy + a.Umassdti * w.bv;
-    } else if (SIMPLE) {
-        cc1 = o.strintx + a.forcex + w.taux + a.Umassdti * (p.brlx * a.uold + 0.0);
-        cc2 = o.strinty + a.forcey + w.tauy + a.Umassdti * (p.brlx * a.vold + 0.0);
-    } else {
-        cc1 = o.strintx + a.forcex + w.taux + a.Umassdti * (p.brlx * a.uold + p.revp * a.uvel_init);
-        cc2 = o.strinty + a.forcey + w.tauy + a.Umassdti * (p.brlx * a.vold + p.revp * a.vvel_init);
-    }
-    o.u = (w.cca * cc1 + w.ccb * cc2) / w.ab2;
-    o.v = (w.cca * cc2 - w.ccb * cc1) / w.ab2;
-    o.taubx = -o.u * w.Cb;
-    o.tauby = -o.v * w.Cb;
-}
-
-template <bool SIMPLE = false, bool TBU = true>
-__device__ __forceinline__ void stepu_cell(const EvpScalars &p, const StepuIn &a, StepuOut &o)
-{
-    StepuPre w;
-    stepu_pre_cell<SIMPLE, TBU, false>(p, a, w);
-    stepu_post_cell<SIMPLE, false>(p, a, w, o);
-}
-
-struct DeformOut {
-    double divu, shear, vort, rdg_conv, rdg_shear;
-};
-
-__device__ __forceinline__ void deform_cell(const EvpScalars &p, const StressIn &a, double tarear,
-                                            double dyU_ij, double dyU_im, double dyU_jm, double dyU_mm,
-                                            double dxU_ij, double dxU_im, double dxU_jm, double dxU_mm,
-                                            DeformOut &o)
-{
-    const double divune = a.cyp * a.u_ij - a.dyT * a.u_im + a.cxp * a.v_ij - a.dxT * a.v_jm;
-    const double divunw = a.cym * a.u_im + a.dyT * a.u_ij + a.cxp * a.v_im - a.dxT * a.v_mm;
-    const double divusw = a.cym * a.u_mm + a.dyT * a.u_jm + a.cxm * a.v_mm + a.dxT * a.v_im;
-    const double divuse = a.cyp * a.u_jm - a.dyT * a.u_mm + a.cxm * a.v_jm + a.dxT * a.v_ij;
-    const double tensionne = -a.cym * a.u_ij - a.dyT * a.u_im + a.cxm * a.v_ij + a.dxT * a.v_jm;
-    const double tensionnw = -a.cyp * a.u_im + a.dyT * a.u_ij + a.cxm * a.v_im + a.dxT * a.v_mm;
-    const double tensionsw = -a.cyp * a.u_mm + a.dyT * a.u_jm + a.cxp * a.v_mm - a.dxT * a.v_im;
-    const double tensionse = -a.cym * a.u_jm - a.dyT * a.u_mm + a.cxp * a.v_jm - a.dxT * a.v_ij;
-    const double shearne = -a.cym * a.v_ij - a.dyT * a.v_im - a.cxm * a.u_ij - a.dxT * a.u_jm;
-    const double shearnw = -a.cyp * a.v_im + a.dyT * a.v_ij - a.cxm * a.u_im - a.dxT * a.u_mm;
-    const double shearsw = -a.cyp * a.v_mm + a.dyT * a.v_jm - a.cxp * a.u_mm + a.dxT * a.u_im;
-    const double shearse = -a.cym * a.v_jm - a.dyT * a.v_mm - a.cxp * a.u_jm + a.dxT * a.u_ij;
-    const double Deltane = sqrt(divune * divune + p.e_factor * (tensionne * tensionne + shearne * shearne));
-    const double Deltanw = sqrt(divunw * divunw + p.e_factor * (tensionnw * tensionnw + shearnw * shearnw));
-    const double Deltasw = sqrt(divusw * divusw + p.e_factor * (tensionsw * tensionsw + shearsw * shearsw));
-    const double Deltase = sqrt(divuse * divuse + p.e_factor * (tensionse * tensionse + shearse * shearse));
-
     o.divu = p25 * (divune + divunw + divuse + divusw) * tarear;
     const double tmp = p25 * (Deltane + Deltanw + Deltase + Deltasw) * tarear;
     o.rdg_conv = -fmin(o.divu, 0.0);
diff --git a/cice_amd/csrc/evp_device.h b/cice_amd/csrc/evp_device.h
--- a/cice_amd/csrc/evp_device.h
+++ b/cice_amd/csrc/evp_device.h
@@ -84,6 +84,13 @@
     void *const *peer_raw;
     const size_t *peer_raw_stride;
 };
+#ifndef EVP_RES2_RANGE_DEFAULT
+#define EVP_RES2_RANGE_DEFAULT 1
+#endif
+#ifdef CICE_EVP_HIP_TESTING
+hipError_t evp_range_math_probe(long long n, const double *x, const double *num, const double *den, double *sqrt_lib, double *sqrt_core,
+                                double *div_lib, double *div_core, unsigned char *verdict, hipStream_t st);
+#endif
 int evp_resident2_max_blocks_per_cu(bool strict, int cap, unsigned flags, int logw, bool remote, bool coop = false);
 bool evp_resident2_coop_built(bool strict, int cap, int logw, bool remote);
 bool evp_resident2_lean_built(bool strict, int cap, int logw, bool remote);
diff --git a/cice_amd/csrc/evp_host_resident.cpp b/cice_amd/csrc/evp_host_resident.cpp
--- a/cice_amd/csrc/evp_host_resident.cpp
+++ b/cice_amd/csrc/evp_host_resident.cpp
@@ -403,7 +403,8 @@
         R.prof = S.res2_prof;
     }
     const int dbg2 = env_test("CICE_EVP_HIP_RES_DEBUG") ? std::atoi(env_test("CICE_EVP_HIP_RES_DEBUG")) : 0;
-    R.dbg = dbg2;
+    const int want_range = env_test("CICE_EVP_HIP_RES_RANGE") ? std::atoi(env_test("CICE_EVP_HIP_RES_RANGE")) : EVP_RES2_RANGE_DEFAULT;
+    R.dbg = dbg2 | (want_range ? 0 : 1024);
     R.seam = S.res2_seam;
     R.tfold = S.plan.tfold ? 1 : 0;
     R.img3 = S.res2_img3;
diff --git a/cice_amd/csrc/evp_math.h b/cice_amd/csrc/evp_math.h
--- a/cice_amd/csrc/evp_math.h
+++ b/cice_amd/csrc/evp_math.h
@@ -1,6 +1,7 @@
 #pragma once
 #include <hip/hip_runtime.h>
 #include "evp_device.h"
+#include "evp_range_math.h"
 
 namespace {
 
@@ -39,11 +40,22 @@
     }
     template <int MODE = -1, bool TBU = true>
     static __device__ __forceinline__ void stepu(const EvpScalars &p, const UI &a, UO &o) { evp_strict::stepu_cell<MODE == 3, TBU>(p, a, o); }
+    template <int MODE, class POL>
+    static __device__ __forceinline__ void stress(const EvpScalars &p, const SI &a, double (&s)[12], double (&str)[8], const POL &pol)
+    {
+        evp_strict::stress_cell<(MODE == 3 ? 1 : MODE), MODE == 3, POL>(p, a, s, str, pol);
+    }
+    template <int MODE, bool TBU, class POL>
+    static __device__ __forceinline__ void stepu(const EvpScalars &p, const UI &a, UO &o, const POL &pol) { evp_strict::stepu_cell<MODE == 3, TBU, POL>(p, a, o, pol); }
     using UP = evp_strict::StepuPre;
     template <int MODE = -1, bool TBU = true>
     static __device__ __forceinline__ void stepu_pre(const EvpScalars &p, const UI &a, UP &w) { evp_strict::stepu_pre_cell<MODE == 3, TBU>(p, a, w); }
     template <int MODE = -1>
     static __device__ __forceinline__ void stepu_post(const EvpScalars &p, const UI &a, const UP &w, UO &o) { evp_strict::stepu_post_cell<MODE == 3, true>(p, a, w, o); }
+    template <int MODE, bool TBU, class POL>
+    static __device__ __forceinline__ void stepu_pre(const EvpScalars &p, const UI &a, UP &w, const POL &pol) { evp_strict::stepu_pre_cell<MODE == 3, TBU, true, POL>(p, a, w, pol); }
+    template <int MODE, class POL>
+    static __device__ __forceinline__ void stepu_post(const EvpScalars &p, const UI &a, const UP &w, UO &o, const POL &) { evp_strict::stepu_post_cell<MODE == 3, true, POL>(p, a, w, o); }
     static __device__ __forceinline__ void metrics(double hte, double hte_im, double htn, double htn_jm, double dmin, SI &a)
     {
         evp_strict::metrics_cell(hte, hte_im, htn, htn_jm, dmin, a);
@@ -77,11 +89,22 @@
     }
     template <int MODE = -1, bool TBU = true>
     static __device__ __forceinline__ void stepu(const EvpScalars &p, const UI &a, UO &o) { evp_fused::stepu_cell<MODE == 3, TBU>(p, a, o); }
+    template <int MODE, class POL>
+    static __device__ __forceinline__ void stress(const EvpScalars &p, const SI &a, double (&s)[12], double (&str)[8], const POL &pol)
+    {
+        evp_fused::stress_cell<(MODE == 3 ? 1 : MODE), MODE == 3, POL>(p, a, s, str, pol);
+    }
+    template <int MODE, bool TBU, class POL>
+    static __device__ __forceinline__ void stepu(const EvpScalars &p, const UI &a, UO &o, const POL &pol) { evp_fused::stepu_cell<MODE == 3, TBU, POL>(p, a, o, pol); }
     using UP = evp_fused::StepuPre;
     template <int MODE = -1, bool TBU = true>
     static __device__ __forceinline__ void stepu_pre(const EvpScalars &p, const UI &a, UP &w) { evp_fused::stepu_pre_cell<MODE == 3, TBU>(p, a, w); }
     template <int MODE = -1>
     static __device__ __forceinline__ void stepu_post(const EvpScalars &p, const UI &a, const UP &w, UO &o) { evp_fused::stepu_post_cell<MODE == 3, true>(p, a, w, o); }
+    template <int MODE, bool TBU, class POL>
+    static __device__ __forceinline__ void stepu_pre(const EvpScalars &p, const UI &a, UP &w, const POL &pol) { evp_fused::stepu_pre_cell<MODE == 3, TBU, true, POL>(p, a, w, pol); }
+    template <int MODE, class POL>
+    static __device__ __forceinline__ void stepu_post(const EvpScalars &p, const UI &a, const UP &w, UO &o, const POL &) { evp_fused::stepu_post_cell<MODE == 3, true, POL>(p, a, w, o); }
     static __device__ __forceinline__ void metrics(double hte, double hte_im, double htn, double htn_jm, double dmin, SI &a)
     {
         evp_fused::metrics_cell(hte, hte_im, htn, htn_jm, dmin, a);
diff --git a/cice_amd/csrc/evp_range_math.h b/cice_amd/csrc/evp_range_math.h
--- /dev/null
+++ b/cice_amd/csrc/evp_range_math.h
@@ -0,0 +1,73 @@
+#pragma once
+#include <hip/hip_runtime.h>
+
+namespace evp_range {
+
+constexpr int WIN_EXP = 250;
+constexpr unsigned WIN_LO_HI = (unsigned)(1023 - WIN_EXP) << 20;
+constexpr unsigned WIN_SPAN_HI = (unsigned)(2 * WIN_EXP) << 20;
+
+__device__ __forceinline__ unsigned hi_word(double x) { return (unsigned)((unsigned long long)__double_as_longlong(x) >> 32); }
+__device__ __forceinline__ unsigned off_pos(double x) { return hi_word(x) - WIN_LO_HI; }
+__device__ __forceinline__ unsigned off_abs(double x) { return (hi_word(x) & 0x7fffffffu) - WIN_LO_HI; }
+__device__ __forceinline__ bool outside(unsigned off) { return off >= WIN_SPAN_HI; }
+__device__ __forceinline__ unsigned umax(unsigned a, unsigned b) { return a > b ? a : b; }
+
+__device__ __forceinline__ double sqrt_core(double x)
+{
+#pragma clang fp contract(off)
+    const double r = __builtin_amdgcn_rsq(x);
+    double g = x * r;
+    double h = 0.5 * r;
+    const double e = __builtin_fma(-h, g, 0.5);
+    g = __builtin_fma(g, e, g);
+    h = __builtin_fma(h, e, h);
+    double d = __builtin_fma(-g, g, x);
+    g = __builtin_fma(d, h, g);
+    d = __builtin_fma(-g, g, x);
+    g = __builtin_fma(d, h, g);
+    return g;
+}
+
+__device__ __forceinline__ double div_core(double n, double d)
+{
+#pragma clang fp contract(off)
+    double r = __builtin_amdgcn_rcp(d);
+    double e = __builtin_fma(-d, r, 1.0);
+    r = __builtin_fma(r, e, r);
+    e = __builtin_fma(-d, r, 1.0);
+    r = __builtin_fma(r, e, r);
+    double q = n * r;
+    e = __builtin_fma(-d, q, n);
+    q = __builtin_fma(e, r, q);
+    return q;
+}
+
+struct LibMath {
+    static constexpr bool ranged = false;
+    static constexpr bool lazy_taub = false;
+};
+struct RangeMath {
+    static constexpr bool ranged = true;
+    static constexpr bool lazy_taub = false;
+    unsigned long long cbad = 0;
+    bool off = false;
+    mutable unsigned nlib = 0;
+    __device__ __forceinline__ bool wave_inside(bool lane_outside, bool with_cbad) const
+    {
+        if (off) { ++nlib; return false; }
+        unsigned long long bad = __builtin_amdgcn_ballot_w64(lane_outside);
+        if (with_cbad) bad |= cbad;
+        if (__builtin_expect(bad != 0, 0)) { ++nlib; return false; }
+        return true;
+    }
+    static __device__ __forceinline__ bool percall_outside(double strength, double DminTarea)
+    {
+        return outside(off_abs(strength)) || outside(off_pos(DminTarea));
+    }
+};
+struct RangeMathLazy : RangeMath {
+    static constexpr bool lazy_taub = true;
+};
+
+}
diff --git a/cice_amd/csrc/evp_resident2.hip b/cice_amd/csrc/evp_resident2.hip
--- a/cice_amd/csrc/evp_resident2.hip
+++ b/cice_amd/csrc/evp_resident2.hip
@@ -1,6 +1,7 @@
 #include <hip/hip_runtime.h>
 #include <stdint.h>
 #include <algorithm>
+#include <type_traits>
 
 #ifdef CICE_EVP_HIP_TESTING
 #define RES_DBG(R) ((R).dbg)
@@ -89,6 +90,13 @@
     static_assert(!LEAN || (!REMOTE && !COOP && LOGW == 4), "LEAN: one rank, 16 x 16 tiles, one thread per rim cell");
     static_assert(!RIMU || LEAN, "RIMU: a schedule of the lean loop");
     using MM = Math<STRICT>;
+#ifdef CICE_EVP_HIP_TESTING
+    constexpr bool RANGE = LEAN;
+#else
+    constexpr bool RANGE = LEAN && EVP_RES2_RANGE_DEFAULT;
+#endif
+    using POL = std::conditional_t<RANGE, std::conditional_t<RIMU, evp_range::RangeMathLazy, evp_range::RangeMath>, evp_range::LibMath>;
+    using POLE = std::conditional_t<RANGE, evp_range::RangeMath, evp_range::LibMath>;
     constexpr int W = 1 << LOGW;
     constexpr int H = 256 / W;
     constexpr int LW = W + 1;
@@ -268,6 +276,8 @@
 
     typename MM::SI a;
     double s[12];
+    POL pol;
+    bool percall_out = false;
     if (actN) {
 #pragma unroll
         for (int k = 0; k < 12; ++k) s[k] = R.tab[R.cur0 * 12 + k][c];
@@ -284,7 +294,13 @@
         s_tc[1 * 256 + t] = a.DminTarea;
         s_tc[2 * 256 + t] = a.dxhy;
         s_tc[3 * 256 + t] = a.dyhx;
-    }
+        if constexpr (POL::ranged) percall_out = POL::percall_outside(a.strength, a.DminTarea);
+    }
+    if constexpr (POL::ranged) {
+        pol.cbad = __builtin_amdgcn_ballot_w64(percall_out);
+        pol.off = (RES_DBG(R) & 1024) != 0;
+    }
+    const POLE &pole = pol;
     if (isU) {
         s_uc[0 * 256 + t] = A.vrelfac[cu];
         s_uc[1 * 256 + t] = A.uocn[cu];
@@ -500,7 +516,7 @@
             a.u_mm = s_u[li - LW - 1]; a.v_mm = s_v[li - LW - 1];
             a.strength = s_tc[0 * 256 + t]; a.DminTarea = s_tc[1 * 256 + t];
             a.dxhy = s_tc[2 * 256 + t]; a.dyhx = s_tc[3 * 256 + t];
-            MM::template stress<CAP>(A.p, a, s, str);
+            MM::template stress<CAP, POLE>(A.p, a, s, str, pole);
         }
         EVP_STAMP(pacc1)
         double sx1, sy2;
@@ -572,8 +588,8 @@
             q.sx2 = s_str[0 * SP + sp + SW]; q.sx3 = s_str[2 * SP + sp + SW + 1];
             q.sy0 = str[4]; q.sy1 = s_str[1 * SP + sp + SW];
             q.sy2 = sy2; q.sy3 = s_str[3 * SP + sp + SW + 1];
-            if (tbu) MM::template stepu<CAP, true>(A.p, q, o);
-            else MM::template stepu<CAP, false>(A.p, q, o);
+            if (tbu) MM::template stepu<CAP, true, POLE>(A.p, q, o, pole);
+            else MM::template stepu<CAP, false, POLE>(A.p, q, o, pole);
             u_own = o.u; v_own = o.v;
             if (k == R.ndte - 1 && !R.dry) {
                 R.tab[24][c] = o.strintx; R.tab[25][c] = o.strinty;
@@ -687,7 +703,7 @@
     if constexpr (RIMU) if (rimw && isU) {
         typename MM::UI q;
         ucell_operands(q);
-        MM::template stepu_pre<CAP, false>(A.p, q, upre);
+        MM::template stepu_pre<CAP, false, POL>(A.p, q, upre, pol);
     }
     auto subcycle_rim = [&](const int k, const v4u *rd, v4u *wr) -> bool {
         const unsigned want = R.tag_base + (unsigned)k;
@@ -739,7 +755,7 @@
                 a.u_mm = s_u[li - LW - 1]; a.v_mm = s_v[li - LW - 1];
                 a.strength = s_tc[0 * 256 + t]; a.DminTarea = s_tc[1 * 256 + t];
                 a.dxhy = s_tc[2 * 256 + t]; a.dyhx = s_tc[3 * 256 + t];
-                MM::template stress<CAP>(A.p, a, s, str);
+                MM::template stress<CAP, POL>(A.p, a, s, str, pol);
                 s_str[0 * SP + sp] = str[2];
                 s_str[1 * SP + sp] = str[5];
                 s_str[2 * SP + sp] = str[3];
@@ -775,6 +791,34 @@
         }
         if (!bad) {
             double fin0 = 0.0, fin1 = 0.0, fin2 = 0.0, fin3 = 0.0;
+            if constexpr (POL::lazy_taub) {
+                typename MM::UO o;
+                if (isU) {
+                    typename MM::UI q;
+                    ucell_operands(q);
+                    q.sx0 = s_str[6 * SP + usp]; q.sx1 = s_str[4 * SP + usp + 1];
+                    q.sx2 = s_str[0 * SP + usp + SW]; q.sx3 = s_str[2 * SP + usp + SW + 1];
+                    q.sy0 = s_str[7 * SP + usp]; q.sy1 = s_str[1 * SP + usp + SW];
+                    q.sy2 = s_str[5 * SP + usp + 1]; q.sy3 = s_str[3 * SP + usp + SW + 1];
+                    if (!rimw) MM::template stepu_pre<CAP, false, POL>(A.p, q, upre, pol);
+                    MM::template stepu_post<CAP, POL>(A.p, q, upre, o, pol);
+                    u_own = o.u; v_own = o.v;
+                }
+                if (ownU) {
+                    const unsigned tag = want + 1u;
+                    if (pub) st_rec2_s(wr, own_off, pack_rec(u_own, tag), pack_rec(v_own, tag));
+                    if (img0 >= 0) st_rec2_s(wr, img_off0, pack_rec(img_sg0 * u_own, tag), pack_rec(img_sg0 * v_own, tag));
+                    if (img1 >= 0) st_rec2_s(wr, img_off1, pack_rec(img_sg1 * u_own, tag), pack_rec(img_sg1 * v_own, tag));
+                    if (img2 >= 0) st_rec2_s(wr, img_off2, pack_rec(img_sg2 * u_own, tag), pack_rec(img_sg2 * v_own, tag));
+                }
+                if (isU) {
+                    s_u[uli] = u_own; s_v[uli] = v_own;
+                    if (k == R.ndte - 1 && !R.dry) {
+                        R.tab[24][cu] = o.strintx; R.tab[25][cu] = o.strinty;
+                        R.tab[26][cu] = -u_own * upre.Cb; R.tab[27][cu] = -v_own * upre.Cb;
+                    }
+                }
+            } else {
             if (isU) {
                 typename MM::UI q;
                 typename MM::UO o;
@@ -783,8 +827,8 @@
                 q.sx2 = s_str[0 * SP + usp + SW]; q.sx3 = s_str[2 * SP + usp + SW + 1];
                 q.sy0 = s_str[7 * SP + usp]; q.sy1 = s_str[1 * SP + usp + SW];
                 q.sy2 = s_str[5 * SP + usp + 1]; q.sy3 = s_str[3 * SP + usp + SW + 1];
-                if (!rimw) MM::template stepu_pre<CAP, false>(A.p, q, upre);
-                MM::template stepu_post<CAP>(A.p, q, upre, o);
+                if (!rimw) MM::template stepu_pre<CAP, false, POL>(A.p, q, upre, pol);
+                MM::template stepu_post<CAP, POL>(A.p, q, upre, o, pol);
                 u_own = o.u; v_own = o.v;
                 fin0 = o.strintx; fin1 = o.strinty; fin2 = o.taubx; fin3 = o.tauby;
             }
@@ -802,6 +846,7 @@
                     R.tab[26][cu] = fin2; R.tab[27][cu] = fin3;
                 }
             }
+            }
             EVP_STAMP(pacc3)
         }
         __syncthreads();
@@ -810,7 +855,7 @@
         if (rimw && isU) {
             typename MM::UI q;
             ucell_operands(q);
-            MM::template stepu_pre<CAP, false>(A.p, q, upre);
+            MM::template stepu_pre<CAP, false, POL>(A.p, q, upre, pol);
         }
         return true;
     };
@@ -840,7 +885,9 @@
         unsigned long long *o = R.prof + ((size_t)tile * 4 + (tq >> 6)) * 8;
         o[0] = pacc0; o[1] = pacc1; o[2] = pacc2; o[3] = pacc3; o[4] = pacc4;
         o[5] = (unsigned long long)cu_rank | ((unsigned long long)(PERM && R.cuload ? s_cu : 0) << 8) | ((unsigned long long)(s_simd[t >> 6] & 3) << 24);
-        o[6] = (unsigned long long)(t >> 6); o[7] = (unsigned long long)R.nact[tile];
+        unsigned long long nlib = 0;
+        if constexpr (POL::ranged) nlib = pol.nlib;
+        o[6] = (unsigned long long)(t >> 6) | (nlib << 8); o[7] = (unsigned long long)R.nact[tile];
     }
     if (REMOTE && ring_remote) {
         v4u ra, rb;
@@ -921,6 +968,33 @@
 
 }
 
+#ifdef CICE_EVP_HIP_TESTING
+namespace {
+__global__ __launch_bounds__(256) void range_math_probe(long long n, const double *x, const double *num, const double *den, double *sqrt_lib,
+                                                        double *sqrt_core, double *div_lib, double *div_core, unsigned char *verdict)
+{
+    const long long e = (long long)blockIdx.x * 256 + threadIdx.x;
+    if (e >= n) return;
+    const double xx = x[e], nn = num[e], dd = den[e];
+    sqrt_lib[e] = sqrt(xx);
+    sqrt_core[e] = evp_range::sqrt_core(xx);
+    div_lib[e] = nn / dd;
+    div_core[e] = evp_range::div_core(nn, dd);
+    const bool x_in = !evp_range::outside(evp_range::off_pos(xx));
+    const bool q_in = !evp_range::outside(evp_range::umax(evp_range::off_abs(nn), evp_range::off_abs(dd)));
+    verdict[e] = (unsigned char)((x_in ? 1 : 0) | (q_in ? 2 : 0));
+}
+}
+hipError_t evp_range_math_probe(long long n, const double *x, const double *num, const double *den, double *sqrt_lib, double *sqrt_core,
+                                double *div_lib, double *div_core, unsigned char *verdict, hipStream_t st)
+{
+    if (n <= 0) return hipSuccess;
+    hipLaunchKernelGGL(range_math_probe, dim3((unsigned)((n + 255) / 256)), dim3(256), 0, st, n, x, num, den, sqrt_lib, sqrt_core, div_lib,
+                       div_core, verdict);
+    return hipGetLastError();
+}
+#endif
+
 void evp_resident_geometry(int max_ni, int max_nj, int logw, int *gx, int *gy)
 {
     const int W = 1 << logw, H = 256 / W;
diff --git a/cice_amd/evp.py b/cice_amd/evp.py
--- a/cice_amd/evp.py
+++ b/cice_amd/evp.py
@@ -42,7 +42,7 @@
     "cice_evp_hip_debug_device_allocs", "cice_evp_hip_debug_cuload", "cice_evp_hip_debug_prof", "cice_evp_hip_debug_cgrid_prof", "cice_evp_hip_debug_cgres_prof", "cice_evp_hip_plan_build", "cice_evp_hip_halo_plan", "cice_evp_hip_seam_plan",
     "cice_evp_hip_peer_plan", "cice_evp_hip_peer_signs", "cice_evp_hip_center_plan", "cice_evp_hip_stress_plan",
     "cice_evp_hip_fold_split_plan", "cice_evp_hip_plan_flags", "cice_evp_hip_fold_images_plan", "cice_evp_hip_cgrid_fold_xplan",
-    "cice_evp_hip_cgrid_fold_xpeers", "cice_evp_hip_plan_dump", "cice_evp_hip_rim_plan",
+    "cice_evp_hip_cgrid_fold_xpeers", "cice_evp_hip_plan_dump", "cice_evp_hip_rim_plan", "cice_evp_hip_debug_range_math",
 ]
 TEST_ENV = [
     "CICE_EVP_HIP_RES_REMOTE", "CICE_EVP_HIP_RES_REMOTE_BREAK", "CICE_EVP_HIP_RES_ORDER", "CICE_EVP_HIP_RES_PROF", "CICE_EVP_HIP_RES_DEBUG",
@@ -51,7 +51,7 @@
     "CICE_EVP_HIP_CGRID_ONE_STRIP", "CICE_EVP_HIP_CGRID_FAST", "CICE_EVP_HIP_HALO_DEBUG", "CICE_EVP_HIP_SEAM_FIN", "CICE_EVP_HIP_OVERLAP",
     "CICE_EVP_HIP_HALO_RIDE", "CICE_EVP_HIP_GATHER", "CICE_EVP_HIP_SIMPLE", "CICE_EVP_HIP_SELF_EXCHANGE", "CICE_EVP_HIP_FLAGS", "CICE_EVP_HIP_LEAN",
     "CICE_EVP_HIP_PREFETCH", "CICE_EVP_HIP_FAULT_REPLAY", "CICE_EVP_HIP_MARCH_BANDSEG", "CICE_EVP_HIP_CGRID_PROF",
-    "CICE_EVP_HIP_NO_OVERLAP", "CICE_EVP_HIP_TYB", "CICE_EVP_HIP_NOGRAPH", "CICE_EVP_HIP_GRAPH_RCCL", "CICE_EVP_HIP_RES_LOGW", "CICE_EVP_HIP_RES_COOP", "CICE_EVP_HIP_RES_LEAN", "CICE_EVP_HIP_RES_RIMU",
+    "CICE_EVP_HIP_NO_OVERLAP", "CICE_EVP_HIP_TYB", "CICE_EVP_HIP_NOGRAPH", "CICE_EVP_HIP_GRAPH_RCCL", "CICE_EVP_HIP_RES_LOGW", "CICE_EVP_HIP_RES_COOP", "CICE_EVP_HIP_RES_LEAN", "CICE_EVP_HIP_RES_RIMU", "CICE_EVP_HIP_RES_RANGE",
     "CICE_EVP_HIP_MARCH_EXT", "CICE_EVP_HIP_MARCH_DIRECT", "CICE_EVP_HIP_CGRID_FUSED", "CICE_EVP_HIP_CGRID_GEO",
     "CICE_EVP_HIP_CGRID_RES_SLEEP", "CICE_EVP_HIP_CGRID_RES_CULL", "CICE_EVP_HIP_CGRID_RES_DEBUG",
     "CICE_EVP_HIP_CGRID_STRIP", "CICE_EVP_HIP_CGRID_STRIP_SEG", "CICE_EVP_HIP_CGRID_STRIP_EDGE", "CICE_EVP_HIP_CGRID_STRIP_RIDE", "CICE_EVP_HIP_CGRID_STRIP_LEN", "CICE_EVP_HIP_CGRID_STRIP_ITEMS", "CICE_EVP_HIP_CGRID_STRIP_LAST",
@@ -857,3 +857,19 @@
         _check(lib, rc if rc < 0 else -1, "(rim_plan)")
     return dict(perm=perm, uperm=uperm, cls=cls, n_lt=info[:, 0], n_lu=info[:, 1], nact=info[:, 2], nact_packed=info[:, 3],
                 ok=info[:, 4].astype(bool), gx=int(info[0, 5]), gy=int(info[0, 6]))
+
+
+def range_math(x: np.ndarray, num: np.ndarray, den: np.ndarray) -> dict:
+    lib = load_library(testing=True)
+    x, num, den = (np.ascontiguousarray(a, dtype=np.float64) for a in (x, num, den))
+    assert x.ndim == 1 and x.shape == num.shape == den.shape
+    n = x.size
+    out = {k: np.empty(n, dtype=np.float64) for k in ("sqrt_lib", "sqrt_core", "div_lib", "div_core")}
+    verdict = np.zeros(n, dtype=np.uint8)
+    dp = lambda a: a.ctypes.data_as(_f64p)
+    _check(lib, lib.cice_evp_hip_debug_range_math(C.c_int64(n), dp(x), dp(num), dp(den), dp(out["sqrt_lib"]), dp(out["sqrt_core"]),
+                                                  dp(out["div_lib"]), dp(out["div_core"]), verdict.ctypes.data_as(C.POINTER(C.c_uint8))),
+           "(debug_range_math)")
+    out["x_inside"] = (verdict & 1) != 0
+    out["q_inside"] = (verdict & 2) != 0
+    return out
diff --git a/include/cice_evp_hip_testing.h b/include/cice_evp_hip_testing.h
--- a/include/cice_evp_hip_testing.h
+++ b/include/cice_evp_hip_testing.h
@@ -31,6 +31,8 @@
 int cice_evp_hip_march_fold_plan(const cice_evp_hip_dims *dims, int32_t ext, int32_t tyb, int32_t *out10, int32_t *tile_rows);
 int cice_evp_hip_debug_cuload(int32_t *out, int32_t n);
 int cice_evp_hip_debug_prof(uint64_t *out, int32_t ntiles_max);
+int cice_evp_hip_debug_range_math(int64_t n, const double *x, const double *num, const double *den, double *sqrt_lib, double *sqrt_core,
+                                  double *div_lib, double *div_core, uint8_t *verdict);
 int cice_evp_hip_debug_cgrid_prof(uint64_t *out, int32_t ntiles_max);
 int cice_evp_hip_debug_cgres_prof(uint64_t *out, int32_t ntiles_max);
 int cice_evp_hip_debug_device_allocs(int64_t *count);
```

Measured after the change: 33.30 billion, median of 6. 2.8% higher.
